# zhuker/lamejs

Measured on AMD Instinct MI355X. Metric: 1152-sample frames/s encoded (44.1kHz 128kbps CBR); bit-exact, higher is better.
Workload: dtype f64; 1 GPU; BASELINE configs[2]: stereo 44.1kHz 128kbps CBR, 1 stream(s) x 100000 synthetic sine frames per GPU; input=Int16 PCM resident in HBM, output=MP3 bytes in HBM, seed_repaired_frames=0, distinct_streams=1, distinct_devices=1

## Files before the change

### lamejs_amd/csrc/k_quant.h

```cpp
#pragma once
#include "lhip_defs.h"
#include "lhip_wave.h"
#include "lhip_math.h"
#include "lhip_layout.h"

namespace lhip {

struct GI {
    double xrpow_max;
    int part2_3_length, big_values, count1, global_gain, scalefac_compress, block_type;
    int table_select[3], subblock_gain[4];
    int region0_count, region1_count, preflag, scalefac_scale, count1table_select;
    int part2_length, sfb_lmax, sfb_smin, psy_lmax, sfbmax, psymax, sfbdivide;
    int count1bits, max_nonzero_coeff;
    int firstcut;
};

struct NoiseRes { double max_noise; int over_count, over_SSD, bits; };

LHIP_DEV void uni_gi(GI& g) {
    g.xrpow_max = unid(g.xrpow_max);
    g.part2_3_length = uni(g.part2_3_length); g.big_values = uni(g.big_values); g.count1 = uni(g.count1); g.global_gain = uni(g.global_gain);
    g.scalefac_compress = uni(g.scalefac_compress); g.block_type = uni(g.block_type);
    for (int i = 0; i < 3; i++) g.table_select[i] = uni(g.table_select[i]);
    for (int i = 0; i < 4; i++) g.subblock_gain[i] = uni(g.subblock_gain[i]);
    g.region0_count = uni(g.region0_count); g.region1_count = uni(g.region1_count); g.preflag = uni(g.preflag); g.scalefac_scale = uni(g.scalefac_scale);
    g.count1table_select = uni(g.count1table_select); g.part2_length = uni(g.part2_length); g.sfb_lmax = uni(g.sfb_lmax); g.sfb_smin = uni(g.sfb_smin);
    g.psy_lmax = uni(g.psy_lmax); g.sfbmax = uni(g.sfbmax); g.psymax = uni(g.psymax); g.sfbdivide = uni(g.sfbdivide);
    g.count1bits = uni(g.count1bits); g.max_nonzero_coeff = uni(g.max_nonzero_coeff); g.firstcut = uni(g.firstcut);
}

#if defined(LHIP_PHASE_PROF) && !defined(LHIP_HOSTSIM)
#define PH_BEGIN() const unsigned long long ph_t0_ = __builtin_amdgcn_s_memtime()
#define PH_END(L, id) do { if (lane == 0) { (L).prof[id] += (unsigned int)(__builtin_amdgcn_s_memtime() - ph_t0_); (L).prof[32 + id] += 1; } } while (0)
#define PH_MARK(L, id, t) do { const unsigned long long n_ = __builtin_amdgcn_s_memtime(); if (lane == 0) { (L).prof[id] += (unsigned int)(n_ - (t)); (L).prof[32 + id] += 1; } (t) = n_; } while (0)
#define PH_NOW() __builtin_amdgcn_s_memtime()
#else
#define PH_BEGIN() do {} while (0)
#define PH_END(L, id) do {} while (0)
#define PH_MARK(L, id, t) do {} while (0)
#define PH_NOW() 0ull
#endif
#ifdef LHIP_PROF_BALANCE
#define PH_MARKB(L, id, t) PH_MARK(L, id, t)
#else
#define PH_MARKB(L, id, t) do {} while (0)
#endif
enum { PH_INIT, PH_XRPOW, PH_XMIN, PH_QUANTIZE, PH_COUNT, PH_NOISE, PH_BALANCE, PH_SFSTORE, PH_HUFFDIV, PH_PUBLISH, PH_COPY, PH_TOTAL,
       PH_C_LOAD, PH_C_QUADS, PH_C_MAX, PH_C_SUMS, PH_C_FIN, PH_N_WALK, PH_N_TERMS, PH_N_SUMS, PH_Q_MASK, PH_Q_LINES, PH_N, PH_DRAIN = 29 ,
       PH_N_LINES = 30, PH_N_FOLD = 31 ,
       PH_B_TRIG = 22, PH_B_AMP = 23, PH_B_BREAK = 24, PH_B_BITCOUNT = 25  };

enum { QT_N = 256 };
enum { HL_T1 = 0, HL_T2 = 4, HL_T3 = 13, HL_T5 = 22, HL_T6 = 38, HL_T7 = 54, HL_T8 = 90, HL_T9 = 126, HL_T10 = 162, HL_T11 = 226,
       HL_T12 = 290, HL_T13 = 354, HL_T14 = 610, HL_T15 = 866, HL_EHI = 1122, HL_ELO = 1378, HL_END = 1634 };
LHIP_DEV int hl_off(int t) {
    switch (t) {
        case 1: return HL_T1; case 2: return HL_T2; case 3: return HL_T3; case 5: return HL_T5; case 6: return HL_T6;
        case 7: return HL_T7; case 8: return HL_T8; case 9: return HL_T9; case 10: return HL_T10; case 11: return HL_T11;
        case 12: return HL_T12; case 13: return HL_T13; case 14: return HL_T14; case 15: return HL_T15; default: return 0;
    }
}
// ... 196 lines not shown
    for (int k = 0; k < NV; k++) { va[k] = X.a[src[k]]; vb[k] = 0.f; }
    if (X.b) {
#pragma unroll
        for (int k = 0; k < NV; k++) vb[k] = X.b[src[k]];
    }
#pragma unroll
    for (int k = 0; k < NV; k++) { LHIP_PIN_LOADED(va[k]); LHIP_PIN_LOADED(vb[k]); }
#pragma unroll
    for (int k = 0; k < NV; k++) {
        float v = va[k];
        if (X.b) { const double l = va[k], r = vb[k]; v = X.side ? (float)((l - r) * (LHIP_SQRT2 * 0.5)) : (float)((l + r) * (LHIP_SQRT2 * 0.5)); }
        L.xr[lane + LHIP_NL * k] = v;
    }
#endif
}

LHIP_DEV void q_init_outer_loop(const Tables& T, const PowBase& pb10, double ath_adjust, GI& g, int block_type,
                                const XrSrc& xr_g, float* xr_wb, int skip_silence, int lane, QuantLds& L, const QuantTabs& Q) {
    lane = fresh_lane(lane);
    unsigned long long tmi_ = PH_NOW(); (void)tmi_;
    (void)pb10; (void)ath_adjust;
#if defined(LHIP_PHASE_PROF) && !defined(LHIP_HOSTSIM)
    __builtin_amdgcn_s_waitcnt(0);
    PH_MARK(L, PH_DRAIN, tmi_);
#endif
    g.part2_3_length = 0; g.big_values = 0; g.count1 = 0; g.global_gain = 210; g.scalefac_compress = 0;
    g.block_type = block_type;
    g.table_select[0] = g.table_select[1] = g.table_select[2] = 0;
    g.subblock_gain[0] = g.subblock_gain[1] = g.subblock_gain[2] = g.subblock_gain[3] = 0;
    g.region0_count = 0; g.region1_count = 0; g.preflag = 0; g.scalefac_scale = 0; g.count1table_select = 0;
    g.part2_length = 0; g.sfb_lmax = SBPSY_l; g.sfb_smin = SBPSY_s;
    g.psy_lmax = T.sfb21_extra ? SBMAX_l : SBPSY_l;
    g.psymax = g.psy_lmax; g.sfbmax = g.sfb_lmax; g.sfbdivide = 11;
    g.count1bits = 0; g.max_nonzero_coeff = 575; g.xrpow_max = 0; g.firstcut = 64;
    int nsfb;
    if (block_type == SHORT_TYPE) {
        g.sfb_smin = 0; g.sfb_lmax = 0;
        g.psymax = 3 * ((T.sfb21_extra ? SBMAX_s : SBPSY_s));
        g.sfbmax = 3 * SBPSY_s;
        g.sfbdivide = g.sfbmax - 18;
        g.psy_lmax = 0;
        nsfb = 3 * SBMAX_s;
        LHIP_LANE_ONCE(i, 0, nsfb) {
            const int sfb = i / 3, win = i - 3 * sfb;
            const int w = Q.sfb_s[sfb + 1] - Q.sfb_s[sfb];
            L.width[i] = (int16_t)w; L.window[i] = (int16_t)win; L.start[i] = (int16_t)(3 * Q.sfb_s[sfb] + win * w);
        }
        if (lane == 0) L.start[nsfb] = 576;
        q_load_lines(xr_g, 1, lane, L, Q);
    } else {
        nsfb = SBMAX_l;
        LHIP_LANE_ONCE(i, 0, SBMAX_l) {
            L.width[i] = (int16_t)(Q.sfb_l[i + 1] - Q.sfb_l[i]); L.window[i] = 3; L.start[i] = (int16_t)Q.sfb_l[i];
        }
        if (lane == 0) L.start[SBMAX_l] = 576;
        q_load_lines(xr_g, 0, lane, L, Q);
    }
    LHIP_LANE_ONCE(i, 0, (SFBMAX) + 1) { L.sfw[i] = 0; L.sfb[i] = 0; }
    wave_sync();
    PH_MARK(L, PH_COPY, tmi_);

    if (skip_silence) return;
    if (block_type != SHORT_TYPE) {
        const int lo = Q.psfb21[0];
        int top = lo - 1;
        for (int j = lo + lane; j < 576; j += LHIP_NL) {
            int gsfb = 0;
// ... 62 lines not shown
#else
    unsigned endm = 0;
    double keep[NLN_FOLD]; int bnd[NLN_FOLD];
    int prevb = (lane == 0) ? -1 : (int)l2s[NLN_FOLD * lane - 1];
#pragma unroll
    for (int k = 0; k < NLN_FOLD; k++) {
        const int j = NLN_FOLD * lane + k;
        bnd[k] = l2s[j];
        keep[k] = (bnd[k] != prevb) ? 0.0 : 1.0;
        prevb = bnd[k];
    }
    const int nextb = (lane == LHIP_NL - 1) ? -1 : (int)l2s[NLN_FOLD * (lane + 1)];
#pragma unroll
    for (int k = 0; k < NLN_FOLD; k++) if (bnd[k] != (k + 1 < NLN_FOLD ? bnd[k + 1 < NLN_FOLD ? k + 1 : k] : nextb)) endm |= 1u << k;
    const int nsteps = (maxlen + NLN_FOLD - 1) / NLN_FOLD + 1;
    double carry = 0.0;
    for (int st = 0; st + 1 < nsteps; st++) {
        double sacc = carry;
#pragma unroll
        for (int k = 0; k < NLN_FOLD; k++) sacc = __builtin_fma(sacc, keep[k], tq[k]);
        carry = wave_shr1d(sacc, 0.0);
    }
    {
        double sacc = carry;
#pragma unroll
        for (int k = 0; k < NLN_FOLD; k++) { sacc = __builtin_fma(sacc, keep[k], tq[k]); tq[k] = sacc; }
    }
#pragma unroll
    for (int k = 0; k < NLN_FOLD; k++) if ((endm >> k) & 1u) L.nsum[bnd[k]] = tq[k];
#endif
    wave_sync();
}

LHIP_DEV void q_calc_xmin(const Tables& T, double ath_adjust, double masking_lower, const float* ratio ,
                          GI& g, int lane, QuantLds& L, const QuantTabs& Q) {
    lane = fresh_lane(lane);
    {
        double tq[NLN_FOLD];
#pragma unroll
        for (int k = 0; k < NLN_FOLD; k++) { const double x = L.xr[NLN_FOLD * lane + k]; tq[k] = x * x; }
        int maxw = 0;
        const int nb = (g.block_type != SHORT_TYPE) ? g.psy_lmax : 3 * SBPSY_s;
        LHIP_LANE_ONCE(b, 0, nb) if (maxw < L.width[b]) maxw = L.width[b];
        maxw = wave_max(maxw);
        fold_band_sums(tq, line2sfb(Q, g.block_type), maxw, lane, L);
    }
    if (g.block_type != SHORT_TYPE) {
        LHIP_LANE_ONCE(gsfb, 0, g.psy_lmax) {
            double xmin = ath_adjust * (double)T.ATH_l[gsfb];
            const double en0 = L.nsum[gsfb];
            const double en = ratio[E_EN_L + gsfb];
            if (en > 0.0) {
                const double x = en0 * (double)ratio[E_THM_L + gsfb] * masking_lower / en;
                if (xmin < x) xmin = x;
            }
            const float xm = (float)(xmin * (double)T.longfact[gsfb]);
            L.xmin[gsfb] = xm; L.rxmin[gsfb] = recip_for_div((double)xm);
        }
        int t = -1;
        for (int k = lane; k < 576; k += LHIP_NL) if (!((double)L.xr[k] == 0)) t = k;
        t = wave_max(t);
        g.max_nonzero_coeff = (t >= 575) ? 575 : t + 1;
    } else {
        LHIP_LANE_ONCE(sfb, 0, SBPSY_s) {
            const double tmpATH = ath_adjust * (double)T.ATH_s[sfb];
            float px[3];
            for (int b = 0; b < 3; b++) {
                const int gs = 3 * sfb + b;
                double xmin = tmpATH;
                const double en0 = L.nsum[gs];
                const double en = ratio[E_EN_S + sfb * 3 + b];
                if (en > 0.0) {
                    const double x = en0 * (double)ratio[E_THM_S + sfb * 3 + b] * masking_lower / en;
                    if (xmin < x) xmin = x;
                }
                px[b] = (float)(xmin * (double)T.shortfact[sfb]);
            }
            if (T.useTemporal) {
                if ((double)px[0] > (double)px[1]) px[1] = (float)((double)px[1] + ((double)px[0] - (double)px[1]) * T.decay);
                if ((double)px[1] > (double)px[2]) px[2] = (float)((double)px[2] + ((double)px[1] - (double)px[2]) * T.decay);
            }
            L.xmin[3 * sfb] = px[0]; L.xmin[3 * sfb + 1] = px[1]; L.xmin[3 * sfb + 2] = px[2];
            L.rxmin[3 * sfb] = recip_for_div((double)px[0]); L.rxmin[3 * sfb + 1] = recip_for_div((double)px[1]); L.rxmin[3 * sfb + 2] = recip_for_div((double)px[2]);
        }
        g.max_nonzero_coeff = 575;
    }
    q_set_firstcut(g, lane, L);
    wave_sync();
}

enum { NPL = (288 + LHIP_NL - 1) / LHIP_NL };
LHIP_DEV void q_quantize(const Tables& T, const GI& g, const int32_t* scalefac, int16_t* ix, int use_prev,
                         int pn_gain, int pn_sfb_count1, int (&vx)[NPL], int (&vy)[NPL], int lane, QuantLds& L, const QuantTabs& Q) {
    lane = fresh_lane(lane);
    const double istep = ipow20(Q, g.global_gain);
    const int may_big = !(g.xrpow_max * istep < (double)QT_N);
    const int sfbmax = (g.block_type == SHORT_TYPE) ? 38 : 21;
    const int prev_data_use = use_prev && (g.global_gain == pn_gain);
    unsigned long long tm_ = PH_NOW(); (void)tm_;
    float xa[NPL], xb[NPL];
#pragma unroll
    for (int j = 0; j < NPL; j++) {
        const int p = 2 * (lane + LHIP_NL * j);
        xa[j] = 0.f; xb[j] = 0.f;
        if (p < 576) { struct F2 { float x, y; }; const F2 xx = *(const F2*)(L.xrpow + p); xa[j] = xx.x; xb[j] = xx.y; }
    }
    uint64_t m_cached = 0, m_zo = 0;
    if (use_prev) {
        LHIP_LANE_ONCE(sfb, 0, (sfbmax) + 1) {
            int step = -1;
            const int pstep = L.pn_step[sfb];
            if (prev_data_use || g.block_type == NORM_TYPE) step = sf_step(Q, g, scalefac, L.window, sfb);
            if (prev_data_use && pstep == step) m_cached |= 1ull << sfb;
            else if (pn_sfb_count1 > 0 && sfb >= pn_sfb_count1 && pstep > 0 && step >= pstep) m_zo |= 1ull << sfb;
        }
    }
    m_cached = wave_lane_bits(m_cached); m_zo = wave_lane_bits(m_zo);
    const uint64_t m_cut = (use_prev && g.firstcut <= sfbmax) ? ((~0ull << g.firstcut) & ((2ull << sfbmax) - 1) & ~m_cached) : 0;
    const int sstar = m_cut ? (int)__builtin_ctzll(m_cut) : 99;
    if (sstar <= sfbmax) m_zo &= ~(1ull << sstar);
    PH_MARK(L, PH_Q_MASK, tm_);
    const uint8_t* l2s = line2sfb(Q, g.block_type);
    const int need_old = (m_cached != 0);
    const float istep_f = Q.ipow20[g.global_gain];
    int ra[NPL], rb[NPL];
    q_floor_prod(xa, xb, istep_f, ra, rb);
    float aa[NPL], ab[NPL];
    if (!may_big) {
#pragma unroll
        for (int j = 0; j < NPL; j++) { aa[j] = Q.adj43[ra[j]]; ab[j] = Q.adj43[rb[j]]; }
    } else {
#pragma unroll
        for (int j = 0; j < NPL; j++) { aa[j] = Q.adj43[ra[j] < QT_N ? ra[j] : QT_N - 1]; ab[j] = Q.adj43[rb[j] < QT_N ? rb[j] : QT_N - 1]; }
#pragma unroll
        for (int j = 0; j < NPL; j++) {
            if (ra[j] >= QT_N) aa[j] = T.adj43[ra[j]];
            if (rb[j] >= QT_N) ab[j] = T.adj43[rb[j]];
        }
    }
    q_floor_fma(xa, xb, istep_f, aa, ab, vx, vy);
    if (!need_old && m_zo == 0) {
#pragma unroll
        for (int j = 0; j < NPL; j++) {
            const int p = 2 * (lane + LHIP_NL * j);
            if (p < 576) *(uint32_t*)(ix + p) = (uint32_t)vx[j] | ((uint32_t)vy[j] << 16);
        }
    } else if (m_zo == 0) {
#pragma unroll
        for (int j = 0; j < NPL; j++) {
            const int p = 2 * (lane + LHIP_NL * j);
            int sf = 0; uint32_t oldw = 0;
            if (p < 576) { sf = l2s[p]; oldw = *(const uint32_t*)(ix + p); }
            const int cached = (int)((m_cached >> sf) & 1);
            const int va = cached ? (int)(oldw & 0xffffu) : vx[j], vb = cached ? (int)(oldw >> 16) : vy[j];
            vx[j] = va; vy[j] = vb;
            if (p < 576) *(uint32_t*)(ix + p) = (uint32_t)va | ((uint32_t)vb << 16);
        }
    } else {
        const double compareval0 = (1.0 - 0.4054) / istep;
        float zo_thr = (float)compareval0;
        if ((double)zo_thr < compareval0) zo_thr = f32_next_up(zo_thr);
#pragma unroll
        for (int j = 0; j < NPL; j++) {
            const int p = 2 * (lane + LHIP_NL * j);
            int sf = 0; uint32_t oldw = 0;
            if (p < 576) { sf = l2s[p]; if (need_old) oldw = *(const uint32_t*)(ix + p); }
            const int cached = (int)((m_cached >> sf) & 1), zo = (int)((m_zo >> sf) & 1);
            int va = vx[j], vb = vy[j];
            if (zo) { va = (xa[j] < zo_thr) ? 0 : 1; vb = (xb[j] < zo_thr) ? 0 : 1; }
            const int oa = (int)(oldw & 0xffffu), ob = (int)(oldw >> 16);
            va = cached ? oa : va;
            vb = cached ? ob : vb;
            vx[j] = va; vy[j] = vb;
            if (p < 576) *(uint32_t*)(ix + p) = (uint32_t)va | ((uint32_t)vb << 16);
        }
    }
    wave_sync();
    PH_MARK(L, PH_Q_LINES, tm_);
}

struct RegionPlan { int kind, t1, xlen, lb1, lb2, choice, choice2, o0, o1, o2; };

LHIP_DEV void esc_choice(int mx15, int* choice, int* choice2, int* lb1, int* lb2) {
    const int bl = 32 - __builtin_clz((unsigned)mx15);
    const int c24 = bl <= 4 ? 0 : bl <= 9 ? bl - 4 : bl <= 11 ? 6 : 7;
    int f16 = bl <= 4 ? bl - 1 : 4 + ((bl - 5) >> 1);
    if (f16 > 7) f16 = 7;
    int c16 = c24 - 8 + 8;
    if (c16 < f16) c16 = f16;
    *choice2 = 24 + c24; *choice = 16 + c16;
    *lb1 = (int)((0xDA864321u >> (4 * c16)) & 15u);
    *lb2 = (int)((0xDB987654u >> (4 * c24)) & 15u);
}

LHIP_DEV int plan_index(int m) { return m <= 15 ? m : (m <= IXMAX_VAL ? 15 + (32 - __builtin_clz((unsigned)(m - 15) | 1u)) : 29); }
LHIP_DEV void q_fill_plans(QuantTabs& Q, int tid, int nthr) {
// ... 59 lines not shown
        case 2: { int t1 = r.t1, sum2 = s0 & 0xffff, sum = s0 >> 16; if (sum > sum2) { sum = sum2; t1++; } *bits += sum; return t1; }
        case 4: { int t = r.t1; if (s0 > s1) { s0 = s1; t++; } if (s0 > s2) { s0 = s2; t = r.t1 + 2; } *bits += s0; return t; }
        case 5: { int c = r.choice; if (s0 > s1) { s0 = s1; c = r.choice2; } *bits += s0; return c; }
        default: *bits = LARGE_BITS; return -1;
    }
}

LHIP_DEV int q_choose_table(const Tables& T, const int16_t* ix, int a, int b, int* bits, int lane, const QuantLds& L, const QuantTabs& Q) {
    int mx = 0;
    for (int p = a + 2 * lane; p < b; p += 2 * LHIP_NL) { const int x1 = ix[p], x2 = ix[p + 1]; if (mx < x1) mx = x1; if (mx < x2) mx = x2; }
    mx = wave_max(mx);
    const RegionPlan r = plan_region_(Q, mx);
    int s0 = 0, s1 = 0, s2 = 0;
    if (r.kind >= 1 && r.kind <= 5)
        for (int p = a + 2 * lane; p < b; p += 2 * LHIP_NL) pair_bits(Q, r, ix[p], ix[p + 1], s0, s1, s2);
    s0 = wave_sum(s0);
    if (r.kind >= 4) s1 = wave_sum(s1);
    if (r.kind == 4) s2 = wave_sum(s2);
    return finish_region(r, s0, s1, s2, bits);
}

LHIP_DEV int pack_cond_fields(const GI& g, int mask) {
    return mask | ((g.table_select[0] + 1) << 4) | ((g.table_select[1] + 1) << 10) | ((g.table_select[2] + 1) << 16) |
           (g.region0_count << 22) | (g.region1_count << 26);
}
LHIP_DEV int apply_cond_fields(int state, int asg) {
    if (asg & 1) state = (state & ~(63 << 4)) | (asg & (63 << 4));
    if (asg & 2) state = (state & ~(63 << 10)) | (asg & (63 << 10));
    if (asg & 4) state = (state & ~(63 << 16)) | (asg & (63 << 16));
    if (asg & 8) state = (state & ~(0x3ff << 22)) | (asg & (0x3ff << 22));
    return state & ~15;
}

LHIP_DEV int q_noquant_count_bits(const Tables& T, GI& g, const int16_t* ix, int (&vx)[NPL], int (&vy)[NPL], int use_prev, int* pn_sfb_count1, int* asg_mask, int lane, QuantLds& L, const QuantTabs& Q) {
    *asg_mask = 0;
    lane = fresh_lane(lane);
    unsigned long long tm_ = PH_NOW(); (void)tm_;
    int i = ((g.max_nonzero_coeff + 2) >> 1) << 1;
    if (i > 576) i = 576;
    if (use_prev) *pn_sfb_count1 = 0;
    int firstbig;
#if LHIP_NL == 1
    {
        int top = 0;
        for (int j = 0; j < NPL; j++) if ((vx[j] | vy[j]) != 0) top = 2 * (lane + LHIP_NL * j) + 2;
        i = top;
        const int nq = i >> 2;
        firstbig = nq;
        for (int k = 0; k < nq; k++) {
            const int e = i - 4 * k;
            if (((ix[e - 1] | ix[e - 2] | ix[e - 3] | ix[e - 4]) & 0x7fff) > 1) { firstbig = k; break; }
        }
    }
#else
    {
        int tp = -1, bp = -1;
#pragma unroll
        for (int j = 0; j < NPL; j++) {
            const uint64_t nz = wave_ballot((vx[j] | vy[j]) != 0), bg = wave_ballot((vx[j] | vy[j]) > 1);
            if (nz) tp = 64 * j + 63 - (int)__builtin_clzll(nz);
            if (bg) bp = 64 * j + 63 - (int)__builtin_clzll(bg);
        }
        i = 2 * tp + 2;
        const int P = tp + 1, nq = i >> 2;
        firstbig = (P - 1 - bp) >> 1;
        if (firstbig > nq) firstbig = nq;
    }
#endif
    g.count1 = i;
    PH_MARK(L, PH_C_LOAD, tm_);
    int a12 = 0;
    for (int k = lane; k < firstbig; k += LHIP_NL) {
        const int e = i - 4 * k;
        const uint32_t w0 = *(const uint32_t*)(ix + e - 4), w1 = *(const uint32_t*)(ix + e - 2);
        const int p = (int)(((w0 & 1u) << 3) | ((w0 >> 16) << 2) | ((w1 & 1u) << 1) | (w1 >> 16));
        a12 += Q.t32l[p] + (Q.t33l[p] << 16);
    }
    i -= 4 * firstbig;
    g.big_values = i;
    int a1, a2, bits;
#define COUNT1_FINISH(A12) do { const int c1_ = (A12) & 0xffff, c2_ = (int)((unsigned)(A12) >> 16); bits = c1_; g.count1table_select = 0; \
                                if (c1_ > c2_) { bits = c2_; g.count1table_select = 1; } g.count1bits = bits; } while (0)
    PH_MARK(L, PH_C_QUADS, tm_);
    if (i == 0) { const int t = wave_sum(a12); COUNT1_FINISH(t); return bits; }
    int use2 = 0, cnt1_norm = 0;
    if (g.block_type == SHORT_TYPE) {
        a1 = 3 * Q.sfb_s[3];
        if (a1 > g.big_values) a1 = g.big_values;
        a2 = g.big_values;
    } else if (g.block_type == NORM_TYPE) {
        const uint32_t bt = Q.bvtab[i >> 1];
        g.region0_count = (int)((bt >> 20) & 15u); g.region1_count = (int)((bt >> 24) & 7u);
        a1 = (int)(bt & 1023u); a2 = (int)((bt >> 10) & 1023u);
        cnt1_norm = (int)(bt >> 27);
        if (a2 < i) use2 = 1;
    } else {
        g.region0_count = 7;
        g.region1_count = SBMAX_l - 1 - 7 - 1;
        a1 = Q.sfb_l[7 + 1];
        a2 = i;
        if (a1 > a2) a1 = a2;
    }
    if (a1 > i) a1 = i;
    if (a2 > i) a2 = i;
    *asg_mask = (g.block_type != SHORT_TYPE ? 8 : 0) | (use2 ? 4 : 0) | (0 < a1 ? 1 : 0) | (a1 < a2 ? 2 : 0);
    int m0 = 0, m1 = 0, m2 = 0;
    int rj[NPL];
#pragma unroll
    for (int j = 0; j < NPL; j++) {
        rj[j] = 3;
        if (2 * LHIP_NL * j >= i) continue;
        const int p = 2 * (lane + LHIP_NL * j);
        const int r = (p >= a1) + (p >= a2) + (p >= i);
        const int m = vx[j] > vy[j] ? vx[j] : vy[j];
        const int mr0 = (r == 0) ? m : 0, mr1 = (r == 1) ? m : 0, mr2 = (r == 2) ? m : 0;
        m0 = m0 > mr0 ? m0 : mr0; m1 = m1 > mr1 ? m1 : mr1; m2 = m2 > mr2 ? m2 : mr2;
        rj[j] = r;
    }
    { int mm[3] = {m0, m1, m2}; wave_max_n(mm); m0 = mm[0]; m1 = mm[1]; m2 = mm[2]; }
    struct LanePlan { int kind, t0, t1, t2, lbA, lbB; };
#if LHIP_NL == 1
    LanePlan lp[3]; int pv[3];
#define LP_(r) lp[r]
#define PV_(r) pv[r]
#else
    LanePlan lp1; int pv1 = 0;
    lp1.kind = 0; lp1.t0 = lp1.t1 = lp1.t2 = lp1.lbA = lp1.lbB = 0;
#define LP_(r) lp1
#define PV_(r) pv1
#endif
    LHIP_LANE_ONCE(r, 0, 3) {
        const int m = (r == 0) ? m0 : (r == 1) ? m1 : (r == 2) ? m2 : 0;
        const QuantTabs::PlanEnt pe = Q.plan[plan_index(m)];
        L.rdesc[r][0] = pe.d0;
        L.rdesc[r][1] = pe.d1;
        LanePlan& q = LP_(r);
        q.kind = (int)(pe.pw & 7u); q.t0 = (int)((pe.pw >> 3) & 63u); q.t1 = (int)((pe.pw >> 9) & 63u); q.t2 = (int)((pe.pw >> 15) & 63u);
        q.lbA = (int)((pe.pw >> 21) & 15u); q.lbB = (int)((pe.pw >> 25) & 15u);
    }
    wave_sync();
    PH_MARK(L, PH_C_MAX, tm_);
#if LHIP_NL == 1
    typedef uint64_t acc_t; enum { FB = 21 };
#else
    typedef uint32_t acc_t; enum { FB = 10 };
#endif
    const acc_t FM = ((acc_t)1 << FB) - 1;
    acc_t accA = 0, accB = 0, accC = 0, accN = 0;
    const int any_esc = (m0 > 15) | (m1 > 15) | (m2 > 15);
#if LHIP_NL == 1
#pragma unroll
    for (int j = 0; j < NPL; j++) {
        const int p = 2 * (lane + LHIP_NL * j);
        if (p < i) {
            const int r = (p >= a1) + (p >= a2);
            const uint64_t d = *(const uint64_t*)L.rdesc[r];
            const uint32_t d0 = (uint32_t)d, d1 = (uint32_t)(d >> 32);
            const int x = vx[j], y = vy[j];
            const int idx = (x < 15 ? x : 15) * (int)(d1 >> 16) + (y < 15 ? y : 15);
            const int sh = FB * r;
            accA += (acc_t)Q.hlen[(d0 & 0xffffu) + idx] << sh;
            accB += (acc_t)Q.hlen[(d0 >> 16) + idx] << sh;
            accC += (acc_t)Q.hlen[(d1 & 0xffffu) + idx] << sh;
            if (any_esc) accN += (acc_t)((x > 14) + (y > 14)) << sh;
        }
    }
    (void)rj;
#else
    if (any_esc) {
#pragma unroll
        for (int j = 0; j < NPL; j++) {
            if (rj[j] < 3) {
                const int r = rj[j];
                const uint64_t d = *(const uint64_t*)L.rdesc[r];
                const uint32_t d0 = (uint32_t)d, d1 = (uint32_t)(d >> 32);
                const int x = vx[j], y = vy[j];
                const int idx = (x < 15 ? x : 15) * (int)(d1 >> 16) + (y < 15 ? y : 15);
                const unsigned mult = 1u << (FB * r);
                accA = mul24((unsigned)Q.hlen[(d0 & 0xffffu) + idx], mult) + accA;
                accB = mul24((unsigned)Q.hlen[(d0 >> 16) + idx], mult) + accB;
                accC = mul24((unsigned)Q.hlen[(d1 & 0xffffu) + idx], mult) + accC;
                accN = mul24((unsigned)((x > 14) + (y > 14)), mult) + accN;
            }
        }
    } else {
#pragma unroll
        for (int j = 0; j < NPL; j++) {
            if (rj[j] < 3) {
                const int r = rj[j];
                const uint64_t d = *(const uint64_t*)L.rdesc[r];
                const uint32_t d0 = (uint32_t)d, d1 = (uint32_t)(d >> 32);
                const int idx = vx[j] * (int)(d1 >> 16) + vy[j];
                const unsigned mult = 1u << (FB * r);
                accA = mul24((unsigned)Q.hlen[(d0 & 0xffffu) + idx], mult) + accA;
                accB = mul24((unsigned)Q.hlen[(d0 >> 16) + idx], mult) + accB;
                accC = mul24((unsigned)Q.hlen[(d1 & 0xffffu) + idx], mult) + accC;
            }
        }
    }
#endif
#define FLD(A, R) ((uint32_t)(((A) >> (FB * (R))) & FM))
    int qq[7] = {(int)(FLD(accA, 0) | (FLD(accB, 0) << 16)), (int)(FLD(accC, 0) | (FLD(accN, 0) << 16)), (int)(FLD(accA, 1) | (FLD(accB, 1) << 16)),
                 (int)(FLD(accC, 1) | (FLD(accN, 1) << 16)), (int)(FLD(accA, 2) | (FLD(accB, 2) << 16)), (int)(FLD(accC, 2) | (FLD(accN, 2) << 16)), a12};
    wave_sum_n(qq);
    const int q0 = qq[0], q1 = qq[1], q2 = qq[2], q3 = qq[3], q4 = qq[4], q5 = qq[5];
    COUNT1_FINISH(qq[6]);
#undef COUNT1_FINISH
#undef FLD
    PH_MARK(L, PH_C_SUMS, tm_);
    LHIP_LANE_ONCE(r, 0, 3) {
        const LanePlan& q = LP_(r);
        const int qa = (r == 0) ? q0 : (r == 1) ? q2 : q4, qc = (r == 0) ? q1 : (r == 1) ? q3 : q5;
        const int n = (int)((unsigned)qc >> 16);
        const int c0 = (qa & 0xffff) + n * q.lbA, c1 = (int)((unsigned)qa >> 16) + n * q.lbB, c2 = qc & 0xffff;
        int b = c0, t = q.t0;
        if ((q.kind == 2 || q.kind == 4 || q.kind == 5) && b > c1) { b = c1; t = q.t1; }
        if (q.kind == 4 && b > c2) { b = c2; t = q.t2; }
        if (q.kind == 0) { b = 0; t = 0; }
        if (q.kind == 6) { b = 0; t = 63; }
        PV_(r) = t | ((q.kind == 6) << 6) | (b << 8);
    }
#if LHIP_NL == 1
    const int pv0 = pv[0], pv1_ = pv[1], pv2 = pv[2];
#else
    const int pv0 = wave_bcast(pv1, 0), pv1_ = wave_bcast(pv1, 1), pv2 = wave_bcast(pv1, 2);
#endif
#define APPLY(PV, SLOT) do { const int t_ = (PV) & 63; if ((PV) & 64) bits = LARGE_BITS; else bits += (PV) >> 8; g.table_select[SLOT] = (t_ == 63) ? -1 : t_; } while (0)
    if (use2) APPLY(pv2, 2);
    if (0 < a1) APPLY(pv0, 0);
    if (a1 < a2) APPLY(pv1_, 1);
#undef APPLY
#undef LP_
#undef PV_
    if (use_prev && g.block_type == NORM_TYPE) *pn_sfb_count1 = cnt1_norm;
    PH_MARK(L, PH_C_FIN, tm_);
    return bits;
}

struct PrevNoise { int gain, sfb_count1; };

LHIP_DEV int q_count_bits(const Tables& T, GI& g, const int32_t* scalefac, int16_t* ix, int use_pn, PrevNoise& pn, int* asg, int lane, QuantLds& L, const QuantTabs& Q) {
    *asg = 0;
    {
        const double ip = ipow20(Q, g.global_gain);
        if (g.xrpow_max * ip > (double)IXMAX_VAL * (1.0 - 0x1p-50)) {
            const double w = (double)IXMAX_VAL / ip;
            if (g.xrpow_max > w) return LARGE_BITS;
        }
    }
    int vx[NPL], vy[NPL];
    { PH_BEGIN(); q_quantize(T, g, scalefac, ix, use_pn, use_pn ? pn.gain : 0, use_pn ? pn.sfb_count1 : 0, vx, vy, lane, L, Q); PH_END(L, PH_QUANTIZE); }
    int cnt1 = pn.sfb_count1;
    PH_BEGIN();
    int amask = 0;
    const int r = q_noquant_count_bits(T, g, ix, vx, vy, use_pn, &cnt1, &amask, lane, L, Q);
    *asg = pack_cond_fields(g, amask);
    if (use_pn) pn.sfb_count1 = cnt1;
    PH_END(L, PH_COUNT);
    return r;
}

struct NoiseCommit { int fresh, step, cls; float dist; double x; };
LHIP_DEV void q_noise_commit(const GI& g, const NoiseCommit& nc, PrevNoise& pn, int lane, QuantLds& L) {
    lane = fresh_lane(lane);
    LHIP_LANE_ONCE(sfb, 0, g.psymax) {
        if (nc.fresh) { L.pn_step[sfb] = nc.step; L.pn_dist[sfb] = nc.dist; L.pn_x[sfb] = nc.x; L.pn_cls[sfb] = (int16_t)nc.cls; }
    }
    pn.gain = g.global_gain;
    wave_sync();
}
LHIP_DEV void q_calc_noise_(const Tables& T, const GI& g, const int32_t* scalefac, const int16_t* ix, NoiseRes* res,
                           int use_pn, PrevNoise& pn, int need_max, int lane, QuantLds& L, const QuantTabs& Q, NoiseCommit* defer = nullptr) {
    lane = fresh_lane(lane);
    unsigned long long tm_ = PH_NOW(); (void)tm_;
    const int is_short = g.block_type == SHORT_TYPE;
    const int may_big = !(g.xrpow_max * ipow20(Q, g.global_gain) < (double)(QT_N - 1));
#if LHIP_NL == 1
    const uint8_t* l2s = line2sfb(Q, g.block_type);
    int over = 0, ssd = 0;
    uint64_t m_fresh = 0;
    (void)may_big; (void)is_short;
    for (int sfb = 0; sfb < g.psymax; sfb++) {
        const int s = sf_step(Q, g, scalefac, L.window, sfb);
        if (!(use_pn && L.pn_step[sfb] == s)) m_fresh |= 1ull << sfb;
        L.qmode[sfb] = s;
        L.bstep[sfb] = Q.pow20[s + Q_MAX2];
    }
    PH_MARK(L, PH_N_WALK, tm_);
    {
        double sacc = 0.0;
        for (int j = 0; j < 576; j++) {
            const int bnd = l2s[j];
// ... 188 lines not shown
#define LHIP_PIPE_COUNT(f) do { if (lane == 0) pipe_stats().f++; } while (0)
#else
#define LHIP_PIPE_COUNT(f) do { } while (0)
#endif
#if LHIP_NL != 1
LHIP_DEV void q_count_helper(const Tables& T, CountShare& cs, const QuantLds& Lo, QuantLds& L, const QuantTabs& Q, int lane) {
    for (;;) {
        const int s = wg_wait_not(&cs.state, CS_IDLE, CS_DONE, lane);
        if (s == CS_QUIT) break;
        if (s == CS_BARRIER) { wg_store(&cs.state, CS_IDLE, lane); wg_barrier(); continue; }
#ifdef LHIP_PHASE_PROF
        const unsigned long long hp_seen_ = __builtin_amdgcn_s_memtime();
#endif
#if HO_ON
        const unsigned long long ho_h0_ = HO_NOW();
#endif
        wg_acquire();
        lane = lane_anew(lane);
        GI g;
        g.block_type = uni(s >> 8); g.max_nonzero_coeff = 0;
        g.region0_count = 0; g.region1_count = 0; g.table_select[0] = g.table_select[1] = g.table_select[2] = 0;
        g.count1table_select = 0; g.count1bits = 0; g.count1 = 0; g.big_values = 0;
        int cnt1 = 0, amask = 0;
        int vx[NPL], vy[NPL];
#pragma unroll
        for (int j = 0; j < NPL; j++) {
            const int i = lane + LHIP_NL * j;
            const uint32_t w = i < 288 ? ((const uint32_t*)Lo.ixw)[i] : 0u;
            vx[j] = (int)(w & 0xffffu); vy[j] = (int)(w >> 16);
        }
#ifdef LHIP_PHASE_PROF
        const unsigned long long hp_start_ = __builtin_amdgcn_s_memtime();
#endif
        const int bits = uni(q_noquant_count_bits(T, g, Lo.ixw, vx, vy, 1, &cnt1, &amask, lane, L, Q));
#ifdef LHIP_PHASE_PROF
        const unsigned long long hp_end_ = __builtin_amdgcn_s_memtime();
#endif
        uni_gi(g);
        const uint32_t w0 = (uint32_t)bits | ((uint32_t)g.count1 << 17);
        const uint32_t w1 = (uint32_t)g.big_values | ((uint32_t)g.count1bits << 10) | ((uint32_t)g.count1table_select << 23) | ((uint32_t)g.region0_count << 24) | ((uint32_t)g.region1_count << 28);
        const uint32_t w2 = (uint32_t)(g.table_select[0] + 1) | ((uint32_t)(g.table_select[1] + 1) << 6) | ((uint32_t)(g.table_select[2] + 1) << 12) | ((uint32_t)uni(cnt1) << 18) | ((uint32_t)uni(amask) << 24);
        if (lane == 0) { cs.w[0] = w0; cs.w[1] = w1; cs.w[2] = w2; }
#ifdef LHIP_PHASE_PROF
        if (lane == 0) { const unsigned long long now_ = __builtin_amdgcn_s_memtime(); cs.acc[0] += (unsigned int)(hp_seen_ - cs.t_post); cs.acc[1] += (unsigned int)(hp_start_ - hp_seen_);
                         cs.acc[2] += (unsigned int)(hp_end_ - hp_start_); cs.acc[3] += (unsigned int)(now_ - hp_end_); cs.acc[7] += 1; cs.t_reply = now_; }
#endif
#if HO_ON
        const unsigned long long ho_h1_ = HO_NOW();
        if (lane == 0) cs.t_reply = ho_h1_;
#endif
        wg_store(&cs.state, CS_DONE, lane);
#if HO_ON
        HO_ADD(cs, 3, ho_h1_ - ho_h0_); HO_ADD(cs, 4, 1); HO_ADD(cs, 5, ho_h0_ - cs.t_post);
#endif
    }
}
LHIP_DEV int q_count_bits_piped(const Tables& T, GI& g, const int32_t* scalefac, int16_t* ix, PrevNoise& pn, int* asg, CountShare& cs,
                                NoiseRes* ni, NoiseCommit* nc, int need_max, int* spec, int lane, QuantLds& L, const QuantTabs& Q) {
    *asg = 0; *spec = 0;
    {
        const double ip = ipow20(Q, g.global_gain);
        if (g.xrpow_max * ip > (double)IXMAX_VAL * (1.0 - 0x1p-50)) {
            const double w = (double)IXMAX_VAL / ip;
            if (g.xrpow_max > w) return LARGE_BITS;
        }
    }
    {
        int vx[NPL], vy[NPL];
        PH_BEGIN(); q_quantize(T, g, scalefac, ix, 1, pn.gain, pn.sfb_count1, vx, vy, lane, L, Q); PH_END(L, PH_QUANTIZE);
        (void)vx; (void)vy;
    }
#ifdef LHIP_PHASE_PROF
    if (lane == 0) cs.t_post = __builtin_amdgcn_s_memtime();
#endif
#if HO_ON
    const unsigned long long ho_t0_ = HO_NOW();
    if (lane == 0) cs.t_post = ho_t0_;
#endif
    wg_store(&cs.state, CS_REQ | (g.block_type << 8), lane);
    LHIP_PIPE_COUNT(piped);
    { PH_BEGIN(); q_calc_noise_(T, g, scalefac, ix, ni, 1, pn, need_max, lane, L, Q, nc); PH_END(L, PH_NOISE); }
    *spec = 1;
#if HO_ON
    const unsigned long long ho_t1_ = HO_NOW();
#endif
    PH_BEGIN();
#ifdef LHIP_PHASE_PROF
    const unsigned long long op_wait0_ = __builtin_amdgcn_s_memtime();
#endif
    (void)wg_wait_not(&cs.state, CS_REQ | (g.block_type << 8), CS_REQ | (g.block_type << 8), lane);
#ifdef LHIP_PHASE_PROF
    if (lane == 0) { const unsigned long long now_ = __builtin_amdgcn_s_memtime(); cs.acc[4] += (unsigned int)(now_ - cs.t_reply); cs.acc[5] += (unsigned int)(op_wait0_ - cs.t_post); cs.acc[6] += (unsigned int)(now_ - op_wait0_); }
#endif
#if HO_ON
    const unsigned long long ho_t2_ = HO_NOW();
#endif
    wg_acquire();
    const uint32_t w0 = (uint32_t)uni((int)cs.w[0]), w1 = (uint32_t)uni((int)cs.w[1]), w2 = (uint32_t)uni((int)cs.w[2]);
#if HO_ON
    HO_ADD(cs, 0, ho_t1_ - ho_t0_); HO_ADD(cs, 1, ho_t2_ - ho_t1_); HO_ADD(cs, 2, 1); HO_ADD(cs, 6, ho_t2_ - cs.t_reply);
#endif
    const int bits = (int)(w0 & 0x1ffffu), amask = (int)((w2 >> 24) & 15u);
// ... 51 lines not shown
    uint32_t m = 0;
    LHIP_LANE_ONCE(i, 0, end) {
        int v = scalefac[i];
        if (v < 0) v = 0;
        const int part = (i >= b1) + (i >= b2) + (i >= b3);
        m |= (uint32_t)v << (8 * part);
    }
    m = (uint32_t)wave_or((int)m);
    int over = 0, slen[4];
    for (int p = 0; p < 4; p++) {
        const uint32_t mp = (m >> (8 * p)) & 0xffu;
        if (mp > ((range >> (8 * p)) & 0xffu)) over = 1;
        slen[p] = mp ? 32 - __builtin_clz(mp) : 0;
    }
    if (!over) {
        g.scalefac_compress = pre ? 500 + slen[0] * 3 + slen[1] : ((slen[0] * 5 + slen[1]) << 4) + (slen[2] << 2) + slen[3];
        g.part2_length = slen[0] * n0 + slen[1] * n1 + slen[2] * n2 + slen[3] * n3;
    }
    return over;
}

LHIP_DEV int q_scale_bitcount_any(const Tables& T, const QuantTabs& Q, GI& g, int32_t* scalefac, int lane) {
    return T.mode_gr == 2 ? q_scale_bitcount(Q, g, scalefac, lane) : q_scale_bitcount_lsf(g, scalefac, lane);
}

LHIP_DEV int q_loop_break(const GI& g, const int32_t* scalefac, int lane, QuantLds& L, const QuantTabs& Q) {
    lane = fresh_lane(lane);
    int z = 0;
    LHIP_LANE_ONCE(sfb, 0, g.sfbmax)
        if (scalefac[sfb] + band_sbgain(g, L.window, sfb) == 0) z = 1;
    return !wave_any(z);
}

LHIP_DEV void q_amplify_flagged(GI& g, double amp, uint64_t m_amp, int lane, QuantLds& L, const QuantTabs& Q) {
    lane = fresh_lane(lane);
    float m = 0.f;
    const uint8_t* l2s = line2sfb(Q, g.block_type);
    struct F2 { float x, y; };
    F2 xx[NPL]; int bnd[NPL];
#pragma unroll
    for (int j = 0; j < NPL; j++) {
        const int p = 2 * (lane + LHIP_NL * j);
        xx[j].x = 0.f; xx[j].y = 0.f; bnd[j] = 0;
        if (p < 576) { xx[j] = *(const F2*)(L.xrpow + p); bnd[j] = l2s[p]; }
    }
#pragma unroll
    for (int j = 0; j < NPL; j++) {
        const int p = 2 * (lane + LHIP_NL * j);
        const double a = ((m_amp >> bnd[j]) & 1) ? amp : 1.0;
        xx[j].x = (float)((double)xx[j].x * a); xx[j].y = (float)((double)xx[j].y * a);
        if (p < 576) *(F2*)(L.xrpow + p) = xx[j];
        m = fmax_nonneg(m, fmax_nonneg(xx[j].x, xx[j].y));
    }
    m = wave_maxf_pos(m);
    if ((double)m > g.xrpow_max) g.xrpow_max = m;
    wave_sync();
}

LHIP_DEV void q_amp_scalefac_bands(const Tables& T, GI& g, int32_t* scalefac, int* all_nonzero, int* pre_bad, int* m12_out,
                                   int lane, QuantLds& L, const QuantTabs& Q) {
    lane = fresh_lane(lane);
    const double ifqstep34 = (g.scalefac_scale == 0) ? 1.29683955465100964055 : 1.68179283050742922612;
    float tr = 0.f;
    LHIP_LANE_ONCE(sfb, 0, g.sfbmax) if (tr < L.distort[sfb]) tr = L.distort[sfb];
    double trigger = wave_maxf_pos(tr);
    const int by_square = T.noise_shaping_amp == 1 && trigger > 1.0;
    const double max_dist = trigger;
    switch (T.noise_shaping_amp) {
        case 2: break;
        case 1:
            if (!(trigger > 1.0)) trigger *= .95;
            break;
        default:
            if (trigger > 1.0) trigger = 1.0;
            else trigger *= .95;
            break;
    }
    uint64_t m_amp = 0;
    LHIP_LANE_ONCE(sfb, 0, g.sfbmax) {
        const double d = (double)L.distort[sfb];
        const int below = by_square ? (d * d < max_dist) : (d < trigger);
        if (!below) m_amp |= 1ull << sfb;
    }
    m_amp = wave_lane_bits(m_amp);
    if (T.noise_shaping_amp == 2 && m_amp) m_amp = 1ull << __builtin_ctzll(m_amp);
    int z = 0, bad = 0, m12 = 0;
    LHIP_LANE_ONCE(sfb, 0, g.sfbmax) {
        const int v = scalefac[sfb] + (int)((m_amp >> sfb) & 1);
        scalefac[sfb] = v;
        if (v + band_sbgain(g, L.window, sfb) == 0) z = 1;
        if (sfb >= 11 && sfb < SBPSY_l && v < Q.pretab[sfb]) bad = 1;
        m12 |= (sfb < g.sfbdivide) ? v : (v << 8);
    }
    {
        const int r = wave_or(m12 | (z << 16) | (bad << 17));
        *m12_out = r & 0xffff; *all_nonzero = !((r >> 16) & 1); *pre_bad = (r >> 17) & 1;
    }
    { unsigned long long tt_ = PH_NOW(); (void)tt_; q_amplify_flagged(g, ifqstep34, m_amp, lane, L, Q); PH_MARKB(L, PH_B_TRIG, tt_); }
}

LHIP_DEV int q_scale_bitcount_from(const QuantTabs& Q, GI& g, int32_t* scalefac, int pre_bad, int m12, int lane) {
    lane = fresh_lane(lane);
    const int sh = (g.block_type == SHORT_TYPE) ? 24 : 16;
    if (g.block_type != SHORT_TYPE && 0 == g.preflag && !pre_bad) {
        g.preflag = 1;
        wave_sync();
        LHIP_LANE_ONCE(sfb, 11, SBPSY_l) scalefac[sfb] -= Q.pretab[sfb];
        wave_sync();
        m12 = 0;
        LHIP_LANE_ONCE(sfb, 0, g.sfbmax) { const int v = scalefac[sfb]; m12 |= (sfb < g.sfbdivide) ? v : (v << 8); }
        m12 = wave_or(m12);
    }
    const int m1 = m12 & 0xff, m2 = m12 >> 8;
    int best = 0x7fffffff;
    LHIP_LANE_ONCE(k, 0, 16) {
        const uint32_t e = Q.sbc[k];
        if (m1 < (int)(e & 0xffu) && m2 < (int)((e >> 8) & 0xffu)) { const int v = (int)((e >> sh) & 0xffu) * 16 + k; if (v < best) best = v; }
    }
    best = wave_min(best);
    g.part2_length = LARGE_BITS;
    if (best != 0x7fffffff) { g.part2_length = best >> 4; g.scalefac_compress = best & 15; }
    return g.part2_length == LARGE_BITS;
}

LHIP_DEV void q_inc_scalefac_scale(const Tables& T, GI& g, int32_t* scalefac, int lane, QuantLds& L, const QuantTabs& Q) {
    lane = fresh_lane(lane);
    uint64_t m_amp = 0;
    LHIP_LANE_ONCE(sfb, 0, g.sfbmax) {
        int s = scalefac[sfb];
        if (g.preflag != 0) s += Q.pretab[sfb];
        if ((s & 1) != 0) { s++; m_amp |= 1ull << sfb; }
        scalefac[sfb] = s >> 1;
    }
    m_amp = wave_lane_bits(m_amp);
    wave_sync();
    g.preflag = 0;
    g.scalefac_scale = 1;
    q_amplify_flagged(g, 1.29683955465100964055, m_amp, lane, L, Q);
}

LHIP_DEV int q_inc_subblock_gain(const Tables& T, GI& g, int32_t* scalefac, int lane, QuantLds& L, const QuantTabs& Q) {
    lane = fresh_lane(lane);
    for (int window = 0; window < 3; window++) {
        int s1 = 0, s2 = 0;
        LHIP_LANE_ONCE3(sfb, window, g.sfbmax) {
            const int v = scalefac[sfb];
            if (sfb < g.sfbdivide) { if (s1 < v) s1 = v; } else { if (s2 < v) s2 = v; }
        }
        s1 = wave_max(s1); s2 = wave_max(s2);
        if (s1 < 16 && s2 < 8) continue;
        if (sbgain(g, window) >= 7) return 1;
        if (window == 0) g.subblock_gain[0]++; else if (window == 1) g.subblock_gain[1]++; else g.subblock_gain[2]++;
        wave_sync();
        for (int sfb = window; sfb < g.sfbmax + 3; sfb += 3) {
            double amp;
            int doamp = 0;
            int s = (sfb < g.sfbmax) ? scalefac[sfb] : 0;
            wave_sync();
            if (sfb < g.sfbmax) {
                s = s - (4 >> g.scalefac_scale);
                if (s >= 0) { if (lane == 0) scalefac[sfb] = s; }
                else {
                    if (lane == 0) scalefac[sfb] = 0;
                    amp = ipow20(Q, 210 + s * (1 << (g.scalefac_scale + 1)));
                    doamp = 1;
                }
            } else { amp = ipow20(Q, 202); doamp = 1; }
            wave_sync();
            if (uni(doamp)) {
                float m = 0.f;
                const int st = L.start[sfb], w = L.width[sfb];
                for (int i = st + lane; i < st + w; i += LHIP_NL) {
                    const float v = (float)((double)L.xrpow[i] * amp);
                    L.xrpow[i] = v;
                    m = fmax_nonneg(m, v);
                }
                m = wave_maxf_pos(m);
                if ((double)m > g.xrpow_max) g.xrpow_max = m;
            }
        }
        wave_sync();
    }
    return 0;
}

LHIP_DEV int q_balance_noise(const Tables& T, GI& g, int32_t* scalefac, int lane, QuantLds& L, const QuantTabs& Q) {
    lane = fresh_lane(lane);
    unsigned long long tb_ = PH_NOW(); (void)tb_;
    int all_nonzero, pre_bad, m12;
    q_amp_scalefac_bands(T, g, scalefac, &all_nonzero, &pre_bad, &m12, lane, L, Q);
    PH_MARKB(L, PH_B_AMP, tb_);
    int status = all_nonzero;
    if (status) return 0;
    status = T.mode_gr == 2 ? q_scale_bitcount_from(Q, g, scalefac, pre_bad, m12, lane) : q_scale_bitcount_lsf(g, scalefac, lane);
    PH_MARKB(L, PH_B_BITCOUNT, tb_);
    if (!status) return 1;
    if (T.noise_shaping > 1) {
        if (0 == g.scalefac_scale) {
            q_inc_scalefac_scale(T, g, scalefac, lane, L, Q);
            status = 0;
        } else if (g.block_type == SHORT_TYPE && T.subblock_gain > 0) {
            status = (q_inc_subblock_gain(T, g, scalefac, lane, L, Q) || q_loop_break(g, scalefac, lane, L, Q));
        }
    }
    if (!status) status = q_scale_bitcount_any(T, Q, g, scalefac, lane);
    return !status;
}

LHIP_DEV int q_quant_compare(const NoiseRes& best, const NoiseRes& calc) {
    int better;
    if (best.over_count > 0) {
        better = calc.over_SSD <= best.over_SSD;
        if (calc.over_SSD == best.over_SSD) better = calc.bits < best.bits;
    } else {
        better = ((calc.max_noise < 0) && ((calc.max_noise * 10 + calc.bits) <= (best.max_noise * 10 + best.bits)));
    }
    if (best.over_count == 0) better = better && calc.bits < best.bits;
    return better;
}

LHIP_DEV void gi_keep_store(QuantLds& L, const GI& w, int lane) {
    lane = fresh_lane(lane);
    if (lane == 0) {
        int32_t* k = L.gkeep;
        k[0] = w.part2_3_length; k[1] = w.big_values; k[2] = w.count1; k[3] = w.global_gain; k[4] = w.scalefac_compress;
        k[5] = w.table_select[0]; k[6] = w.table_select[1]; k[7] = w.table_select[2];
        k[8] = w.subblock_gain[0]; k[9] = w.subblock_gain[1]; k[10] = w.subblock_gain[2]; k[11] = w.subblock_gain[3];
        k[12] = w.region0_count; k[13] = w.region1_count; k[14] = w.preflag; k[15] = w.scalefac_scale; k[16] = w.count1table_select;
        k[17] = w.part2_length; k[18] = w.count1bits;
        union { double d; int32_t i[2]; } u; u.d = w.xrpow_max; k[19] = u.i[0]; k[20] = u.i[1];
    }
}
LHIP_DEV void gi_keep_load(const QuantLds& L, GI& g) {
    const int32_t* k = L.gkeep;
    g.part2_3_length = uni(k[0]); g.big_values = uni(k[1]); g.count1 = uni(k[2]); g.global_gain = uni(k[3]); g.scalefac_compress = uni(k[4]);
    g.table_select[0] = uni(k[5]); g.table_select[1] = uni(k[6]); g.table_select[2] = uni(k[7]);
    g.subblock_gain[0] = uni(k[8]); g.subblock_gain[1] = uni(k[9]); g.subblock_gain[2] = uni(k[10]); g.subblock_gain[3] = uni(k[11]);
    g.region0_count = uni(k[12]); g.region1_count = uni(k[13]); g.preflag = uni(k[14]); g.scalefac_scale = uni(k[15]); g.count1table_select = uni(k[16]);
    g.part2_length = uni(k[17]); g.count1bits = uni(k[18]);
    union { double d; int32_t i[2]; } u; u.i[0] = uni(k[19]); u.i[1] = uni(k[20]); g.xrpow_max = u.d;
}

#if defined(LHIP_HOSTSIM)
struct SearchStats {
    long bs[40] = {0}, bsup[40] = {0}, run[40] = {0}, run_cnt1_moved[40] = {0}, rounds = 0, evals = 0, searches = 0, run_steps = 0, run_steps_cnt1_moved = 0, run_steps_zo = 0;
    long bsdir[8][3][2] = {{{0}}};
    long mfail[24] = {0}, mfit[24] = {0};
    bool on = getenv("LAMEJS_SEARCH_STATS") != nullptr;
    ~SearchStats() {
        if (!on) return;
        fprintf(stderr, "search stats: %ld granule-channel searches, %ld evaluations, %ld outer-loop rounds; %ld evaluations inside gain++ runs (%ld of them with sfb_count1 moved by the evaluation before, %ld with a live 0/1 shortcut)\n", searches, evals, rounds, run_steps, run_steps_cnt1_moved, run_steps_zo);
        auto pr = [](const char* nm, const long* h) { fprintf(stderr, "  %s:", nm); for (int i = 0; i < 40; i++) if (h[i]) fprintf(stderr, " %d:%ld", i, h[i]); fprintf(stderr, "\n"); };
        pr("bin-search evaluations per search", bs); pr("step-up evaluations after it", bsup); pr("gain++ run length per outer-loop round (0 = the first evaluation fits)", run);
        pr("runs in which sfb_count1 moved, by run length", run_cnt1_moved);
        fprintf(stderr, "  bin-search evaluations, index / last move (- up down): under/over:"); for (int i = 0; i < 8; i++) for (int d = 0; d < 3; d++) if (bsdir[i][d][0] + bsdir[i][d][1]) fprintf(stderr, " %d%c:%ld/%ld", i, "-ud"[d], bsdir[i][d][0], bsdir[i][d][1]); fprintf(stderr, "\n");
        fprintf(stderr, "  first evaluation of a round, by margin huff_bits - previous bits (bucket of 8 bits: fails / fits):"); for (int i = 0; i < 24; i++) if (mfail[i] + mfit[i]) fprintf(stderr, " %d:%ld/%ld", 8 * (i - 4), mfail[i], mfit[i]); fprintf(stderr, "\n");
    }
};
inline SearchStats& search_stats() { static SearchStats t; return t; }
#define LHIP_SS(...) do { if (lane == 0 && search_stats().on) { SearchStats& ss_ = search_stats(); __VA_ARGS__; } } while (0)
#else
#define LHIP_SS(...) do { } while (0)
#endif
LHIP_DEV void q_outer_loop(const Tables& T, GI& g, int targ_bits, int bs_start, int bs_step, int* bs_gain_out,
                           int16_t* kept, GrSide* rec, uint32_t* dig, int64_t dn, int lane, QuantLds& L, const QuantTabs& Q, CountShare* cs = nullptr) {
    lane = fresh_lane(lane);
    enum { ST_BS, ST_BSUP, ST_A, ST_B };
    NoiseRes best, ni;
    PrevNoise pn; pn.gain = 0; pn.sfb_count1 = 0;
    best.max_noise = 0; best.over_count = 0; best.over_SSD = 0; best.bits = 0;
    LHIP_LANE_ONCE(i, 0, (SFBMAX) + 1) { L.pn_step[i] = 0; L.pn_dist[i] = 0.f; L.pn_x[i] = 1.0; L.pn_cls[i] = 0; L.distort[i] = 0.f; }
    wave_sync();
    targ_bits = uni(targ_bits); bs_start = uni(bs_start); bs_step = uni(bs_step);
    uni_gi(g);
    GI w = g;
    int CurrentStep = bs_step, flagGoneOver = 0, Direction = 0;
    const int desired_rate = targ_bits - w.part2_length;
    w.global_gain = bs_start;
    int best_part2_3_length = 9999999, age = 0, maxggain = 255, huff_bits = 0, first = 1;
    int kept_p23 = g.part2_3_length;
    const int search_limit = 3;
    int st = ST_BS, nbs = 0;
    int ss_nbs = 0, ss_nup = 0, ss_run = 0, ss_moved = 0, ss_first_ = 0, ss_prev_bits_ = 0; (void)ss_nbs; (void)ss_nup; (void)ss_run; (void)ss_moved; (void)ss_first_; (void)ss_prev_bits_;
    LHIP_SS(ss_.searches++);
    for (;;) {
#ifndef LHIP_NO_FORCE_UNI
        uni_gi(w); kept_p23 = uni(kept_p23); st = uni(st); CurrentStep = uni(CurrentStep); flagGoneOver = uni(flagGoneOver); Direction = uni(Direction);
        best_part2_3_length = uni(best_part2_3_length); age = uni(age); maxggain = uni(maxggain); huff_bits = uni(huff_bits); first = uni(first);
        pn.gain = uni(pn.gain); pn.sfb_count1 = uni(pn.sfb_count1);
        best.max_noise = unid(best.max_noise); best.over_count = uni(best.over_count); best.over_SSD = uni(best.over_SSD); best.bits = uni(best.bits);
#endif
        int asg = 0;
        const int cnt1_seen = pn.sfb_count1;
        int nBits, spec = 0;
        NoiseCommit nc; nc.fresh = 0; nc.step = 0; nc.cls = 0; nc.dist = 0.f; nc.x = 0.0;
#if LHIP_NL != 1
        if (cs != nullptr && st >= ST_A) nBits = q_count_bits_piped(T, w, L.sfw, L.ixw, pn, &asg, *cs, &ni, &nc, best.over_count == 0, &spec, lane, L, Q);
        else
#endif
        nBits = q_count_bits(T, w, L.sfw, L.ixw, st >= ST_A, pn, &asg, lane, L, Q);
        LHIP_SS(ss_.evals++; if (st == ST_BS) ss_nbs++; else if (st == ST_BSUP) ss_nup++;
                if (st >= ST_A && ss_run > 0) { ss_.run_steps++; if (ss_moved) ss_.run_steps_cnt1_moved++; if (cnt1_seen > 0) ss_.run_steps_zo++; });
        if (st <= ST_BSUP && nbs < BS_TAB_MAX) { if (lane == 0) { L.memo.bs_tab[nbs] = (w.global_gain << 24) | nBits; L.memo.bs_asg[nbs] = asg; } nbs++; }
        LHIP_SS(if (st <= ST_BSUP) { const int i_ = (ss_nbs + ss_nup - 1) < 7 ? (ss_nbs + ss_nup - 1) : 7; ss_.bsdir[i_ < 0 ? 0 : i_][st == ST_BSUP ? 1 : Direction][nBits > desired_rate]++; });
        if (st == ST_BS) {
            if (CurrentStep == 1 || nBits == desired_rate) st = ST_BSUP;
            else {
                int step;
                if (nBits > desired_rate) {
                    if (Direction == 2) flagGoneOver = 1;
                    if (flagGoneOver) CurrentStep /= 2;
                    Direction = 1;
                    step = CurrentStep;
                } else {
                    if (Direction == 1) flagGoneOver = 1;
                    if (flagGoneOver) CurrentStep /= 2;
                    Direction = 2;
                    step = -CurrentStep;
                }
                w.global_gain += step;
                if (w.global_gain < 0) { w.global_gain = 0; flagGoneOver = 1; }
                if (w.global_gain > 255) { w.global_gain = 255; flagGoneOver = 1; }
                continue;
            }
        }
        if (st == ST_BSUP) {
            if (nBits > desired_rate && w.global_gain < 255) { w.global_gain++; continue; }
            w.part2_3_length = nBits;
            LHIP_SS(ss_.bs[ss_nbs < 39 ? ss_nbs : 39]++; ss_.bsup[ss_nup < 39 ? ss_nup : 39]++);
            *bs_gain_out = w.global_gain;
            wave_sync();
            LHIP_LANE_ONCE(i, 0, nbs) {
                const int32_t e = L.memo.bs_tab[i], a = L.memo.bs_asg[i];
// ... 21 lines not shown
            if (best.over_count == 0) {
                st = ST_B;
                if (pn.sfb_count1 != cnt1_seen) continue;
                if (nBits > best_part2_3_length && w.global_gain <= maxggain) { LHIP_SS(ss_run++; ss_moved = (pn.sfb_count1 != cnt1_seen)); w.global_gain++; continue; }
                if (w.global_gain > maxggain) break;
            }
        } else {
            w.part2_3_length = nBits;
            if (nBits > best_part2_3_length && w.global_gain <= maxggain) { LHIP_SS(ss_run++; ss_moved = (pn.sfb_count1 != cnt1_seen)); w.global_gain++; continue; }
            if (w.global_gain > maxggain) break;
        }
        LHIP_SS(if (st >= ST_A) { ss_.rounds++; ss_.run[ss_run < 39 ? ss_run : 39]++; }  ss_run = 0; ss_moved = 0);
        if (spec) { q_noise_commit(w, nc, pn, lane, L); LHIP_PIPE_COUNT(committed); }
        else q_calc_noise(T, w, L.sfw, L.ixw, &ni, 1, pn, best.over_count == 0, lane, L, Q);
        ni.bits = w.part2_3_length;
        int keep;
        if (first) keep = 1;
        else keep = q_quant_compare(best, ni);
        if (keep) {
            if (!first) best_part2_3_length = kept_p23;
            best = ni;
            gi_keep_store(L, w, lane);
            kept_p23 = w.part2_3_length;
            for (int i = lane; i < 288; i += LHIP_NL) ((uint32_t*)kept)[i] = ((const uint32_t*)L.ixw)[i];
            LHIP_LANE_ONCE(i, 0, (SFBMAX) + 1) L.sfb[i] = L.sfw[i];
            wave_sync();
            age = 0;
        } else if (T.full_outer_loop == 0) {
            if (++age > search_limit && best.over_count == 0) break;
        }
        if (!first && !((w.global_gain + w.scalefac_scale) < 255)) break;
        first = 0;
        int bal_;
        { PH_BEGIN(); bal_ = q_balance_noise(T, w, L.sfw, lane, L, Q); PH_END(L, PH_BALANCE); }
        if (!bal_) break;
        maxggain = (w.scalefac_scale != 0) ? 254 : 255;
        huff_bits = targ_bits - w.part2_length;
        if (huff_bits <= 0) break;
        LHIP_SS(ss_first_ = 1; ss_prev_bits_ = w.part2_3_length);
        st = ST_A;
    }
    wave_sync();
    { const GI inv = w; g = inv; gi_keep_load(L, g); }
}

LHIP_DEV void q_best_scalefac_store(const Tables& T, GI& g, int gr, int ch, int gr0_block_type, int* scfsi ,
                                    int lane, QuantLds& L, const QuantTabs& Q) {
    lane = fresh_lane(lane);
    int32_t* sf = L.sfb;
    int recalc = 0;
    {
        LHIP_LANE_ONCE(sfb, 0, (SFBMAX) + 1) L.qmode[sfb] = 0;
        wave_sync();
        const uint8_t* l2s = line2sfb(Q, g.block_type);
        for (int p = 2 * lane; p < 576; p += 2 * LHIP_NL)
            if (*(const uint32_t*)(L.ixw + p) != 0) L.qmode[l2s[p]] = 1;
        wave_sync();
        int any = 0;
        LHIP_LANE_ONCE(sfb, 0, g.sfbmax) if (!L.qmode[sfb]) { sf[sfb] = -2; any = 1; }
        if (wave_any(any)) recalc = -2;
        wave_sync();
    }
    if (0 == g.scalefac_scale && 0 == g.preflag) {
        int s = 0;
        LHIP_LANE_ONCE(sfb, 0, g.sfbmax) if (sf[sfb] > 0) s |= sf[sfb];
        s = wave_or(s);
        if (0 == (s & 1) && s != 0) {
// ... 398 lines not shown
            targ[1] -= move_bits;
        } else {
            targ[0] += targ[1] - 125;
            targ[1] = 125;
        }
    }
    move_bits = targ[0] + targ[1];
    if (move_bits > max_bits) {
        targ[0] = js_toint32((max_bits * targ[0]) / move_bits);
        targ[1] = js_toint32((max_bits * targ[1]) / move_bits);
    }
}

LHIP_DEV int targ_bits_for(const Tables& T, int mean_bits, int gr, int ResvSize, int* targ) {
    const int C = uni_here(T.channels_out);
    int rs = ResvSize, tbits, bits = 0;
    if (gr != 0) rs += mean_bits;
    tbits = mean_bits;
    if (rs * 10 > 0) tbits += rs;
    for (int ch = 0; ch < C; ++ch) {
        const double t = (double)tbits / C;
        targ[ch] = js_toint32(t < MAX_BITS_PER_CHANNEL ? t : (double)MAX_BITS_PER_CHANNEL);
        bits += targ[ch];
    }
    if (bits > MAX_BITS_PER_GRANULE)
        for (int ch = 0; ch < C; ++ch) {
            targ[ch] = js_toint32((double)targ[ch] * MAX_BITS_PER_GRANULE);
            targ[ch] = js_toint32((double)targ[ch] / bits);
        }
    return tbits < MAX_BITS_PER_GRANULE ? tbits : MAX_BITS_PER_GRANULE;
}

struct UnitOut { int bits; Seed next; int block_type; int active; };
LHIP_DEV UnitOut q_unit(const Tables& T, const PowBase& pb10, const Workspace& W, int C, int Cp, int fidx, int gslot, int gr, int ch, int mode_ext,
                        double ath_adjust, int targ_ch, Seed used, int gr0_bt, int lane, QuantLds& L, const QuantTabs& Q, CountShare* cs = nullptr) {
    lane = lane_anew(lane);
    UnitOut u; u.next = used;
    GI g;
    const int bt = W.blocktype[(int64_t)gslot * C + ch];
    const double masking_lower = (bt != SHORT_TYPE) ? T.masking_lower_long : T.masking_lower_short;
    const float* ratio = W.E + ((int64_t)(gslot - 1) * Cp + ch + mode_ext) * E_STRIDE;
    { PH_BEGIN(); q_init_outer_loop(T, pb10, ath_adjust, g, bt, xr_source(W, C, gslot, ch, mode_ext == 2), mode_ext == 2 ? nullptr : W.xr + ((int64_t)gslot * C + ch) * 576, 0, lane, L, Q); PH_END(L, PH_INIT); }
    int active = 0, bs_gain = 0;
    if (q_init_xrpow(g, lane, L, Q)) {
        active = 1;
        { PH_BEGIN(); q_calc_xmin(T, ath_adjust, masking_lower, ratio, g, lane, L, Q); PH_END(L, PH_XMIN); }
        int16_t* kept = cs ? cs->kept : W.l3 + (((int64_t)fidx * 2 + gr) * C + ch) * 576;
        { PH_BEGIN(); q_outer_loop(T, g, targ_ch, used.start, used.step, &bs_gain, kept, W.side + ((int64_t)fidx * 2 + gr) * C + ch, W.vdig + ((int64_t)fidx * 2 + gr) * C + ch, W.vdig_n, lane, L, Q, cs); PH_END(L, PH_XRPOW); }
        uni_gi(g); bs_gain = uni(bs_gain);
        lane = lane_anew(lane);
        wave_sync();
#if LHIP_NL == 1
        for (int i = lane; i < 288; i += LHIP_NL) ((uint32_t*)L.ixw)[i] = ((const uint32_t*)kept)[i];
#else
        {
            uint32_t kw[NPL];
#pragma unroll
            for (int j = 0; j < NPL; j++) { const int i = lane + LHIP_NL * j; kw[j] = ((const uint32_t*)kept)[i < 288 ? i : 287]; }
#pragma unroll
            for (int j = 0; j < NPL; j++) LHIP_PIN_LOADED(kw[j]);
#pragma unroll
            for (int j = 0; j < NPL; j++) { const int i = lane + LHIP_NL * j; if (i < 288) ((uint32_t*)L.ixw)[i] = kw[j]; }
        }
#endif
        wave_sync();
        Seed nx; nx.step = (used.start - bs_gain >= 4) ? 4 : 2; nx.start = bs_gain;
        u.next = nx;
    } else {
        for (int i = lane; i < 576; i += LHIP_NL) L.ixw[i] = 0;
        wave_sync();
    }
    int scfsi[4];
    { PH_BEGIN(); q_best_scalefac_store(T, g, gr, ch, gr0_bt, scfsi, lane, L, Q); PH_END(L, PH_SFSTORE); }
    uni_gi(g);
    if (T.use_best_huffman == 1) { PH_BEGIN(); q_best_huffman_divide(T, g, lane, L, Q); PH_END(L, PH_HUFFDIV); }
    uni_gi(g);
    u.bits = g.part2_3_length + g.part2_length;
    u.block_type = g.block_type;
    if (gr == 0) { LHIP_LANE_ONCE(i, 0, (SFBMAX) + 1) L.sf_gr0[ch][i] = (int8_t)L.sfb[i]; }
    lane = lane_anew(lane);
    GrSide* out = W.side + ((int64_t)fidx * 2 + gr) * C + ch;
    if (lane == 0) {
        out->part2_3_length = g.part2_3_length; out->part2_length = g.part2_length; out->big_values = g.big_values;
        out->count1 = g.count1; out->global_gain = g.global_gain; out->scalefac_compress = g.scalefac_compress;
        out->block_type = g.block_type;
        for (int i = 0; i < 3; i++) { out->table_select[i] = g.table_select[i]; out->subblock_gain[i] = g.subblock_gain[i]; }
        out->region0_count = g.region0_count; out->region1_count = g.region1_count; out->preflag = g.preflag;
        out->scalefac_scale = g.scalefac_scale; out->count1table_select = g.count1table_select;
        out->sfbmax = g.sfbmax; out->sfbdivide = g.sfbdivide;
        out->active = active; out->bs_start = used.start; out->bs_step_in = used.step; out->bs_gain = bs_gain;
        W.vdig[((int64_t)fidx * 2 + gr) * C + ch] = vd_head(active, used.start, used.step, bs_gain);
        out->targ_bits = targ_ch;
        out->mode_ext = mode_ext;
        out->scfsi = scfsi[0] | (scfsi[1] << 1) | (scfsi[2] << 2) | (scfsi[3] << 3);
    }
    LHIP_LANE_ONCE(i, 0, SFBMAX) out->scalefac[i] = L.sfb[i];
    if (!active && lane == 0) { out->bs_ntab = 0; out->bs_state = 0; }
    int16_t* l3o = W.l3 + (((int64_t)fidx * 2 + gr) * C + ch) * 576;
    for (int i = lane; i < 576; i += LHIP_NL) {
        const int v = L.ixw[i];
        l3o[i] = (int16_t)(((double)L.xr[i] < 0) ? -v : v);
    }
    wave_sync();
    u.active = active;
    return u;
}

template <int PAIR = 0, int RESV = 0>
LHIP_DEV void kb_quant(const Tables& T, const PowBase& pb10, const Workspace& W, const StreamDesc* SD, int fslot,
                       int chain, int lane, QuantLds& L, const QuantTabs& Q, int my_ch = -1, int* mbox = nullptr, const ResvState* rvp = nullptr,
                       int* hint = nullptr, CountShare* cs = nullptr, const int* later_granules_ready = nullptr) {
    const int C = T.channels_out;
    const int st = W.fslot_stream[fslot];
    const StreamDesc sd = SD[st];
    const int k = fslot - sd.fslot0 - 1;
    if (k < 0) return;
    const int fidx = sd.out_slot0 + k;
    if (chain == 1 && !W.seed_flag[fidx]) return;
#ifdef LHIP_PHASE_PROF
    const unsigned long long ph_total0_ = __builtin_amdgcn_s_memtime();
#endif
    const double ath_adjust = W.ath_adjust[fslot];
    const int padding = frame_padding(T, sd, k);
    const int mean_bits = (frame_bits_of(T, padding) - T.sideinfo_len * 8) / T.mode_gr;
    Seed seed0, seed1;
    seed0.start = seed1.start = W.spec_start; seed0.step = seed1.step = W.spec_step;
    if (chain == 2) {
        const int32_t* ps = W.seed + (int64_t)(fslot - 1) * C * 2;
        seed0.start = uni(ps[0]); seed0.step = uni(ps[1]);
        if (C > 1) { seed1.start = uni(ps[2]); seed1.step = uni(ps[3]); }
    } else if (chain || k == 0) {
        seed0 = seed_before(W, sd, C, k, 0, 0);
        if (C > 1) seed1 = seed_before(W, sd, C, k, 0, 1);
    }
#ifndef LHIP_NO_SEED_HINT
    else if (hint && hint[0] == st) {
        if (hint[1] >= 0) { seed0.start = hint[1]; seed0.step = 2; }
        if (C > 1 && hint[2] >= 0) { seed1.start = hint[2]; seed1.step = 2; }
    }
#endif
    int gr0_bt0 = 0, gr0_bt1 = 0;
// ... 11 lines not shown
        if (ResvMax > resvLimit) ResvMax = resvLimit;
        if (ResvMax < 0) ResvMax = 0;
        if (T.mode != 1) q_frame_pe(T, W, sd, k, lane, L);
        double f = 0.0;
        for (int gr = 0; gr < T.mode_gr; gr++)
            for (int ch = 0; ch < C; ch++) { pe_use[gr][ch] = L.nsum[4 * gr + ch + mode_ext]; f += pe_use[gr][ch]; }
        pefir_new = (float)f;
        {
            const double fircoef[9] = {-0.0207887 * 5, -0.0378413 * 5, -0.0432472 * 5, -0.031183 * 5, 7.79609e-18 * 5, 0.0467745 * 5,
                                       0.10091 * 5, 0.151365 * 5, 0.187098 * 5};
            f = rv->pefirbuf[10];
            for (int i = 0; i < 9; i++) f += ((double)rv->pefirbuf[i + 1] + (double)(i == 0 ? pefir_new : rv->pefirbuf[19 - i])) * fircoef[i];
        }
        f = (670 * 5 * T.mode_gr * C) / f;
        for (int gr = 0; gr < T.mode_gr; gr++)
            for (int ch = 0; ch < C; ch++) pe_use[gr][ch] *= f;
        wave_sync();
    }
    q_ath_pseudo(T, pb10, ath_adjust, lane, L, Q);
    for (int gr = 0; gr < T.mode_gr; gr++) {
        const int gslot = sd.gslot0 + 1 + T.mode_gr * k + gr;
        if (gr > 0 && later_granules_ready) { (void)wg_wait_not(later_granules_ready, 0, 0, lane); wg_acquire(); }
        int targ[2] = {0, 0};
        const double max_bits = resv ? q_on_pe_resv(T, pe_use[gr], targ, mean_bits, gr, ResvSize, ResvMax) : (double)targ_bits_for(T, mean_bits, gr, ResvSize, targ);
        if (mode_ext == 2) {
            const float* te = W.tot_ener + (int64_t)(gslot - 1) * 4;
            double r = (double)te[2] + (double)te[3];
            if (r > 0) r = (double)te[3] / r;
            q_reduce_side(targ, r, mean_bits, max_bits);
        }
        const int targ0 = uni(targ[0]), targ1 = uni(targ[1]);
        for (int ch = 0; ch < C; ch++) {
            if (PAIR && ch != my_ch) continue;
            const UnitOut u = q_unit(T, pb10, W, C, Cp, fidx, gslot, gr, ch, mode_ext, ath_adjust, ch == 0 ? targ0 : targ1, ch == 0 ? seed0 : seed1,
                                     ch == 0 ? gr0_bt0 : gr0_bt1, lane, L, Q, cs);
            if (u.active) { if (ch == 0) seed0 = u.next; else seed1 = u.next; }
            if (!PAIR) ResvSize = uni(ResvSize - u.bits);
            else if (lane == 0) mbox[2 * gr + ch] = u.bits;
            if (gr == 0) { if (ch == 0) gr0_bt0 = u.block_type; else gr0_bt1 = u.block_type; }
        }
        if (PAIR) {
            if (cs) wg_store(&cs->state, CS_BARRIER, lane);
            wg_barrier();
            ResvSize = uni(ResvSize - (mbox[2 * gr] + mbox[2 * gr + 1]));
        }
    }
    if constexpr (resv) if (lane == 0 && (!PAIR || my_ch == 0)) {
        const double mdb0 = rv->main_data_begin;
        int rs = ResvSize + mean_bits * T.mode_gr, over_bits, stuffingBits = 0;
        if ((over_bits = rs % 8) != 0) stuffingBits += over_bits;
        over_bits = (rs - stuffingBits) - ResvMax;
        if (over_bits > 0) stuffingBits += over_bits;
        const double mdb_bytes = (mdb0 * 8 < stuffingBits ? mdb0 * 8 : (double)stuffingBits) / 8;
        FrameResv fr;
        fr.drain_pre = js_toint32(8 * mdb_bytes);
        stuffingBits -= fr.drain_pre;
        rs -= fr.drain_pre;
        fr.main_data_begin = mdb0 - mdb_bytes;
        fr.drain_post = stuffingBits;
        rs -= stuffingBits;
        fr.ResvSize = rs; fr.ResvMax = ResvMax; fr.pefir_new = pefir_new; fr.pad_ = 0;
        W.fr[fidx] = fr;
    }
    if (hint) { hint[0] = st; hint[1] = seed0.start; hint[2] = C > 1 ? seed1.start : -1; }
    if (chain == 1 && lane == 0) W.seed_flag[fidx] = 0;
    if (chain == 2 && lane == 0) {
        int32_t* ps = W.seed + (int64_t)fslot * C * 2;
        if (!PAIR || my_ch == 0) { ps[0] = seed0.start; ps[1] = seed0.step; }
        if (C > 1 && (!PAIR || my_ch == 1)) { ps[2] = seed1.start; ps[3] = seed1.step; }
    }
#ifdef LHIP_PHASE_PROF
    if (lane == 0) { L.prof[PH_TOTAL] += (unsigned int)(__builtin_amdgcn_s_memtime() - ph_total0_); L.prof[32 + PH_TOTAL] += 1; }
#endif
}

LHIP_DEV void kb_validate(const Tables& T, const PowBase& pb10, const Workspace& W, const StreamDesc* SD, int fslot,
                          int lane, QuantLds& L, const QuantTabs& Q) {
    const int C = T.channels_out;
    const int st = W.fslot_stream[fslot];
    const StreamDesc sd = SD[st];
    const int k = fslot - sd.fslot0 - 1;
    if (k < 0) return;
    const int fidx = sd.out_slot0 + k;
    if (uni(W.seed_flag[fidx]) != 2) return;
    const double ath_adjust = W.ath_adjust[fslot];
    int bad = 0;
    for (int gr = 0; gr < T.mode_gr && !bad; gr++) {
        const int gslot = sd.gslot0 + 1 + T.mode_gr * k + gr;
        for (int ch = 0; ch < C && !bad; ch++) {
            const GrSide* rec = W.side + ((int64_t)fidx * 2 + gr) * C + ch;
            if (!rec->active) continue;
            const Seed s = seed_before(W, sd, C, k, gr, ch);
            if (s.start == rec->bs_start && s.step == rec->bs_step_in) continue;
            const int ntab = uni(rec->bs_ntab);
            int my_ent = 0, my_asg = 0;
            LHIP_LANE_ONCE(i, 0, ntab) { my_ent = rec->bs_tab[i]; my_asg = rec->bs_asg[i]; }
            GI g;
            PrevNoise pn_none; pn_none.gain = 0; pn_none.sfb_count1 = 0;
            int inited = 0;
            const int desired_rate = uni(rec->targ_bits);
            int gain = uni(s.start), CurrentStep = uni(s.step), flagGoneOver = 0, Direction = 0, up = 0;
            GI g0;
            g0.table_select[0] = g0.table_select[1] = g0.table_select[2] = 0; g0.region0_count = 0; g0.region1_count = 0;
            int cstate = pack_cond_fields(g0, 0);
            for (;;) {
                int nBits = -1, asg = 0;
#if LHIP_NL == 1
                for (int i = 0; i < ntab; i++) if ((int)((uint32_t)rec->bs_tab[i] >> 24) == gain) { nBits = rec->bs_tab[i] & 0xffffff; asg = rec->bs_asg[i]; break; }
                (void)my_ent; (void)my_asg;
#else
                {
                    const uint64_t hit = wave_ballot(lane < ntab && (int)((uint32_t)my_ent >> 24) == gain);
                    if (hit) {
                        const int src = (int)__builtin_ctzll(hit);
                        nBits = wave_bcast(my_ent, src) & 0xffffff;
                        asg = wave_bcast(my_asg, src);
                    }
                }
#endif
                if (nBits < 0) {
                    if (!inited) {
                        const int ms = uni(rec->mode_ext) == 2;
                        if (ms) q_ath_pseudo(T, pb10, ath_adjust, lane, L, Q);
                        q_init_outer_loop(T, pb10, ath_adjust, g, W.blocktype[(int64_t)gslot * C + ch],
                                          xr_source(W, C, gslot, ch, ms), nullptr, ms ? 0 : 1, lane, L, Q);
                        q_init_xrpow(g, lane, L, Q);
                        if (g.block_type != SHORT_TYPE) {
                            int t = -1;
                            for (int i = lane; i < 576; i += LHIP_NL) if (!((double)L.xr[i] == 0)) t = i;
                            t = wave_max(t);
                            g.max_nonzero_coeff = (t >= 575) ? 575 : t + 1;
                        }
                        q_set_firstcut(g, lane, L);
                        inited = 1;
                    }
                    g.global_gain = gain;
                    nBits = q_count_bits(T, g, L.sfb, L.ixw, 0, pn_none, &asg, lane, L, Q);
                }
                nBits = uni(nBits);
                cstate = apply_cond_fields(cstate, uni(asg));
                if (!up) {
                    if (CurrentStep == 1 || nBits == desired_rate) up = 1;
                    else {
                        int step;
                        if (nBits > desired_rate) {
                            if (Direction == 2) flagGoneOver = 1;
                            if (flagGoneOver) CurrentStep /= 2;
                            Direction = 1;
                            step = CurrentStep;
                        } else {
                            if (Direction == 1) flagGoneOver = 1;
                            if (flagGoneOver) CurrentStep /= 2;
                            Direction = 2;
                            step = -CurrentStep;
                        }
                        gain += step;
                        if (gain < 0) { gain = 0; flagGoneOver = 1; }
                        if (gain > 255) { gain = 255; flagGoneOver = 1; }
                        continue;
                    }
                }
                if (nBits > desired_rate && gain < 255) { gain++; continue; }
                break;
            }
            if (gain != rec->bs_gain || cstate != (rec->bs_state & ~15)) bad = 1;
        }
    }
    if (lane == 0) {
        W.seed_flag[fidx] = bad ? 1 : 0;
        if (bad) {
// ... 149 lines not shown
```

### lamejs_amd/csrc/k_quant_tail.h

```cpp
#pragma once
namespace lhip {

struct TailOffer { int state, fslot, gr, mode_ext, targ, seed_start, seed_step, gr0_bt, bits, next_start, next_step, block_type, active, pad_[3]; };
struct TailShare { int drawing, pad_[3]; TailOffer offer[8]; };

#if defined(LHIP_WAVESIM)
struct TailStats { long claimed = 0, withdrawn = 0; ~TailStats() { if (getenv("LAMEJS_TAILHELP_STATS")) fprintf(stderr, "tail-help: %ld granule-channels by helpers, %ld offers withdrawn\n", claimed, withdrawn); } };
inline TailStats& tail_stats() { static TailStats t; return t; }
#define LHIP_TAIL_COUNT(f) do { if (lane == 0) tail_stats().f++; } while (0)
#else
#define LHIP_TAIL_COUNT(f) do { } while (0)
#endif

LHIP_DEV void kb_quant_th(const Tables& T, const PowBase& pb10, const Workspace& W, const StreamDesc* SD, int fslot, int lane, QuantLds& L,
                          const QuantTabs& Q, int* hint, TailShare& TS, int wv) {
    lane = lane_anew(lane);
    const int C = T.channels_out;
    const int st = uni(W.fslot_stream[fslot]);
    const StreamDesc sd = SD[st];
    const int k = uni(fslot - sd.fslot0 - 1);
    if (k < 0) return;
    const int fidx = uni(sd.out_slot0 + k);
#ifdef LHIP_PHASE_PROF
    const unsigned long long ph_total0_ = __builtin_amdgcn_s_memtime();
#endif
    const double ath_adjust = unid(W.ath_adjust[fslot]);
    const int padding = uni(frame_padding(T, sd, k));
    const int mean_bits = uni((frame_bits_of(T, padding) - T.sideinfo_len * 8) / T.mode_gr);
    Seed seed0, seed1;
    seed0.start = seed1.start = W.spec_start; seed0.step = seed1.step = W.spec_step;
    if (k == 0) {
        seed0 = seed_before(W, sd, C, k, 0, 0);
        if (C > 1) seed1 = seed_before(W, sd, C, k, 0, 1);
        seed0.start = uni(seed0.start); seed0.step = uni(seed0.step); seed1.start = uni(seed1.start); seed1.step = uni(seed1.step);
    } else if (hint[0] == st) {
        if (hint[1] >= 0) { seed0.start = hint[1]; seed0.step = 2; }
        if (C > 1 && hint[2] >= 0) { seed1.start = hint[2]; seed1.step = 2; }
    }
    int gr0_bt0 = 0, gr0_bt1 = 0;
    const int Cp = T.psy_channels;
    const int mode_ext = (T.mode == 1) ? q_ms_decision(T, W, sd, k, lane, L) : 0;
    int ResvSize = 0;
    q_ath_pseudo(T, pb10, ath_adjust, lane, L, Q);
    TailOffer& o = TS.offer[wv];
    for (int gr = 0; gr < T.mode_gr; gr++) {
        const int gslot = sd.gslot0 + 1 + T.mode_gr * k + gr;
        int targ[2] = {0, 0};
        const double max_bits = (double)targ_bits_for(T, mean_bits, gr, ResvSize, targ);
        if (mode_ext == 2) {
            const float* te = W.tot_ener + (int64_t)(gslot - 1) * 4;
            double r = (double)te[2] + (double)te[3];
            if (r > 0) r = (double)te[3] / r;
            q_reduce_side(targ, r, mean_bits, max_bits);
        }
        const int targ0 = uni(targ[0]), targ1 = uni(targ[1]);
        if (C == 2) {
            if (lane == 0) { o.fslot = fslot; o.gr = gr; o.mode_ext = mode_ext; o.targ = targ1; o.seed_start = seed1.start; o.seed_step = seed1.step; o.gr0_bt = gr0_bt1; }
            wg_store(&o.state, 1, lane);
        }
        for (int ch = 0; ch < C; ch++) {
            if (ch == 1 && wg_cas(&o.state, 1, 0, lane) != 1) {
                { long spins = 0; while (wg_load(&o.state, lane) != 3) { wg_idle(); LHIP_SPIN_GUARD(spins); } }
                wg_acquire();
                const int bits = uni(o.bits), act = uni(o.active), ns = uni(o.next_start), nstep = uni(o.next_step), bt = uni(o.block_type);
                if (act) { seed1.start = ns; seed1.step = nstep; }
                ResvSize = uni(ResvSize - bits);
                if (gr == 0) gr0_bt1 = bt;
                wg_store(&o.state, 0, lane);
                continue;
            }
            if (ch == 1) LHIP_TAIL_COUNT(withdrawn);
            const UnitOut u = q_unit(T, pb10, W, C, Cp, fidx, gslot, gr, ch, mode_ext, ath_adjust, ch == 0 ? targ0 : targ1, ch == 0 ? seed0 : seed1,
                                     ch == 0 ? gr0_bt0 : gr0_bt1, lane, L, Q);
            if (u.active) { if (ch == 0) seed0 = u.next; else seed1 = u.next; }
            ResvSize = uni(ResvSize - u.bits);
            if (gr == 0) { if (ch == 0) gr0_bt0 = u.block_type; else gr0_bt1 = u.block_type; }
        }
    }
    hint[0] = st; hint[1] = seed0.start; hint[2] = C > 1 ? seed1.start : -1;
#ifdef LHIP_PHASE_PROF
    if (lane == 0) { L.prof[PH_TOTAL] += (unsigned int)(__builtin_amdgcn_s_memtime() - ph_total0_); L.prof[32 + PH_TOTAL] += 1; }
#endif
}

LHIP_DEV void tail_help(const Tables& T, const PowBase& pb10, const Workspace& W, const StreamDesc* SD, int lane, QuantLds* Lall, int wv, int nwaves,
                        const QuantTabs& Q, TailShare& TS) {
    lane = lane_anew(lane);
    QuantLds& L = Lall[wv];
    const int C = T.channels_out, Cp = T.psy_channels;
    wg_add(&TS.drawing, -1, lane);
    long idle_rounds = 0;
    for (;;) {
        int took = 0;
        for (int w = 0; w < nwaves; w++) {
            if (w == wv) continue;
            TailOffer& o = TS.offer[w];
            if (wg_load(&o.state, lane) != 1) continue;
            if (wg_cas(&o.state, 1, 2, lane) != 1) continue;
            wg_acquire();
            took = 1;
            lane = lane_anew(lane);
            LHIP_TAIL_COUNT(claimed);
            const int fslot = uni(o.fslot), gr = uni(o.gr), mode_ext = uni(o.mode_ext), targ = uni(o.targ), gr0_bt = uni(o.gr0_bt);
            Seed seed; seed.start = uni(o.seed_start); seed.step = uni(o.seed_step);
            const int st = uni(W.fslot_stream[fslot]);
            const StreamDesc sd = SD[st];
            const int k = uni(fslot - sd.fslot0 - 1), fidx = uni(sd.out_slot0 + k), gslot = uni(sd.gslot0 + 1 + T.mode_gr * k + gr);
            const double ath_adjust = unid(W.ath_adjust[fslot]);
            q_ath_pseudo(T, pb10, ath_adjust, lane, L, Q);
            if (gr == 1) { LHIP_LANE_ONCE(i, 0, (SFBMAX) + 1) L.sf_gr0[1][i] = Lall[w].sf_gr0[1][i]; }
            wave_sync();
            const UnitOut u = q_unit(T, pb10, W, C, Cp, fidx, gslot, gr, 1, mode_ext, ath_adjust, targ, seed, gr0_bt, lane, L, Q);
            if (gr == 0) { LHIP_LANE_ONCE(i, 0, (SFBMAX) + 1) Lall[w].sf_gr0[1][i] = L.sf_gr0[1][i]; }
            if (lane == 0) { o.bits = u.bits; o.active = u.active; o.next_start = u.next.start; o.next_step = u.next.step; o.block_type = u.block_type; }
            wg_store(&o.state, 3, lane);
        }
        if (!took) {
            if (wg_load(&TS.drawing, lane) <= 0) break;
            wg_idle();
            LHIP_SPIN_GUARD(idle_rounds);
        }
    }
}

}
```

### lamejs_amd/csrc/lhip_api.cpp

```cpp
#include "../../include/lamejs_hip.h"
#include "lhip_defs.h"
#include "lhip_wave.h"
#include "lhip_math.h"
#include "lhip_layout.h"
#include "k_psy.h"
#include "k_fb.h"
#include "k_quant.h"
#if !defined(LHIP_HOSTSIM) || defined(LHIP_WAVESIM)
#include "k_quant_tail.h"
#endif
#include "k_bits.h"
#include "k_crc.h"
#include "k_ingest.h"
#include "k_gain.h"

#include <string>
#include <vector>
#include <map>
#include <mutex>
#include <thread>
#include <atomic>
#include <memory>
#include <cstring>
#include <cstdlib>
// ... 574 lines not shown
    Context* ctx = get_context(device);
    std::lock_guard<std::mutex> lk(ctx->mu);
    ctx->stream = hip_stream;
    return 0;
}

void lhip_last_batch_stats(int64_t* frames, int64_t* repaired_frames, int64_t* repair_iterations) {
#ifndef LHIP_HOSTSIM
    if (g_stat_pending) {
        Context* ctx = g_stat_pending;
        g_stat_pending = nullptr;
        std::lock_guard<std::mutex> lk(ctx->mu);
        int32_t fx[3] = {0, 0, 0};
        WorkSet& ws = ctx->ws;
        void* st = ctx->stream;
        if (rt::set_device(ctx->device) && rt::d2h(fx, (const int32_t*)ws.nflagged.p + FX_STATS, sizeof fx, st) && rt::sync(st)) {
            g_stat_repaired = fx[0]; g_stat_iters = fx[1];
            if (fx[2]) set_err("seed-chain repair did not converge");
        }
    }
#endif
    if (frames) *frames = g_stat_frames;
    if (repaired_frames) *repaired_frames = g_stat_repaired;
    if (repair_iterations) *repair_iterations = g_stat_iters;
}

int lhip_debug_last_paths(uint32_t* mask) {
    if (!mask) { set_err("lhip_debug_last_paths: null argument"); return LHIP_ERR_INTERNAL; }
    *mask = g_last_paths;
    return 0;
}

int64_t lhip_debug_read(int what, void* dst, size_t cap) {
#ifdef LHIP_PHASE_PROF
    if (what == 9) { const size_t n = cap < sizeof g_call_prof ? cap : sizeof g_call_prof; memcpy(dst, g_call_prof, n); return (int64_t)n; }
#endif
    Context* ctx = nullptr;
    { std::lock_guard<std::mutex> lk(g_ctx_mu); for (auto& kv : g_ctx) if (kv.second->ws.have_last) ctx = kv.second.get(); }
    if (!ctx) { set_err("no batch has run"); return LHIP_ERR_INTERNAL; }
    std::lock_guard<std::mutex> lk(ctx->mu);
    rt::set_device(ctx->device);
    const WorkSet& ws = ctx->ws;
    const Workspace& W = ws.lastW;
    const size_t GC = (size_t)W.ngslots * ws.lastC;
    const void* src = nullptr; size_t n = 0;
    switch (what) {
        case 0: src = W.xr; n = GC * 576 * 4; break;
        case 1: src = W.blocktype; n = GC * 4; break;
        case 2: src = W.E; n = (size_t)W.ngslots * ws.lastCp * E_STRIDE * 4; break;
        case 3: src = W.ath_adjust; n = (size_t)W.nfslots * 8; break;
        case 4: src = W.side; n = (size_t)W.nframes_total * 2 * ws.lastC * sizeof(GrSide); break;
        case 5: src = W.sb; n = GC * SB_STRIDE * 4; break;
        case 6: src = W.peaks; n = GC * PK_STRIDE * 4; break;
        case 7: src = W.prof; n = PROF_BYTES; break;
        case 8: src = W.nflagged; n = 256; break;
        default: set_err("unknown tap"); return LHIP_ERR_INTERNAL;
    }
    if (n > cap) n = cap;
    if (!rt::d2h(dst, src, n, ctx->stream) || !rt::sync(ctx->stream)) return LHIP_ERR_INTERNAL;
    return (int64_t)n;
}

int lhip_stream_info(const lhip_stream* s, lhip_stream_info_t* info) {
    if (!s || s->magic != 0x4c484950) { set_err("bad stream handle"); return LHIP_ERR_BAD_HANDLE; }
    if (!info) { set_err("lhip_stream_info: null argument"); return LHIP_ERR_INTERNAL; }
    if (!s->tag) { set_err("lhip_stream_info: the stream was not created with the infoTag option (its totals are not kept)"); return LHIP_ERR_INTERNAL; }
// ... 253 lines not shown
```

### lamejs_amd/csrc/lhip_kernels.h

```cpp
#pragma once
#define XCD_GRID(n) (8 * (((n) + 7) / 8))
static __device__ __forceinline__ int xcd_item(int b, int n) { const int it = (b & 7) * ((n + 7) >> 3) + (b >> 3); return it < n && (b >> 3) < ((n + 7) >> 3) ? it : -1; }
__global__ __launch_bounds__(64) void g_load(Tables T, Workspace W, const StreamDesc* SD, const StreamIO* IO) { kb_load(T, W, SD, IO, blockIdx.x, threadIdx.x); }
__global__ __launch_bounds__(64) void g_save(Tables T, Workspace W, const StreamDesc* SD, const StreamIO* IO) { kb_save(T, W, SD, IO, blockIdx.x, threadIdx.x); }
#ifndef LHIP_WPB
#define LHIP_WPB 4
#endif
enum { WPB = LHIP_WPB };
#define XCD_GRID_W(n) XCD_GRID(((n) + WPB - 1) / WPB)
static __device__ __forceinline__ int xcd_wave_item(int n, int* lane) {
    const int wv = __builtin_amdgcn_readfirstlane((int)(threadIdx.x >> 6));
    *lane = (int)(threadIdx.x & 63);
    const int g = xcd_item(blockIdx.x, (n + WPB - 1) / WPB);
    const int it = g * WPB + wv;
    return (g >= 0 && it < n) ? it : -1;
}
#define WAVE_LDS(TYPE, NAME) __shared__ TYPE NAME##_[WPB]; TYPE& NAME = NAME##_[__builtin_amdgcn_readfirstlane((int)(threadIdx.x >> 6))]
__global__ __launch_bounds__(64 * WPB) void g_psyA(Tables T, Workspace W, const StreamDesc* SD, const StreamIO* IO, int chn0, int nch) {
    WAVE_LDS(PsyALds, L);
    int lane;
    const int it = xcd_wave_item(W.ngslots * nch, &lane);
    if (it >= 0) kb_psyA(T, W, SD, IO, it / nch, chn0 + it % nch, lane, L);
}
__global__ __launch_bounds__(256) void g_prep(Tables T, Workspace W, const StreamDesc* SD, const StreamIO* IO, int nstreams) {
// ... 12 lines not shown
    int lane;
    const int it = xcd_wave_item(W.ngslots, &lane);
    if (it >= 0) kb_psyB<NCH>(T, pb, W, SD, it, lane, L, par);
}
__global__ __launch_bounds__(64, 4) void g_poly(Tables T, Workspace W, const StreamDesc* SD, const StreamIO* IO, int nitems) {
    __shared__ PolyLds L;
    const int it = xcd_item(blockIdx.x, (nitems + POLY_PER_WAVE - 1) / POLY_PER_WAVE);
    if (it >= 0) kb_polyphase(T, W, SD, IO, it, nitems, threadIdx.x, L);
}
__global__ __launch_bounds__(64) void g_mdct(Tables T, Workspace W, const StreamDesc* SD) {
    __shared__ MdctLds L;
    const int it = xcd_item(blockIdx.x, W.ngslots);
    if (it >= 0) kb_mdct(T, W, SD, it, threadIdx.x, L);
}
#ifdef LHIP_PHASE_PROF
enum { QWAVES = 7 };
#else
enum { QWAVES = 8 };
#endif
#ifndef LHIP_QOCC
#define LHIP_QOCC 4
#endif
LHIP_DEV int next_frame_slot(int32_t* ctr) {
    int v = 0;
    if ((threadIdx.x & 63) == 0) v = atomicAdd(ctr, 1);
    return __builtin_amdgcn_readfirstlane(v);
}
struct QArgs { Tables T; PowBase pb; Workspace W; const StreamDesc* SD; int chain, nfs, ctr; };
#ifdef LHIP_QVGPR
#define LHIP_QUANT_BOUNDS __attribute__((amdgpu_flat_work_group_size(1, 64 * QWAVES), amdgpu_waves_per_eu(LHIP_QOCC, 8), amdgpu_num_vgpr((LHIP_QVGPR) / 2)))
#else
#define LHIP_QUANT_BOUNDS __launch_bounds__(64 * QWAVES, LHIP_QOCC)
#endif
template <int RESV> __global__ LHIP_QUANT_BOUNDS void g_quant(QArgs a_unused) {
    __shared__ QuantTabs Q;
    __shared__ QuantLds L[QWAVES];
    __shared__ TailShare TS;
#ifndef LHIP_PHASE_PROF
    static_assert(QWAVES * sizeof(QuantLds) + sizeof(QuantTabs) + sizeof(TailShare) <= 80 * 1024, "g_quant: LDS budget for 2 workgroups per CU exceeded");
#endif
    const QArgs* A = (const QArgs*)__builtin_amdgcn_kernarg_segment_ptr();
    q_copy_tabs(A->T, Q, threadIdx.x, 64 * QWAVES);
    if (threadIdx.x == 0) TS.drawing = QWAVES;
    if (threadIdx.x < QWAVES) TS.offer[threadIdx.x].state = 0;
    const bool tail_help_on = !RESV && A->T.channels_out == 2;
    __syncthreads();
    const int wv = __builtin_amdgcn_readfirstlane(threadIdx.x >> 6);
#ifdef LHIP_PHASE_PROF
    L[wv].prof[threadIdx.x & 63] = 0;
#endif
#if defined(LHIP_PHASE_PROF) || defined(LHIP_WAVE_TIMES)
    const unsigned long long wave_t0_ = wall_clock64();
#endif
    int hint[3] = {-1, -1, -1};
    for (;;) {
        const int fslot = next_frame_slot(A->W.work_ctr + A->ctr);
        if (fslot >= A->nfs) break;
        if constexpr (!RESV) kb_quant_th(A->T, A->pb, A->W, A->SD, fslot, threadIdx.x & 63, L[wv], Q, hint, TS, wv);
        else kb_quant<0, RESV>(A->T, A->pb, A->W, A->SD, fslot, A->chain, threadIdx.x & 63, L[wv], Q, -1, nullptr, nullptr, nullptr);
        hint[0] = __builtin_amdgcn_readfirstlane(hint[0]); hint[1] = __builtin_amdgcn_readfirstlane(hint[1]); hint[2] = __builtin_amdgcn_readfirstlane(hint[2]);
    }
    if (tail_help_on) tail_help(A->T, A->pb, A->W, A->SD, threadIdx.x & 63, L, wv, QWAVES, Q, TS);
#ifdef LHIP_PHASE_PROF
    atomicAdd((unsigned long long*)A->W.prof + (threadIdx.x & 63), (unsigned long long)L[wv].prof[threadIdx.x & 63]);
#endif
#if defined(LHIP_PHASE_PROF) || defined(LHIP_WAVE_TIMES)
    {
        const int wid = blockIdx.x * QWAVES + wv;
        if ((threadIdx.x & 63) == 0 && wid < 8192) { A->W.prof[64 + 2 * wid] = wave_t0_; A->W.prof[64 + 2 * wid + 1] = wall_clock64(); }
    }
#endif
}
template <int RESV> __global__ __launch_bounds__(128, LHIP_QOCC) void g_quant_pair(QArgs a_unused) {
    __shared__ QuantTabs Q;
    __shared__ QuantLds L[2];
    __shared__ int mbox[4];
    const QArgs* A = (const QArgs*)__builtin_amdgcn_kernarg_segment_ptr();
    q_copy_tabs(A->T, Q, threadIdx.x, 128);
    __syncthreads();
    const int wv = __builtin_amdgcn_readfirstlane(threadIdx.x >> 6);
    kb_quant<1, RESV>(A->T, A->pb, A->W, A->SD, blockIdx.x, A->chain, threadIdx.x & 63, L[wv], Q, wv, mbox);
}
__global__ __launch_bounds__(256) void g_validate_fast(Tables T, Workspace W, const StreamDesc* SD, int nfs) {
    __shared__ ValidateShare S;
    const int t = blockIdx.x * 256 + threadIdx.x, fslot = t >> 2;
    kb_validate_fast_quad(T, W, SD, fslot < nfs ? fslot : 0, t & 3, fslot < nfs, S);
}
enum { FX_NFLAG = 0, FX_NSLOW = 1, FX_WORK_REPAIR = 2, FX_WORK_SLOW = 3, FX_PARITY_STRIDE = 8, FX_BAR = 24, FX_STATS = 32 };
LHIP_DEV void grid_barrier(int32_t* bar, int nblocks) {
    __syncthreads();
    if (nblocks > 1 && threadIdx.x == 0) {
        __builtin_amdgcn_fence(__ATOMIC_RELEASE, "agent");
        asm volatile("s_waitcnt vmcnt(0)" ::: "memory");
        const int gen = __hip_atomic_load(bar + 1, __ATOMIC_RELAXED, __HIP_MEMORY_SCOPE_AGENT);
        if (__hip_atomic_fetch_add(bar, 1, __ATOMIC_RELAXED, __HIP_MEMORY_SCOPE_AGENT) == nblocks - 1) {
            __hip_atomic_store(bar, 0, __ATOMIC_RELAXED, __HIP_MEMORY_SCOPE_AGENT);
            __builtin_amdgcn_fence(__ATOMIC_RELEASE, "agent");
            asm volatile("s_waitcnt vmcnt(0)" ::: "memory");
            __hip_atomic_fetch_add(bar + 1, 1, __ATOMIC_RELAXED, __HIP_MEMORY_SCOPE_AGENT);
        } else {
            for (int n = 0; __hip_atomic_load(bar + 1, __ATOMIC_RELAXED, __HIP_MEMORY_SCOPE_AGENT) == gen; n++) { if (n > (1 << 26)) __builtin_trap(); __builtin_amdgcn_s_sleep(4); }
        }
        __builtin_amdgcn_fence(__ATOMIC_ACQUIRE, "agent");
    }
    __syncthreads();
}
#ifndef LHIP_FIXUP_OCC
#define LHIP_FIXUP_OCC 4
#endif
__global__ __launch_bounds__(64 * QWAVES, LHIP_FIXUP_OCC) void g_fixup(QArgs a_unused) {
    __shared__ QuantTabs Q;
    __shared__ QuantLds L[QWAVES];
    const QArgs* A = (const QArgs*)__builtin_amdgcn_kernarg_segment_ptr();
    const int nfs = A->nfs, nblocks = gridDim.x, nthr = 64 * QWAVES;
    const int wv = __builtin_amdgcn_readfirstlane(threadIdx.x >> 6), lane = threadIdx.x & 63;
    int32_t* base = A->W.nflagged;
    bool tabs = false;
    int repaired = 0, iters = 0, failed = 0;
    for (int it = 0;; it++) {
        int32_t* ctr = base + FX_PARITY_STRIDE * (it & 1);
        Workspace W = A->W;
        W.nflagged = ctr;
        if (blockIdx.x == 0 && threadIdx.x < FX_PARITY_STRIDE) base[FX_PARITY_STRIDE * ((it + 1) & 1) + threadIdx.x] = 0;
        if (it > 0) {
            for (int f = blockIdx.x * nthr + threadIdx.x; f < nfs; f += nblocks * nthr) kb_validate_fast(A->T, W, A->SD, f, it);
            grid_barrier(base + FX_BAR, nblocks);
        }
        const int nslow = __builtin_amdgcn_readfirstlane(__hip_atomic_load(ctr + FX_NSLOW, __ATOMIC_RELAXED, __HIP_MEMORY_SCOPE_AGENT));
        const int gw = blockIdx.x * QWAVES + wv, nw = nblocks * QWAVES;
        if (nslow > 0) {
            if (!tabs) { q_copy_tabs(A->T, Q, threadIdx.x, nthr); __syncthreads(); tabs = true; }
            for (int i = gw; i < nslow; i += nw)
                kb_validate(A->T, A->pb, W, A->SD, __builtin_amdgcn_readfirstlane(W.slow_list[i]), lane, L[wv], Q);
            grid_barrier(base + FX_BAR, nblocks);
        }
        const int nflag = __builtin_amdgcn_readfirstlane(__hip_atomic_load(ctr + FX_NFLAG, __ATOMIC_RELAXED, __HIP_MEMORY_SCOPE_AGENT));
        if (nflag == 0) break;
        repaired += nflag; iters++;
        if (iters > nfs + 2) { failed = 1; break; }
        if (!tabs) { q_copy_tabs(A->T, Q, threadIdx.x, nthr); __syncthreads(); tabs = true; }
        for (int b0 = gw; b0 < nfs; b0 += 64 * nw) {
            int flagged = 0;
            const int f = b0 + nw * lane;
            if (f < nfs) {
                const StreamDesc* sd = A->SD + W.fslot_stream[f];
                const int k = f - sd->fslot0 - 1;
                if (k >= 0) flagged = W.seed_flag[sd->out_slot0 + k] == 1;
            }
            uint64_t m = __ballot(flagged);
            while (m) {
                const int l = (int)__builtin_ctzll(m);
                m &= m - 1;
                const int fr = b0 + nw * l;
                kb_quant(A->T, A->pb, W, A->SD, fr, 1, lane, L[wv], Q);
                if (lane == 0) {
                    const StreamDesc* sd = A->SD + W.fslot_stream[fr];
                    const int k = fr - sd->fslot0 - 1;
                    if (k + 1 < sd->nframes) W.reval[sd->out_slot0 + k + 1] = it + 1;
                }
            }
        }
        grid_barrier(base + FX_BAR, nblocks);
    }
    if (blockIdx.x == 0 && threadIdx.x == 0) { base[FX_STATS + 0] = repaired; base[FX_STATS + 1] = iters; base[FX_STATS + 2] = failed; }
}
__global__ __launch_bounds__(64) void g_bits(Tables T, Workspace W, const StreamDesc* SD) {
    __shared__ BitsLds L;
    kb_bits(T, W, SD, blockIdx.x, threadIdx.x, L);
}
__global__ __launch_bounds__(64) void g_resv_flush(Tables T, Workspace W, const StreamDesc* SD) {
    __shared__ BitsLds L;
    if (SD[blockIdx.x].flush) kb_resv_flush(T, W, blockIdx.x, threadIdx.x, L, W.io[blockIdx.x].state->rv, W.out_bytes + blockIdx.x);
}
__global__ __launch_bounds__(64) void g_out_crc(const CrcDesc* D, int nstreams, uint32_t* partial) {
    const int s = crc_find_stream(D, nstreams, (int)blockIdx.x);
    kb_out_crc(D, s, (int)blockIdx.x - D[s].part0, threadIdx.x, partial);
}
__global__ __launch_bounds__(64) void g_ingest(const IngestDesc* D, int nstreams, float limit, unsigned long long* ctr) {
    __shared__ __attribute__((aligned(16))) uint8_t L[ING_WINDOW];
    const int s = ingest_find_stream(D, nstreams, (int)blockIdx.x);
    const unsigned bad = kb_ingest(D, s, (int64_t)blockIdx.x - D[s].blk0, threadIdx.x, L, limit);
    if (ctr && bad && threadIdx.x == 0) atomicAdd(ctr, (unsigned long long)bad);
}
__global__ __launch_bounds__(GAIN_STAGE_NT) void g_gain_stage(Tables T, Workspace W, const StreamDesc* SD, const StreamIO* IO, const GainDesc* D, int nstreams) {
    const int s = gain_find_stream<true>(D, nstreams, (int)blockIdx.x);
    kb_gain_stage(T, W, SD, IO, D, s, (int64_t)((int)blockIdx.x - D[s].blk0) * GAIN_STAGE_NT + threadIdx.x);
}
// ... 112 lines not shown
```

### lamejs_amd/csrc/lhip_math.h

```cpp
#pragma once
#include "lhip_defs.h"

namespace lhip {

#ifdef LHIP_HOSTSIM
LHIP_DEV uint32_t d_hi(double x) { uint64_t u; memcpy(&u, &x, 8); return (uint32_t)(u >> 32); }
LHIP_DEV uint32_t d_lo(double x) { uint64_t u; memcpy(&u, &x, 8); return (uint32_t)u; }
LHIP_DEV double d_make(uint32_t hi, uint32_t lo) { uint64_t u = ((uint64_t)hi << 32) | lo; double x; memcpy(&x, &u, 8); return x; }
LHIP_DEV double d_sqrt(double x) { return sqrt(x); }
LHIP_DEV double d_abs(double x) { return fabs(x); }
#else
LHIP_DEV uint32_t d_hi(double x) { return (uint32_t)__double2hiint(x); }
LHIP_DEV uint32_t d_lo(double x) { return (uint32_t)__double2loint(x); }
LHIP_DEV double d_make(uint32_t hi, uint32_t lo) { return __hiloint2double((int)hi, (int)lo); }
LHIP_DEV double d_sqrt(double x) { return __builtin_sqrt(x); }
LHIP_DEV double d_abs(double x) { return __builtin_fabs(x); }
#endif
LHIP_DEV double d_with_hi(double x, uint32_t hi) { return d_make(hi, d_lo(x)); }
LHIP_DEV double d_trunc_lo(double x) { return d_make(d_hi(x), 0u); }

LHIP_DEV int32_t js_toint32(double d) {
    if (d >= -2147483648.0 && d <= 2147483647.0) return (int32_t)d;
    const uint32_t hi = d_hi(d), lo = d_lo(d);
    const int32_t e = (int32_t)((hi >> 20) & 0x7ffu);
// ... 57 lines not shown
        return dk * ln2_hi - ((hfsq - (s * (hfsq + R) + dk * ln2_lo)) - f);
    }
    if (k == 0) return f - s * (f - R);
    return dk * ln2_hi - ((s * (f - R) - dk * ln2_lo) - f);
}

LHIP_DEV double v8_log10(double x) {
    const double two54 = 1.80143985094819840000e+16, ivln10 = 4.34294481903251816668e-01,
                 log10_2hi = 3.01029995663611771306e-01, log10_2lo = 3.69423907715893078616e-13;
    int32_t hx = (int32_t)d_hi(x);
    uint32_t lx = d_lo(x);
    int32_t k = 0;
    if (hx < 0x00100000) {
        if (((hx & 0x7fffffff) | lx) == 0) return -two54 / 0.0;
        if (hx < 0) return (x - x) / 0.0;
        k -= 54;
        x *= two54;
        hx = (int32_t)d_hi(x);
    }
    if (hx >= 0x7ff00000) return x + x;
    k += (hx >> 20) - 1023;
    int32_t i = (int32_t)(((uint32_t)k & 0x80000000u) >> 31);
    hx = (hx & 0x000fffff) | ((0x3ff - i) << 20);
    double y = (double)(k + i);
    x = d_with_hi(x, (uint32_t)hx);
    double z = y * log10_2lo + ivln10 * v8_log(x);
    return z + y * log10_2hi;
}

template <int N> LHIP_DEV void q_floor_prod(const float (&xa)[N], const float (&xb)[N], float istep, int (&ra)[N], int (&rb)[N]) {
#ifdef LHIP_HOSTSIM
    for (int j = 0; j < N; j++) { ra[j] = (int)((double)xa[j] * (double)istep); rb[j] = (int)((double)xb[j] * (double)istep); }
#else
    static_assert(N == 5, "device form is written for 5 pairs per lane");
    float a0, a1, a2, a3, a4, b0, b1, b2, b3, b4;
    asm volatile("s_setreg_imm32_b32 hwreg(HW_REG_MODE, 0, 2), 3\n\ts_nop 1\n\t"
                 "v_mul_f32 %0, %10, %20\n\tv_mul_f32 %1, %11, %20\n\tv_mul_f32 %2, %12, %20\n\tv_mul_f32 %3, %13, %20\n\tv_mul_f32 %4, %14, %20\n\t"
                 "v_mul_f32 %5, %15, %20\n\tv_mul_f32 %6, %16, %20\n\tv_mul_f32 %7, %17, %20\n\tv_mul_f32 %8, %18, %20\n\tv_mul_f32 %9, %19, %20\n\t"
                 "s_setreg_imm32_b32 hwreg(HW_REG_MODE, 0, 2), 0\n\ts_nop 1"
                 : "=&v"(a0), "=&v"(a1), "=&v"(a2), "=&v"(a3), "=&v"(a4), "=&v"(b0), "=&v"(b1), "=&v"(b2), "=&v"(b3), "=&v"(b4)
                 : "v"(xa[0]), "v"(xa[1]), "v"(xa[2]), "v"(xa[3]), "v"(xa[4]), "v"(xb[0]), "v"(xb[1]), "v"(xb[2]), "v"(xb[3]), "v"(xb[4]), "v"(istep));
    ra[0] = (int)a0; ra[1] = (int)a1; ra[2] = (int)a2; ra[3] = (int)a3; ra[4] = (int)a4;
    rb[0] = (int)b0; rb[1] = (int)b1; rb[2] = (int)b2; rb[3] = (int)b3; rb[4] = (int)b4;
#endif
}
template <int N> LHIP_DEV void q_floor_fma(const float (&xa)[N], const float (&xb)[N], float istep, const float (&ja)[N], const float (&jb)[N],
                                           int (&va)[N], int (&vb)[N]) {
#ifdef LHIP_HOSTSIM
    for (int j = 0; j < N; j++) {
        va[j] = (int)((double)xa[j] * (double)istep + (double)ja[j]);
        vb[j] = (int)((double)xb[j] * (double)istep + (double)jb[j]);
    }
#else
    static_assert(N == 5, "device form is written for 5 pairs per lane");
    float a0, a1, a2, a3, a4, b0, b1, b2, b3, b4;
    asm volatile("s_setreg_imm32_b32 hwreg(HW_REG_MODE, 0, 2), 3\n\ts_nop 1\n\t"
                 "v_fma_f32 %0, %10, %20, %21\n\tv_fma_f32 %1, %11, %20, %22\n\tv_fma_f32 %2, %12, %20, %23\n\tv_fma_f32 %3, %13, %20, %24\n\tv_fma_f32 %4, %14, %20, %25\n\t"
                 "v_fma_f32 %5, %15, %20, %26\n\tv_fma_f32 %6, %16, %20, %27\n\tv_fma_f32 %7, %17, %20, %28\n\tv_fma_f32 %8, %18, %20, %29\n\tv_fma_f32 %9, %19, %20, %30\n\t"
                 "s_setreg_imm32_b32 hwreg(HW_REG_MODE, 0, 2), 0\n\ts_nop 1"
                 : "=&v"(a0), "=&v"(a1), "=&v"(a2), "=&v"(a3), "=&v"(a4), "=&v"(b0), "=&v"(b1), "=&v"(b2), "=&v"(b3), "=&v"(b4)
                 : "v"(xa[0]), "v"(xa[1]), "v"(xa[2]), "v"(xa[3]), "v"(xa[4]), "v"(xb[0]), "v"(xb[1]), "v"(xb[2]), "v"(xb[3]), "v"(xb[4]), "v"(istep),
                   "v"(ja[0]), "v"(ja[1]), "v"(ja[2]), "v"(ja[3]), "v"(ja[4]), "v"(jb[0]), "v"(jb[1]), "v"(jb[2]), "v"(jb[3]), "v"(jb[4]));
    va[0] = (int)a0; va[1] = (int)a1; va[2] = (int)a2; va[3] = (int)a3; va[4] = (int)a4;
    vb[0] = (int)b0; vb[1] = (int)b1; vb[2] = (int)b2; vb[3] = (int)b3; vb[4] = (int)b4;
#endif
}

LHIP_DEV double v8_log10_pos(double x) {
    const double ivln10 = 4.34294481903251816668e-01, log10_2hi = 3.01029995663611771306e-01, log10_2lo = 3.69423907715893078616e-13;
    const double ln2_hi = 6.93147180369123816490e-01, ln2_lo = 1.90821492927058770002e-10;
    const double Lg1 = 6.666666666666735130e-01, Lg2 = 3.999999999940941908e-01, Lg3 = 2.857142874366239149e-01,
                 Lg4 = 2.222219843214978396e-01, Lg5 = 1.818357216161805012e-01, Lg6 = 1.531383769920937332e-01,
                 Lg7 = 1.479819860511658591e-01;
    int32_t hx = (int32_t)d_hi(x);
    const bool infnan = hx >= 0x7ff00000;
    const int32_t k10 = (hx >> 20) - 1023;
    const int32_t i10 = (int32_t)(((uint32_t)k10 & 0x80000000u) >> 31);
    const double y = (double)(k10 + i10);
    hx = (hx & 0x000fffff) | ((0x3ff - i10) << 20);
    int32_t k = (hx >> 20) - 1023;
    hx &= 0x000fffff;
    const int32_t i = (hx + 0x95f64) & 0x100000;
    const double xm = d_make((uint32_t)(hx | (i ^ 0x3ff00000)), d_lo(x));
    k += (i >> 20);
    const double f = xm - 1.0;
    const bool small = (0x000fffff & (2 + hx)) < 3;
    const double s = f / (2.0 + f);
    const double dk = (double)k;
    const double z = s * s;
    const int32_t i2 = (hx - 0x6147a) | (0x6b851 - hx);
    const double w = z * z;
    const double t1 = w * (Lg2 + w * (Lg4 + w * Lg6));
    const double t2 = z * (Lg1 + w * (Lg3 + w * (Lg5 + w * Lg7)));
    const double R = t2 + t1;
    const double ff = f * f;
    const double hfsq = 0.5 * ff;
    const double Rs = ff * (0.5 - 0.33333333333333333 * f);
// ... 189 lines not shown
```

### lamejs_amd/csrc/lhip_pipeline_hip.h

```cpp
#pragma once
static inline bool g_kt_on_() { return g_kt_on; }
static_assert(FX_STATS_OFF == FX_STATS * 4, "counter block layout");
static bool collect_kernel_times(void* st) { if (g_kt_on) { if (!rt::sync(st)) return false; kt_collect(); } return true; }
static bool collect_repair_stats(Context* ctx, BatchPlan& P, bool fetch_fx, const int32_t* fx) {
    g_stat_pending = nullptr;
    if (fetch_fx) {
        P.repaired = fx[0]; P.iters = fx[1];
        if (fx[2]) { set_err("seed-chain repair did not converge"); return false; }
    } else if (P.nfr > 0) g_stat_pending = ctx;
    return true;
}
static bool run_pipeline(Context* ctx, BatchPlan& P) {
    const TableSet& ts = *P.ts; const Tables& T = ts.T; Workspace& W = P.W; const std::vector<StreamDesc>& sd = P.sd;
    const StreamDesc* dSD = P.dSD; const StreamIO* dIO = P.dIO;
    const int S = P.S, C = T.channels_out, ngs = P.ngs, nfs = P.nfs, nfr = P.nfr; const bool resv = P.resv, use_frame = P.use_frame;
    WorkSet& ws = ctx->ws; void* st = ctx->stream; const int64_t in_total = P.in_total;
    if (P.count_rej) {
        if (!ws.rejected.ensure(64) || !rt::dzero(ws.rejected.p, 8, st)) return false;
        int64_t nb = (in_total + 255) / 256;
        if (nb > 2048) nb = 2048;
        if (nb < 1) nb = 1;
        if (P.count_f32) LAUNCHB(KT_COUNT, g_count_rejected, (int)nb, 256, st, dIO, S, T.channels_in, T.pcm_limit, (unsigned long long*)ws.rejected.p);
        g_rej_pending = ctx;
    }
// ... 30 lines not shown
            hipStream_t a; hipEvent_t e1, e2;
            if (hipStreamCreateWithFlags(&a, hipStreamNonBlocking) == hipSuccess && hipEventCreateWithFlags(&e1, hipEventDisableTiming) == hipSuccess &&
                hipEventCreateWithFlags(&e2, hipEventDisableTiming) == hipSuccess) { ws.aux_stream = a; ws.ev_fork = e1; ws.ev_join = e2; }
        }
        if (ws.aux_stream && hipEventRecord((hipEvent_t)ws.ev_fork, (hipStream_t)st) == hipSuccess &&
            hipStreamWaitEvent((hipStream_t)ws.aux_stream, (hipEvent_t)ws.ev_fork, 0) == hipSuccess) {
            LAUNCHB(KT_SCAN, g_scan_ath, S, ATH_NT, ws.aux_stream, T, W, dSD);
            aux_guard.aux = ws.aux_stream;
            HIPCK(hipEventRecord((hipEvent_t)ws.ev_join, (hipStream_t)ws.aux_stream));
            forked = true;
        }
    }
    if (!forked) LAUNCHB(KT_SCAN, g_scan_ath, S, ATH_NT, st, T, W, dSD);
    LAUNCH(KT_POLY, g_poly, XCD_GRID((ngs * C + POLY_PER_WAVE - 1) / POLY_PER_WAVE), st, T, W, dSD, dIO, ngs * C);
    LAUNCH(KT_MDCT, g_mdct, XCD_GRID(ngs), st, T, W, dSD);
    if (forked) { HIPCK(hipStreamWaitEvent((hipStream_t)st, (hipEvent_t)ws.ev_join, 0)); aux_guard.aux = nullptr; }
    if (resv) {
        QArgs qa; qa.T = T; qa.pb = ts.pb10; qa.W = W; qa.SD = dSD; qa.chain = 2; qa.nfs = nfs; qa.ctr = S <= ctx->num_cus ? 1 : 0;
        P.paths |= qa.ctr ? LHIP_PATH_RESV_STREAM_HELPERS : LHIP_PATH_RESV_STREAM_NOHELPERS;
        LAUNCHB(KT_QUANT, g_resv_stream, S, 64 * RS_WAVES, st, qa);
    } else {
    if (T.psy_channels == 4) LAUNCHB(KT_PSYB, g_psyB<4>, XCD_GRID_W(ngs), 64 * WPB, st, T, ts.pb10, W, dSD, -1);
    else LAUNCHB(KT_PSYB, g_psyB<2>, XCD_GRID_W(ngs), 64 * WPB, st, T, ts.pb10, W, dSD, -1);
    int qgrid = (nfs + QWAVES - 1) / QWAVES;
    if (qgrid > ctx->num_cus * 2) qgrid = ctx->num_cus * 2;
#ifdef LHIP_PHASE_PROF
    const bool pair = false;
#else
    static const int pair_max = []() { const char* e = getenv("LAMEJS_HIP_PAIR_MAX_FRAMES"); return e ? atoi(e) : -1; }();
    const bool pair = (C == 2 && nfs <= (pair_max >= 0 ? pair_max : 6 * ctx->num_cus));
#endif
    P.paths |= pair ? LHIP_PATH_QUANT_PAIR : LHIP_PATH_QUANT_PERSISTENT;
    { QArgs qa; qa.T = T; qa.pb = ts.pb10; qa.W = W; qa.SD = dSD; qa.chain = 0; qa.nfs = nfs; qa.ctr = 0;
      if (pair) LAUNCHB(KT_QUANT, g_quant_pair<0>, nfs, 128, st, qa); else LAUNCHB(KT_QUANT, g_quant<0>, qgrid, 64 * QWAVES, st, qa); }
    if (nfr > 0) {
        QArgs qa; qa.T = T; qa.pb = ts.pb10; qa.W = W; qa.SD = dSD; qa.chain = 1; qa.nfs = nfs; qa.ctr = 0;
        LAUNCHB(KT_VALIDATE, g_validate_fast, (nfs + 63) / 64, 256, st, T, W, dSD, nfs);
        int fgrid = (nfs + 63) / 64;
        if (ctx->fixup_wg_per_cu == 0) {
            int nb = 0;
            if (hipOccupancyMaxActiveBlocksPerMultiprocessor(&nb, (const void*)g_fixup, 64 * QWAVES, 0) != hipSuccess || nb < 1) nb = 1;
            ctx->fixup_wg_per_cu = nb < LHIP_FIXUP_OCC / 2 ? nb : LHIP_FIXUP_OCC / 2;
        }
        if (fgrid > ctx->num_cus * ctx->fixup_wg_per_cu) fgrid = ctx->num_cus * ctx->fixup_wg_per_cu;
        if (fgrid < 1) fgrid = 1;
        P.paths |= fgrid == 1 ? LHIP_PATH_FIXUP_SINGLE : LHIP_PATH_FIXUP_COOP;
        if (fgrid == 1) LAUNCHB(KT_VALIDATE, g_fixup, 1, 64 * QWAVES, st, qa);
        else {
            kt_begin(KT_VALIDATE, st);
            void* kargs[] = {(void*)&qa};
            hipStream_t cst = (hipStream_t)st;
            if (ctx->own_stream) {
                if (!ctx->ev_coop[0]) { if (!rt::event_create(&ctx->ev_coop[0]) || !rt::event_create(&ctx->ev_coop[1])) return false; }
                if (!rt::event_record(ctx->ev_coop[0], st) || !rt::stream_wait_event(nullptr, ctx->ev_coop[0])) return false;
                cst = nullptr;
            }
            hipError_t e_ = hipLaunchCooperativeKernel((const void*)g_fixup, dim3(fgrid), dim3(64 * QWAVES), kargs, 0, cst);
            if (ctx->own_stream && e_ == hipSuccess) { if (!rt::event_record(ctx->ev_coop[1], nullptr) || !rt::stream_wait_event(st, ctx->ev_coop[1])) return false; }
            kt_end(st);
            TRACE_SYNC(g_fixup_cooperative, st);
            if (e_ != hipSuccess) { set_err(std::string("g_fixup (cooperative launch): ") + hipGetErrorString(e_)); return false; }
        }
    }
    LAUNCH(KT_BITS, g_bits, nfs, st, T, W, dSD);
    }
    LAUNCH(KT_SAVE, g_save, S, st, T, W, dSD, dIO);
    }
    if (P.crc_mode == 2) {
        P.paths |= LHIP_PATH_OUT_CRC;
        LAUNCH(KT_OUT_CRC, g_out_crc, P.crc_parts, st, (const CrcDesc*)ws.crc_desc.p, S, (uint32_t*)ws.crc_part.p);
        LAUNCH(KT_OUT_CRC, g_out_crc_fold, S, st, (const CrcDesc*)ws.crc_desc.p, (const uint32_t*)ws.crc_part.p, P.crc_dst);
    }
    if (P.gain.stage_blocks > 0) {
        P.paths |= LHIP_PATH_GAIN;
        LAUNCHB(KT_GAIN_STAGE, g_gain_stage, P.gain.stage_blocks, GAIN_STAGE_NT, st, T, W, dSD, dIO, P.dGD, S);
        if (C == 2) LAUNCH(KT_GAIN, g_gain<2>, P.gain.waves, st, P.dGD, S); else LAUNCH(KT_GAIN, g_gain<1>, P.gain.waves, st, P.dGD, S);
    }
    return true;
}
```

### lamejs_amd/csrc/lhip_pipeline_sim.h

```cpp
#pragma once
#ifdef LHIP_WAVESIM
#define WAVE_RUN(...) wsim::run([&](int lane_) { __VA_ARGS__; })
#else
#define WAVE_RUN(...) do { const int lane_ = 0; __VA_ARGS__; } while (0)
#endif
#ifdef LHIP_WAVESIM
#define QUANT_RUN(chain_) do { if (pair) wsim::run_block(2, [&](int wave_, int lane_) { kb_quant<1, 0>(T, ts.pb10, W, dSD, b, chain_, lane_, LQ2[wave_], QT, wave_, mbox); }); \
                       else WAVE_RUN(kb_quant<0, 0>(T, ts.pb10, W, dSD, b, chain_, lane_, LQ, QT)); } while (0)
#else
#define QUANT_RUN(chain_) WAVE_RUN(kb_quant<0, 0>(T, ts.pb10, W, dSD, b, chain_, lane_, LQ, QT))
#endif
static void gain_sim_run(const Tables& T, const Workspace& W, const StreamDesc* SD, const StreamIO* IO, const GainDesc* D, int S, int stage_blocks, int waves) {
    static thread_local float LG[LHIP_NL * 2 * GAIN_STRIDE];
    for (int b = 0; b < stage_blocks; b++) { const int s = gain_find_stream<true>(D, S, b); for (int t = 0; t < GAIN_STAGE_NT; t++) kb_gain_stage(T, W, SD, IO, D, s, (int64_t)(b - D[s].blk0) * GAIN_STAGE_NT + t); }
    for (int b = 0; b < waves; b++) {
        const int s = gain_find_stream<false>(D, S, b);
        if (D[s].channels == 2) WAVE_RUN(kb_gain<2>(D, s, b - D[s].wave0, lane_, LG)); else WAVE_RUN(kb_gain<1>(D, s, b - D[s].wave0, lane_, LG));
    }
}
static inline bool g_kt_on_() { return false; }
static bool collect_kernel_times(void*) { return true; }
static bool collect_repair_stats(Context*, BatchPlan&, bool, const int32_t*) { return true; }
static bool run_pipeline(Context* ctx, BatchPlan& P) {
    const TableSet& ts = *P.ts; const Tables& T = ts.T; Workspace& W = P.W; const std::vector<StreamDesc>& sd = P.sd;
    const StreamDesc* dSD = P.dSD; const StreamIO* dIO = P.dIO;
    const int S = P.S, C = T.channels_out, ngs = P.ngs, nfs = P.nfs, nfr = P.nfr; const bool resv = P.resv, use_frame = P.use_frame;
    int64_t& repaired = P.repaired; int64_t& iters = P.iters;
    if (P.count_f32) g_rejected = (int64_t)kb_count_rejected(dIO, S, T.channels_in, T.pcm_limit, 0, 1);
    if (P.ingest_tiles > 0) {
        P.paths |= LHIP_PATH_INGEST;
        alignas(16) static thread_local uint8_t LI[ING_WINDOW];
        unsigned long long bad = 0;
        for (int b = 0; b < P.ingest_tiles; b++) { const int s = ingest_find_stream(P.dING, S, b); WAVE_RUN(const unsigned r = kb_ingest(P.dING, s, (int64_t)b - P.dING[s].blk0, lane_, LI, T.pcm_limit); if (lane_ == 0) bad += r); }
        if (P.count_rej) g_rejected += (int64_t)bad;
    }
    static thread_local PsyALds LA; static thread_local PsyBLds4 LB; static thread_local MdctLds LM; static thread_local PolyLds LP; static thread_local QuantLds LQ; static thread_local BitsLds LBi; static thread_local QuantTabs QT;
    q_load_tabs(T, QT, 0, 1);
    if (use_frame) {
        P.paths |= resv ? LHIP_PATH_FRAME_RESV : LHIP_PATH_FRAME;
        const int NW = FR_WAVES;
        alignas(16) static thread_local unsigned char UL[FR_WAVES][FR_LDS_PER_WAVE]; static thread_local int fmbox[12]; static thread_local CountShare fcs[2];
        for (int s = 0; s < S; s++) {
            fcs[0].state = CS_IDLE; fcs[1].state = CS_IDLE;
// ... 50 lines not shown
                    for (int stage = 0; stage < RS_STAGES; stage++) { kb_resv_stage<1>(stage, T, ts.pb10, W, dSD, s, k, F, wave_, lane_, RU[wave_], QT, rmbox, RV, &nout, rcs); wg_barrier(); }
                if (wave_ == 3 && sd[s].flush) kb_resv_flush(T, W, s, lane_, *(BitsLds*)RU[3], RV, &nout);
            });
#else
            for (int k = 0; k <= F; k++)
                for (int stage = 0; stage < RS_STAGES; stage++)
                    for (int wv = 0; wv < RS_WAVES; wv++) kb_resv_stage<0>(stage, T, ts.pb10, W, dSD, s, k, F, wv, 0, RU[wv], QT, rmbox, RV, &nout);
            if (sd[s].flush) kb_resv_flush(T, W, s, 0, *(BitsLds*)RU[3], RV, &nout);
#endif
            dIO[s].state->rv = RV;
            W.out_bytes[s] = nout;
        }
    } else {
#ifdef LHIP_WAVESIM
    static thread_local QuantLds LQ2[2]; static thread_local int mbox[4];
    static const int pair_max = []() { const char* e = getenv("LAMEJS_HIP_PAIR_MAX_FRAMES"); return e ? atoi(e) : 12; }();
    const bool pair = (C == 2 && nfs <= pair_max);
    P.paths |= pair ? LHIP_PATH_QUANT_PAIR : LHIP_PATH_QUANT_PERSISTENT;
#else
    P.paths |= LHIP_PATH_QUANT_PERSISTENT;
#endif
#if defined(LHIP_WAVESIM)
    if (!pair) {
        static thread_local QuantLds LQ8[8]; static thread_local TailShare TS;
        int ctr = 0;
        TS.drawing = 8; for (int w = 0; w < 8; w++) TS.offer[w].state = 0;
        wsim::run_block(8, [&](int wave_, int lane_) {
            int hint[3] = {-1, -1, -1};
            for (;;) {
                int f = 0;
                if (lane_ == 0) f = ctr++;
                f = wave_bcast(f, 0);
                if (f >= nfs) break;
                kb_quant_th(T, ts.pb10, W, dSD, f, lane_, LQ8[wave_], QT, hint, TS, wave_);
            }
            if (C == 2) tail_help(T, ts.pb10, W, dSD, lane_, LQ8, wave_, 8, QT, TS);
        });
    } else
#endif
    {
        int hints[3][3] = {{-1, -1, -1}, {-1, -1, -1}, {-1, -1, -1}};
        for (int b = 0; b < nfs; b++) {
#ifdef LHIP_WAVESIM
            if (pair) { QUANT_RUN(0); continue; }
            int hl[64][3];
            for (int l = 0; l < 64; l++) for (int q = 0; q < 3; q++) hl[l][q] = hints[b % 3][q];
            WAVE_RUN(kb_quant<0, 0>(T, ts.pb10, W, dSD, b, 0, lane_, LQ, QT, -1, nullptr, nullptr, hl[lane_]));
            for (int l = 1; l < 64; l++) for (int q = 0; q < 3; q++) if (hl[l][q] != hl[0][q]) { set_err("wavesim: seed hint not wave-uniform"); return false; }
            for (int q = 0; q < 3; q++) hints[b % 3][q] = hl[0][q];
#else
            WAVE_RUN(kb_quant<0, 0>(T, ts.pb10, W, dSD, b, 0, lane_, LQ, QT, -1, nullptr, nullptr, hints[b % 3]));
#endif
        }
    }
    for (;;) {
        W.nflagged[0] = 0; W.nflagged[1] = 0;
        for (int b = 0; b < nfs; b++) kb_validate_fast(T, W, dSD, b);
        for (int i = 0; i < W.nflagged[1]; i++) WAVE_RUN(kb_validate(T, ts.pb10, W, dSD, W.slow_list[i], lane_, LQ, QT));
        const int nf = W.nflagged[0];
        if (nf == 0) break;
        repaired += nf; iters++;
        for (int b = 0; b < nfs; b++) QUANT_RUN(1);
        if (iters > nfr + 2) { set_err("seed-chain repair did not converge"); return false; }
    }
    for (int b = 0; b < nfs; b++) WAVE_RUN(kb_bits(T, W, dSD, b, lane_, LBi));
    }
    for (int s = 0; s < S; s++) WAVE_RUN(kb_save(T, W, dSD, dIO, s, lane_));
    }
    if (P.crc_mode == 2) {
        P.paths |= LHIP_PATH_OUT_CRC;
        const CrcDesc* D = (const CrcDesc*)ctx->ws.crc_desc.p; uint32_t* part = (uint32_t*)ctx->ws.crc_part.p;
        for (int b = 0; b < P.crc_parts; b++) { const int s = crc_find_stream(D, S, b); WAVE_RUN(kb_out_crc(D, s, b - D[s].part0, lane_, part)); }
        for (int s = 0; s < S; s++) WAVE_RUN(kb_crc_fold(D, s, lane_, part, P.crc_dst));
    }
    if (P.gain.stage_blocks > 0) {
        P.paths |= LHIP_PATH_GAIN;
        gain_sim_run(T, W, dSD, dIO, P.dGD, S, P.gain.stage_blocks, P.gain.waves);
    }
    return true;
}
#undef QUANT_RUN
#undef WAVE_RUN
```

### lamejs_amd/csrc/lhip_tables.h

```cpp
#pragma once
struct lhtb_entry { char name[32]; uint32_t dtype, count, offset, pad; };

struct TableSet {
    Tables T;
    PowBase pb10;
    std::vector<uint8_t> blob;
    void* d_blob = nullptr;
    void* d_extra = nullptr;
    void* d_qtabs = nullptr;
    int device = 0;
    int base_frame_bytes = 0;
    bool bad_option = false;
    InfoTagCfg tag;
    int gain_on = 0;
    ~TableSet() { rt::dfree(d_blob); rt::dfree(d_extra); rt::dfree(d_qtabs); }
};

static const lhtb_entry* find_entry(const uint8_t* b, const char* name) {
    uint32_t n; memcpy(&n, b + 8, 4);
    const lhtb_entry* e = (const lhtb_entry*)(b + 16);
    for (uint32_t i = 0; i < n; i++) if (strncmp(e[i].name, name, 32) == 0) return &e[i];
    return nullptr;
}

static bool parse_blob(TableSet& ts, const void* blob, size_t nbytes, void* stream) {
    if (nbytes < 16) { set_err("tables blob too small"); return false; }
    uint32_t magic, total;
    memcpy(&magic, blob, 4); memcpy(&total, (const uint8_t*)blob + 12, 4);
    if (magic != 0x4254484cu || total > nbytes) { set_err("tables blob: bad magic/size"); return false; }
    ts.blob.assign((const uint8_t*)blob, (const uint8_t*)blob + total);
    const uint8_t* b = ts.blob.data();
    ts.d_blob = rt::dmalloc(total);
    if (!ts.d_blob) { set_err("hipMalloc(tables) failed"); return false; }
    if (!rt::h2d(ts.d_blob, b, total, stream)) return false;
    Tables& T = ts.T;
    memset(&T, 0, sizeof T);
    bool ok = true;
    auto arr = [&](const char* name, uint32_t dtype, int* count) -> const void* {
        const lhtb_entry* e = find_entry(b, name);
        if (!e || e->dtype != dtype) { set_err(std::string("tables blob: entry missing: ") + name); ok = false; return nullptr; }
        if (count) *count = (int)e->count;
        return (const uint8_t*)ts.d_blob + e->offset;
    };
    auto host_arr = [&](const char* name) -> const void* { const lhtb_entry* e = find_entry(b, name); return e ? b + e->offset : nullptr; };
    bool optional = false;
    auto named = [&](const char* names_key, const char* key) -> int {
// ... 139 lines not shown
    auto host_arr = [&](const char* name) -> const void* { const lhtb_entry* e = find_entry(b, name); return e ? b + e->offset : nullptr; };
    const int32_t* h_s3ind = (const int32_t*)host_arr("s3ind");
    const int32_t* h_s3ind_s = (const int32_t*)host_arr("s3ind_s");
    const int32_t* h_nl = (const int32_t*)host_arr("numlines_l");
    const int32_t* h_ns = (const int32_t*)host_arr("numlines_s");
    const int32_t* h_bo_l = (const int32_t*)host_arr("bo_l");
    const int32_t* h_bo_s = (const int32_t*)host_arr("bo_s");
    std::vector<int32_t> extra(4 * CBANDS, 0);
    int k = 0, j = 0;
    for (int p = 0; p < T.npart_l; p++) { extra[p] = k; k += h_s3ind[2 * p + 1] - h_s3ind[2 * p] + 1; extra[2 * CBANDS + p] = j; j += h_nl[p]; }
    if (j != HBLKSIZE) { set_err("long partitions do not cover 513 lines"); return false; }
    T.n_s3_ll = k;
    if (k > PSYB_S3_LDS) { set_err("configuration outside the supported envelope (spreading table larger than g_psyB's LDS copy)"); return false; }
    k = 0; j = 0;
    for (int p = 0; p < T.npart_s; p++) { extra[CBANDS + p] = k; k += h_s3ind_s[2 * p + 1] - h_s3ind_s[2 * p] + 1; extra[3 * CBANDS + p] = j; j += h_ns[p]; }
    if (j != HBLKSIZE_s) { set_err("short partitions do not cover 129 lines"); return false; }
    auto walk = [&](const int32_t* bo, int nb, int npart, int32_t* stop) {
        int b = 0, sb = 0;
        for (; sb < nb; ++b, ++sb) {
            const int lim = bo[sb] < npart ? bo[sb] : npart;
            if (b < lim) b = lim;
            stop[sb] = b;
            if (b >= npart) { ++sb; break; }
        }
        for (; sb < nb; ++sb) stop[sb] = npart;
    };
    extra.resize(4 * CBANDS + SBMAX_l + SBMAX_s);
    walk(h_bo_l, SBMAX_l, T.npart_l, extra.data() + 4 * CBANDS);
    walk(h_bo_s, SBMAX_s, T.npart_s, extra.data() + 4 * CBANDS + SBMAX_l);
    const size_t amp_at = (extra.size() + 1) & ~(size_t)1;
    extra.resize(amp_at + 64);
    {
        const float* h_af = (const float*)host_arr("amp_filter");
        const int32_t* h_order = (const int32_t*)host_arr("mdct_order");
        double amp[32];
        for (int i = 0; i < 32; i++) amp[i] = 1.0;
        T.amp_mask = 0;
        for (int band = 0; band < 32; band++) {
            const double af = (double)h_af[band];
            const int ob = h_order[band];
            if (ob < 0 || ob > 31) { set_err("mdct_order is not a permutation of 0..31"); return false; }
            if (!(af < 1e-12) && af < 1.0) { amp[ob] = af; T.amp_mask |= 1 << ob; }
        }
        memcpy(extra.data() + amp_at, amp, sizeof amp);
    }
    const size_t fold_at = extra.size();
    extra.resize(fold_at + 128 + 24 + 40 + 289);
    {
        const int32_t* h_sl = (const int32_t*)host_arr("sfb_l");
        const int32_t* h_ss = (const int32_t*)host_arr("sfb_s");
        std::vector<int> band_l(576), band_s(576);
        for (int d = 0, sfb = 0; d < 576; d++) { while (sfb < SBMAX_l - 1 && h_sl[sfb + 1] <= d) sfb++; band_l[d] = sfb; }
        for (int d = 0, sfb = 0; d < 576; d++) {
            while (sfb < SBMAX_s - 1 && 3 * h_ss[sfb + 1] <= d) sfb++;
            const int st = h_ss[sfb], w = h_ss[sfb + 1] - st;
            band_s[d] = 3 * sfb + (w > 0 ? (d - 3 * st) / w : 0);
        }
        for (int sh = 0; sh < 2; sh++) {
            const std::vector<int>& b = sh ? band_s : band_l;
            for (int ln = 0; ln < 64; ln++) {
                uint32_t m = 0;
                for (int kk = 0; kk < 9; kk++) {
                    const int jj = 9 * ln + kk;
                    if (jj == 0 || b[jj - 1] != b[jj]) m |= 1u << kk;
                    if (jj == 575 || b[jj + 1] != b[jj]) m |= 1u << (16 + kk);
                }
// ... 73 lines not shown
```

Measured before the change: 2.293 million frames/s.

## Specialize quantize loops to skip zero spectral tail when lowpass zeroes top bands

Adds a tail0 flag per granule, set when all coefficients at index 512 and above are zero, and a SKIP template parameter that, when the lowpass filter zeroes subbands 28-31, runs quantize, bit counting and amplify over only the first 256 pairs. This cuts per-iteration VALU and LDS work in the inner rate loop. The host picks the kernel variant from the amp_filter table. The FMA asm also gains a narrower 4-wide variant. It adds template instantiations, which raises code size and may change register allocation.

```diff
diff --git a/lamejs_amd/csrc/k_quant.h b/lamejs_amd/csrc/k_quant.h
--- a/lamejs_amd/csrc/k_quant.h
+++ b/lamejs_amd/csrc/k_quant.h
@@ -14,6 +14,7 @@
     int part2_length, sfb_lmax, sfb_smin, psy_lmax, sfbmax, psymax, sfbdivide;
     int count1bits, max_nonzero_coeff;
     int firstcut;
+    int tail0;
 };
 
 struct NoiseRes { double max_noise; int over_count, over_SSD, bits; };
@@ -27,7 +28,7 @@
     g.region0_count = uni(g.region0_count); g.region1_count = uni(g.region1_count); g.preflag = uni(g.preflag); g.scalefac_scale = uni(g.scalefac_scale);
     g.count1table_select = uni(g.count1table_select); g.part2_length = uni(g.part2_length); g.sfb_lmax = uni(g.sfb_lmax); g.sfb_smin = uni(g.sfb_smin);
     g.psy_lmax = uni(g.psy_lmax); g.sfbmax = uni(g.sfbmax); g.psymax = uni(g.psymax); g.sfbdivide = uni(g.sfbdivide);
-    g.count1bits = uni(g.count1bits); g.max_nonzero_coeff = uni(g.max_nonzero_coeff); g.firstcut = uni(g.firstcut);
+    g.count1bits = uni(g.count1bits); g.max_nonzero_coeff = uni(g.max_nonzero_coeff); g.firstcut = uni(g.firstcut); g.tail0 = uni(g.tail0);
 }
 
 #if defined(LHIP_PHASE_PROF) && !defined(LHIP_HOSTSIM)
@@ -290,7 +291,7 @@
     g.part2_length = 0; g.sfb_lmax = SBPSY_l; g.sfb_smin = SBPSY_s;
     g.psy_lmax = T.sfb21_extra ? SBMAX_l : SBPSY_l;
     g.psymax = g.psy_lmax; g.sfbmax = g.sfb_lmax; g.sfbdivide = 11;
-    g.count1bits = 0; g.max_nonzero_coeff = 575; g.xrpow_max = 0; g.firstcut = 64;
+    g.count1bits = 0; g.max_nonzero_coeff = 575; g.xrpow_max = 0; g.firstcut = 64; g.tail0 = 0;
     int nsfb;
     if (block_type == SHORT_TYPE) {
         g.sfb_smin = 0; g.sfb_lmax = 0;
@@ -419,8 +420,14 @@
     wave_sync();
 }
 
+LHIP_DEV int q_tail_is_zero(int lane, const QuantLds& L) {
+    int nz = 0;
+    for (int k = 512 + lane; k < 576; k += LHIP_NL) if (!((double)L.xr[k] == 0)) nz = 1;
+    return !wave_any(nz);
+}
+
 LHIP_DEV void q_calc_xmin(const Tables& T, double ath_adjust, double masking_lower, const float* ratio ,
-                          GI& g, int lane, QuantLds& L, const QuantTabs& Q) {
+                          GI& g, int lane, QuantLds& L, const QuantTabs& Q, const int want_tail0 = 0) {
     lane = fresh_lane(lane);
     {
         double tq[NLN_FOLD];
@@ -448,6 +455,7 @@
         for (int k = lane; k < 576; k += LHIP_NL) if (!((double)L.xr[k] == 0)) t = k;
         t = wave_max(t);
         g.max_nonzero_coeff = (t >= 575) ? 575 : t + 1;
+        if (want_tail0) g.tail0 = t < 512;
     } else {
         LHIP_LANE_ONCE(sfb, 0, SBPSY_s) {
             const double tmpATH = ath_adjust * (double)T.ATH_s[sfb];
@@ -471,23 +479,33 @@
             L.rxmin[3 * sfb] = recip_for_div((double)px[0]); L.rxmin[3 * sfb + 1] = recip_for_div((double)px[1]); L.rxmin[3 * sfb + 2] = recip_for_div((double)px[2]);
         }
         g.max_nonzero_coeff = 575;
+        if (want_tail0) g.tail0 = q_tail_is_zero(lane, L);
     }
     q_set_firstcut(g, lane, L);
     wave_sync();
 }
 
 enum { NPL = (288 + LHIP_NL - 1) / LHIP_NL };
+enum { NPL_HEAD = 256 / LHIP_NL };
+#if defined(LHIP_HOSTSIM)
+struct RoundStats { long head = 0, full = 0; };
+inline RoundStats& round_stats() { static RoundStats t; return t; }
+#define LHIP_ROUND_COUNT(f) do { if (lane == 0) __atomic_fetch_add(&round_stats().f, 1L, __ATOMIC_RELAXED); } while (0)
+#else
+#define LHIP_ROUND_COUNT(f) do { } while (0)
+#endif
+template <int NR>
 LHIP_DEV void q_quantize(const Tables& T, const GI& g, const int32_t* scalefac, int16_t* ix, int use_prev,
-                         int pn_gain, int pn_sfb_count1, int (&vx)[NPL], int (&vy)[NPL], int lane, QuantLds& L, const QuantTabs& Q) {
+                         int pn_gain, int pn_sfb_count1, int (&vx)[NR], int (&vy)[NR], int lane, QuantLds& L, const QuantTabs& Q) {
     lane = fresh_lane(lane);
     const double istep = ipow20(Q, g.global_gain);
     const int may_big = !(g.xrpow_max * istep < (double)QT_N);
     const int sfbmax = (g.block_type == SHORT_TYPE) ? 38 : 21;
     const int prev_data_use = use_prev && (g.global_gain == pn_gain);
     unsigned long long tm_ = PH_NOW(); (void)tm_;
-    float xa[NPL], xb[NPL];
-#pragma unroll
-    for (int j = 0; j < NPL; j++) {
+    float xa[NR], xb[NR];
+#pragma unroll
+    for (int j = 0; j < NR; j++) {
         const int p = 2 * (lane + LHIP_NL * j);
         xa[j] = 0.f; xb[j] = 0.f;
         if (p < 576) { struct F2 { float x, y; }; const F2 xx = *(const F2*)(L.xrpow + p); xa[j] = xx.x; xb[j] = xx.y; }
@@ -510,17 +528,17 @@
     const uint8_t* l2s = line2sfb(Q, g.block_type);
     const int need_old = (m_cached != 0);
     const float istep_f = Q.ipow20[g.global_gain];
-    int ra[NPL], rb[NPL];
+    int ra[NR], rb[NR];
     q_floor_prod(xa, xb, istep_f, ra, rb);
-    float aa[NPL], ab[NPL];
+    float aa[NR], ab[NR];
     if (!may_big) {
 #pragma unroll
-        for (int j = 0; j < NPL; j++) { aa[j] = Q.adj43[ra[j]]; ab[j] = Q.adj43[rb[j]]; }
+        for (int j = 0; j < NR; j++) { aa[j] = Q.adj43[ra[j]]; ab[j] = Q.adj43[rb[j]]; }
     } else {
 #pragma unroll
-        for (int j = 0; j < NPL; j++) { aa[j] = Q.adj43[ra[j] < QT_N ? ra[j] : QT_N - 1]; ab[j] = Q.adj43[rb[j] < QT_N ? rb[j] : QT_N - 1]; }
-#pragma unroll
-        for (int j = 0; j < NPL; j++) {
+        for (int j = 0; j < NR; j++) { aa[j] = Q.adj43[ra[j] < QT_N ? ra[j] : QT_N - 1]; ab[j] = Q.adj43[rb[j] < QT_N ? rb[j] : QT_N - 1]; }
+#pragma unroll
+        for (int j = 0; j < NR; j++) {
             if (ra[j] >= QT_N) aa[j] = T.adj43[ra[j]];
             if (rb[j] >= QT_N) ab[j] = T.adj43[rb[j]];
         }
@@ -528,13 +546,13 @@
     q_floor_fma(xa, xb, istep_f, aa, ab, vx, vy);
     if (!need_old && m_zo == 0) {
 #pragma unroll
-        for (int j = 0; j < NPL; j++) {
+        for (int j = 0; j < NR; j++) {
             const int p = 2 * (lane + LHIP_NL * j);
             if (p < 576) *(uint32_t*)(ix + p) = (uint32_t)vx[j] | ((uint32_t)vy[j] << 16);
         }
     } else if (m_zo == 0) {
 #pragma unroll
-        for (int j = 0; j < NPL; j++) {
+        for (int j = 0; j < NR; j++) {
             const int p = 2 * (lane + LHIP_NL * j);
             int sf = 0; uint32_t oldw = 0;
             if (p < 576) { sf = l2s[p]; oldw = *(const uint32_t*)(ix + p); }
@@ -548,7 +566,7 @@
         float zo_thr = (float)compareval0;
         if ((double)zo_thr < compareval0) zo_thr = f32_next_up(zo_thr);
 #pragma unroll
-        for (int j = 0; j < NPL; j++) {
+        for (int j = 0; j < NR; j++) {
             const int p = 2 * (lane + LHIP_NL * j);
             int sf = 0; uint32_t oldw = 0;
             if (p < 576) { sf = l2s[p]; if (need_old) oldw = *(const uint32_t*)(ix + p); }
@@ -674,7 +692,8 @@
     return state & ~15;
 }
 
-LHIP_DEV int q_noquant_count_bits(const Tables& T, GI& g, const int16_t* ix, int (&vx)[NPL], int (&vy)[NPL], int use_prev, int* pn_sfb_count1, int* asg_mask, int lane, QuantLds& L, const QuantTabs& Q) {
+template <int NR>
+LHIP_DEV int q_noquant_count_bits(const Tables& T, GI& g, const int16_t* ix, int (&vx)[NR], int (&vy)[NR], int use_prev, int* pn_sfb_count1, int* asg_mask, int lane, QuantLds& L, const QuantTabs& Q) {
     *asg_mask = 0;
     lane = fresh_lane(lane);
     unsigned long long tm_ = PH_NOW(); (void)tm_;
@@ -685,7 +704,7 @@
 #if LHIP_NL == 1
     {
         int top = 0;
-        for (int j = 0; j < NPL; j++) if ((vx[j] | vy[j]) != 0) top = 2 * (lane + LHIP_NL * j) + 2;
+        for (int j = 0; j < NR; j++) if ((vx[j] | vy[j]) != 0) top = 2 * (lane + LHIP_NL * j) + 2;
         i = top;
         const int nq = i >> 2;
         firstbig = nq;
@@ -698,7 +717,7 @@
     {
         int tp = -1, bp = -1;
 #pragma unroll
-        for (int j = 0; j < NPL; j++) {
+        for (int j = 0; j < NR; j++) {
             const uint64_t nz = wave_ballot((vx[j] | vy[j]) != 0), bg = wave_ballot((vx[j] | vy[j]) > 1);
             if (nz) tp = 64 * j + 63 - (int)__builtin_clzll(nz);
             if (bg) bp = 64 * j + 63 - (int)__builtin_clzll(bg);
@@ -747,9 +766,9 @@
     if (a2 > i) a2 = i;
     *asg_mask = (g.block_type != SHORT_TYPE ? 8 : 0) | (use2 ? 4 : 0) | (0 < a1 ? 1 : 0) | (a1 < a2 ? 2 : 0);
     int m0 = 0, m1 = 0, m2 = 0;
-    int rj[NPL];
-#pragma unroll
-    for (int j = 0; j < NPL; j++) {
+    int rj[NR];
+#pragma unroll
+    for (int j = 0; j < NR; j++) {
         rj[j] = 3;
         if (2 * LHIP_NL * j >= i) continue;
         const int p = 2 * (lane + LHIP_NL * j);
@@ -792,7 +811,7 @@
     const int any_esc = (m0 > 15) | (m1 > 15) | (m2 > 15);
 #if LHIP_NL == 1
 #pragma unroll
-    for (int j = 0; j < NPL; j++) {
+    for (int j = 0; j < NR; j++) {
         const int p = 2 * (lane + LHIP_NL * j);
         if (p < i) {
             const int r = (p >= a1) + (p >= a2);
@@ -811,7 +830,7 @@
 #else
     if (any_esc) {
 #pragma unroll
-        for (int j = 0; j < NPL; j++) {
+        for (int j = 0; j < NR; j++) {
             if (rj[j] < 3) {
                 const int r = rj[j];
                 const uint64_t d = *(const uint64_t*)L.rdesc[r];
@@ -827,7 +846,7 @@
         }
     } else {
 #pragma unroll
-        for (int j = 0; j < NPL; j++) {
+        for (int j = 0; j < NR; j++) {
             if (rj[j] < 3) {
                 const int r = rj[j];
                 const uint64_t d = *(const uint64_t*)L.rdesc[r];
@@ -881,6 +900,7 @@
 
 struct PrevNoise { int gain, sfb_count1; };
 
+template <int NR>
 LHIP_DEV int q_count_bits(const Tables& T, GI& g, const int32_t* scalefac, int16_t* ix, int use_pn, PrevNoise& pn, int* asg, int lane, QuantLds& L, const QuantTabs& Q) {
     *asg = 0;
     {
@@ -890,16 +910,24 @@
             if (g.xrpow_max > w) return LARGE_BITS;
         }
     }
-    int vx[NPL], vy[NPL];
-    { PH_BEGIN(); q_quantize(T, g, scalefac, ix, use_pn, use_pn ? pn.gain : 0, use_pn ? pn.sfb_count1 : 0, vx, vy, lane, L, Q); PH_END(L, PH_QUANTIZE); }
+    int vx[NR], vy[NR];
+    { PH_BEGIN(); q_quantize<NR>(T, g, scalefac, ix, use_pn, use_pn ? pn.gain : 0, use_pn ? pn.sfb_count1 : 0, vx, vy, lane, L, Q); PH_END(L, PH_QUANTIZE); }
     int cnt1 = pn.sfb_count1;
     PH_BEGIN();
     int amask = 0;
-    const int r = q_noquant_count_bits(T, g, ix, vx, vy, use_pn, &cnt1, &amask, lane, L, Q);
+    const int r = q_noquant_count_bits<NR>(T, g, ix, vx, vy, use_pn, &cnt1, &amask, lane, L, Q);
     *asg = pack_cond_fields(g, amask);
     if (use_pn) pn.sfb_count1 = cnt1;
     PH_END(L, PH_COUNT);
     return r;
+}
+template <int SKIP>
+LHIP_DEV int q_count_bits_rounds(const Tables& T, GI& g, const int32_t* scalefac, int16_t* ix, int use_pn, PrevNoise& pn, int* asg, int lane, QuantLds& L, const QuantTabs& Q) {
+    if constexpr (SKIP != 0) {
+        if (g.tail0) { LHIP_ROUND_COUNT(head); return q_count_bits<NPL_HEAD>(T, g, scalefac, ix, use_pn, pn, asg, lane, L, Q); }
+    }
+    LHIP_ROUND_COUNT(full);
+    return q_count_bits<NPL>(T, g, scalefac, ix, use_pn, pn, asg, lane, L, Q);
 }
 
 struct NoiseCommit { int fresh, step, cls; float dist; double x; };
@@ -1154,7 +1182,7 @@
 #ifdef LHIP_PHASE_PROF
         const unsigned long long hp_start_ = __builtin_amdgcn_s_memtime();
 #endif
-        const int bits = uni(q_noquant_count_bits(T, g, Lo.ixw, vx, vy, 1, &cnt1, &amask, lane, L, Q));
+        const int bits = uni(q_noquant_count_bits<NPL>(T, g, Lo.ixw, vx, vy, 1, &cnt1, &amask, lane, L, Q));
 #ifdef LHIP_PHASE_PROF
         const unsigned long long hp_end_ = __builtin_amdgcn_s_memtime();
 #endif
@@ -1189,7 +1217,7 @@
     }
     {
         int vx[NPL], vy[NPL];
-        PH_BEGIN(); q_quantize(T, g, scalefac, ix, 1, pn.gain, pn.sfb_count1, vx, vy, lane, L, Q); PH_END(L, PH_QUANTIZE);
+        PH_BEGIN(); q_quantize<NPL>(T, g, scalefac, ix, 1, pn.gain, pn.sfb_count1, vx, vy, lane, L, Q); PH_END(L, PH_QUANTIZE);
         (void)vx; (void)vy;
     }
 #ifdef LHIP_PHASE_PROF
@@ -1307,20 +1335,21 @@
     return !wave_any(z);
 }
 
-LHIP_DEV void q_amplify_flagged(GI& g, double amp, uint64_t m_amp, int lane, QuantLds& L, const QuantTabs& Q) {
+template <int NR>
+LHIP_DEV void q_amplify_rounds(GI& g, double amp, uint64_t m_amp, int lane, QuantLds& L, const QuantTabs& Q) {
     lane = fresh_lane(lane);
     float m = 0.f;
     const uint8_t* l2s = line2sfb(Q, g.block_type);
     struct F2 { float x, y; };
-    F2 xx[NPL]; int bnd[NPL];
-#pragma unroll
-    for (int j = 0; j < NPL; j++) {
+    F2 xx[NR]; int bnd[NR];
+#pragma unroll
+    for (int j = 0; j < NR; j++) {
         const int p = 2 * (lane + LHIP_NL * j);
         xx[j].x = 0.f; xx[j].y = 0.f; bnd[j] = 0;
         if (p < 576) { xx[j] = *(const F2*)(L.xrpow + p); bnd[j] = l2s[p]; }
     }
 #pragma unroll
-    for (int j = 0; j < NPL; j++) {
+    for (int j = 0; j < NR; j++) {
         const int p = 2 * (lane + LHIP_NL * j);
         const double a = ((m_amp >> bnd[j]) & 1) ? amp : 1.0;
         xx[j].x = (float)((double)xx[j].x * a); xx[j].y = (float)((double)xx[j].y * a);
@@ -1331,7 +1360,15 @@
     if ((double)m > g.xrpow_max) g.xrpow_max = m;
     wave_sync();
 }
-
+template <int SKIP>
+LHIP_DEV void q_amplify_flagged(GI& g, double amp, uint64_t m_amp, int lane, QuantLds& L, const QuantTabs& Q) {
+    if constexpr (SKIP != 0) {
+        if (g.tail0) { q_amplify_rounds<NPL_HEAD>(g, amp, m_amp, lane, L, Q); return; }
+    }
+    q_amplify_rounds<NPL>(g, amp, m_amp, lane, L, Q);
+}
+
+template <int SKIP>
 LHIP_DEV void q_amp_scalefac_bands(const Tables& T, GI& g, int32_t* scalefac, int* all_nonzero, int* pre_bad, int* m12_out,
                                    int lane, QuantLds& L, const QuantTabs& Q) {
     lane = fresh_lane(lane);
@@ -1371,7 +1408,7 @@
         const int r = wave_or(m12 | (z << 16) | (bad << 17));
         *m12_out = r & 0xffff; *all_nonzero = !((r >> 16) & 1); *pre_bad = (r >> 17) & 1;
     }
-    { unsigned long long tt_ = PH_NOW(); (void)tt_; q_amplify_flagged(g, ifqstep34, m_amp, lane, L, Q); PH_MARKB(L, PH_B_TRIG, tt_); }
+    { unsigned long long tt_ = PH_NOW(); (void)tt_; q_amplify_flagged<SKIP>(g, ifqstep34, m_amp, lane, L, Q); PH_MARKB(L, PH_B_TRIG, tt_); }
 }
 
 LHIP_DEV int q_scale_bitcount_from(const QuantTabs& Q, GI& g, int32_t* scalefac, int pre_bad, int m12, int lane) {
@@ -1398,6 +1435,7 @@
     return g.part2_length == LARGE_BITS;
 }
 
+template <int SKIP>
 LHIP_DEV void q_inc_scalefac_scale(const Tables& T, GI& g, int32_t* scalefac, int lane, QuantLds& L, const QuantTabs& Q) {
     lane = fresh_lane(lane);
     uint64_t m_amp = 0;
@@ -1411,7 +1449,7 @@
     wave_sync();
     g.preflag = 0;
     g.scalefac_scale = 1;
-    q_amplify_flagged(g, 1.29683955465100964055, m_amp, lane, L, Q);
+    q_amplify_flagged<SKIP>(g, 1.29683955465100964055, m_amp, lane, L, Q);
 }
 
 LHIP_DEV int q_inc_subblock_gain(const Tables& T, GI& g, int32_t* scalefac, int lane, QuantLds& L, const QuantTabs& Q) {
@@ -1459,11 +1497,12 @@
     return 0;
 }
 
+template <int SKIP>
 LHIP_DEV int q_balance_noise(const Tables& T, GI& g, int32_t* scalefac, int lane, QuantLds& L, const QuantTabs& Q) {
     lane = fresh_lane(lane);
     unsigned long long tb_ = PH_NOW(); (void)tb_;
     int all_nonzero, pre_bad, m12;
-    q_amp_scalefac_bands(T, g, scalefac, &all_nonzero, &pre_bad, &m12, lane, L, Q);
+    q_amp_scalefac_bands<SKIP>(T, g, scalefac, &all_nonzero, &pre_bad, &m12, lane, L, Q);
     PH_MARKB(L, PH_B_AMP, tb_);
     int status = all_nonzero;
     if (status) return 0;
@@ -1472,7 +1511,7 @@
     if (!status) return 1;
     if (T.noise_shaping > 1) {
         if (0 == g.scalefac_scale) {
-            q_inc_scalefac_scale(T, g, scalefac, lane, L, Q);
+            q_inc_scalefac_scale<SKIP>(T, g, scalefac, lane, L, Q);
             status = 0;
         } else if (g.block_type == SHORT_TYPE && T.subblock_gain > 0) {
             status = (q_inc_subblock_gain(T, g, scalefac, lane, L, Q) || q_loop_break(g, scalefac, lane, L, Q));
@@ -1537,6 +1576,7 @@
 #else
 #define LHIP_SS(...) do { } while (0)
 #endif
+template <int SKIP = 0>
 LHIP_DEV void q_outer_loop(const Tables& T, GI& g, int targ_bits, int bs_start, int bs_step, int* bs_gain_out,
                            int16_t* kept, GrSide* rec, uint32_t* dig, int64_t dn, int lane, QuantLds& L, const QuantTabs& Q, CountShare* cs = nullptr) {
     lane = fresh_lane(lane);
@@ -1573,7 +1613,7 @@
         if (cs != nullptr && st >= ST_A) nBits = q_count_bits_piped(T, w, L.sfw, L.ixw, pn, &asg, *cs, &ni, &nc, best.over_count == 0, &spec, lane, L, Q);
         else
 #endif
-        nBits = q_count_bits(T, w, L.sfw, L.ixw, st >= ST_A, pn, &asg, lane, L, Q);
+        nBits = q_count_bits_rounds<SKIP>(T, w, L.sfw, L.ixw, st >= ST_A, pn, &asg, lane, L, Q);
         LHIP_SS(ss_.evals++; if (st == ST_BS) ss_nbs++; else if (st == ST_BSUP) ss_nup++;
                 if (st >= ST_A && ss_run > 0) { ss_.run_steps++; if (ss_moved) ss_.run_steps_cnt1_moved++; if (cnt1_seen > 0) ss_.run_steps_zo++; });
         if (st <= ST_BSUP && nbs < BS_TAB_MAX) { if (lane == 0) { L.memo.bs_tab[nbs] = (w.global_gain << 24) | nBits; L.memo.bs_asg[nbs] = asg; } nbs++; }
@@ -1661,7 +1701,7 @@
         if (!first && !((w.global_gain + w.scalefac_scale) < 255)) break;
         first = 0;
         int bal_;
-        { PH_BEGIN(); bal_ = q_balance_noise(T, w, L.sfw, lane, L, Q); PH_END(L, PH_BALANCE); }
+        { PH_BEGIN(); bal_ = q_balance_noise<SKIP>(T, w, L.sfw, lane, L, Q); PH_END(L, PH_BALANCE); }
         if (!bal_) break;
         maxggain = (w.scalefac_scale != 0) ? 254 : 255;
         huff_bits = targ_bits - w.part2_length;
@@ -2126,11 +2166,15 @@
 }
 
 struct UnitOut { int bits; Seed next; int block_type; int active; };
+template <int SKIP = 0>
 LHIP_DEV UnitOut q_unit(const Tables& T, const PowBase& pb10, const Workspace& W, int C, int Cp, int fidx, int gslot, int gr, int ch, int mode_ext,
                         double ath_adjust, int targ_ch, Seed used, int gr0_bt, int lane, QuantLds& L, const QuantTabs& Q, CountShare* cs = nullptr) {
     lane = lane_anew(lane);
     UnitOut u; u.next = used;
     GI g;
+#if defined(LHIP_HOSTSIM)
+    if (SKIP) { for (int i = 256 + lane; i < 288; i += LHIP_NL) ((uint32_t*)L.ixw)[i] = 0x1fff1fffu; wave_sync(); }
+#endif
     const int bt = W.blocktype[(int64_t)gslot * C + ch];
     const double masking_lower = (bt != SHORT_TYPE) ? T.masking_lower_long : T.masking_lower_short;
     const float* ratio = W.E + ((int64_t)(gslot - 1) * Cp + ch + mode_ext) * E_STRIDE;
@@ -2138,9 +2182,12 @@
     int active = 0, bs_gain = 0;
     if (q_init_xrpow(g, lane, L, Q)) {
         active = 1;
-        { PH_BEGIN(); q_calc_xmin(T, ath_adjust, masking_lower, ratio, g, lane, L, Q); PH_END(L, PH_XMIN); }
+        { PH_BEGIN(); q_calc_xmin(T, ath_adjust, masking_lower, ratio, g, lane, L, Q, SKIP); PH_END(L, PH_XMIN); }
+        if constexpr (SKIP != 0) {
+            if (g.tail0) { for (int i = 256 + lane; i < 288; i += LHIP_NL) ((uint32_t*)L.ixw)[i] = 0u; wave_sync(); }
+        }
         int16_t* kept = cs ? cs->kept : W.l3 + (((int64_t)fidx * 2 + gr) * C + ch) * 576;
-        { PH_BEGIN(); q_outer_loop(T, g, targ_ch, used.start, used.step, &bs_gain, kept, W.side + ((int64_t)fidx * 2 + gr) * C + ch, W.vdig + ((int64_t)fidx * 2 + gr) * C + ch, W.vdig_n, lane, L, Q, cs); PH_END(L, PH_XRPOW); }
+        { PH_BEGIN(); q_outer_loop<SKIP>(T, g, targ_ch, used.start, used.step, &bs_gain, kept, W.side + ((int64_t)fidx * 2 + gr) * C + ch, W.vdig + ((int64_t)fidx * 2 + gr) * C + ch, W.vdig_n, lane, L, Q, cs); PH_END(L, PH_XRPOW); }
         uni_gi(g); bs_gain = uni(bs_gain);
         lane = lane_anew(lane);
         wave_sync();
@@ -2185,7 +2232,7 @@
         out->active = active; out->bs_start = used.start; out->bs_step_in = used.step; out->bs_gain = bs_gain;
         W.vdig[((int64_t)fidx * 2 + gr) * C + ch] = vd_head(active, used.start, used.step, bs_gain);
         out->targ_bits = targ_ch;
-        out->mode_ext = mode_ext;
+        out->mode_ext = uni_here(mode_ext);
         out->scfsi = scfsi[0] | (scfsi[1] << 1) | (scfsi[2] << 2) | (scfsi[3] << 3);
     }
     LHIP_LANE_ONCE(i, 0, SFBMAX) out->scalefac[i] = L.sfb[i];
@@ -2200,7 +2247,7 @@
     return u;
 }
 
-template <int PAIR = 0, int RESV = 0>
+template <int PAIR = 0, int RESV = 0, int SKIP = 0>
 LHIP_DEV void kb_quant(const Tables& T, const PowBase& pb10, const Workspace& W, const StreamDesc* SD, int fslot,
                        int chain, int lane, QuantLds& L, const QuantTabs& Q, int my_ch = -1, int* mbox = nullptr, const ResvState* rvp = nullptr,
                        int* hint = nullptr, CountShare* cs = nullptr, const int* later_granules_ready = nullptr) {
@@ -2278,8 +2325,8 @@
         const int targ0 = uni(targ[0]), targ1 = uni(targ[1]);
         for (int ch = 0; ch < C; ch++) {
             if (PAIR && ch != my_ch) continue;
-            const UnitOut u = q_unit(T, pb10, W, C, Cp, fidx, gslot, gr, ch, mode_ext, ath_adjust, ch == 0 ? targ0 : targ1, ch == 0 ? seed0 : seed1,
-                                     ch == 0 ? gr0_bt0 : gr0_bt1, lane, L, Q, cs);
+            const UnitOut u = q_unit<SKIP>(T, pb10, W, C, Cp, fidx, gslot, gr, ch, mode_ext, ath_adjust, ch == 0 ? targ0 : targ1, ch == 0 ? seed0 : seed1,
+                                           ch == 0 ? gr0_bt0 : gr0_bt1, lane, L, Q, cs);
             if (u.active) { if (ch == 0) seed0 = u.next; else seed1 = u.next; }
             if (!PAIR) ResvSize = uni(ResvSize - u.bits);
             else if (lane == 0) mbox[2 * gr + ch] = u.bits;
@@ -2320,6 +2367,7 @@
 #endif
 }
 
+template <int SKIP>
 LHIP_DEV void kb_validate(const Tables& T, const PowBase& pb10, const Workspace& W, const StreamDesc* SD, int fslot,
                           int lane, QuantLds& L, const QuantTabs& Q) {
     const int C = T.channels_out;
@@ -2376,12 +2424,13 @@
                             for (int i = lane; i < 576; i += LHIP_NL) if (!((double)L.xr[i] == 0)) t = i;
                             t = wave_max(t);
                             g.max_nonzero_coeff = (t >= 575) ? 575 : t + 1;
-                        }
+                            if (SKIP) g.tail0 = t < 512;
+                        } else if (SKIP) g.tail0 = q_tail_is_zero(lane, L);
                         q_set_firstcut(g, lane, L);
                         inited = 1;
                     }
                     g.global_gain = gain;
-                    nBits = q_count_bits(T, g, L.sfb, L.ixw, 0, pn_none, &asg, lane, L, Q);
+                    nBits = q_count_bits_rounds<SKIP>(T, g, L.sfb, L.ixw, 0, pn_none, &asg, lane, L, Q);
                 }
                 nBits = uni(nBits);
                 cstate = apply_cond_fields(cstate, uni(asg));
diff --git a/lamejs_amd/csrc/k_quant_tail.h b/lamejs_amd/csrc/k_quant_tail.h
--- a/lamejs_amd/csrc/k_quant_tail.h
+++ b/lamejs_amd/csrc/k_quant_tail.h
@@ -12,6 +12,7 @@
 #define LHIP_TAIL_COUNT(f) do { } while (0)
 #endif
 
+template <int SKIP>
 LHIP_DEV void kb_quant_th(const Tables& T, const PowBase& pb10, const Workspace& W, const StreamDesc* SD, int fslot, int lane, QuantLds& L,
                           const QuantTabs& Q, int* hint, TailShare& TS, int wv) {
     lane = lane_anew(lane);
@@ -70,8 +71,8 @@
                 continue;
             }
             if (ch == 1) LHIP_TAIL_COUNT(withdrawn);
-            const UnitOut u = q_unit(T, pb10, W, C, Cp, fidx, gslot, gr, ch, mode_ext, ath_adjust, ch == 0 ? targ0 : targ1, ch == 0 ? seed0 : seed1,
-                                     ch == 0 ? gr0_bt0 : gr0_bt1, lane, L, Q);
+            const UnitOut u = q_unit<SKIP>(T, pb10, W, C, Cp, fidx, gslot, gr, ch, mode_ext, ath_adjust, ch == 0 ? targ0 : targ1, ch == 0 ? seed0 : seed1,
+                                        ch == 0 ? gr0_bt0 : gr0_bt1, lane, L, Q);
             if (u.active) { if (ch == 0) seed0 = u.next; else seed1 = u.next; }
             ResvSize = uni(ResvSize - u.bits);
             if (gr == 0) { if (ch == 0) gr0_bt0 = u.block_type; else gr0_bt1 = u.block_type; }
@@ -83,6 +84,7 @@
 #endif
 }
 
+template <int SKIP>
 LHIP_DEV void tail_help(const Tables& T, const PowBase& pb10, const Workspace& W, const StreamDesc* SD, int lane, QuantLds* Lall, int wv, int nwaves,
                         const QuantTabs& Q, TailShare& TS) {
     lane = lane_anew(lane);
@@ -110,7 +112,7 @@
             q_ath_pseudo(T, pb10, ath_adjust, lane, L, Q);
             if (gr == 1) { LHIP_LANE_ONCE(i, 0, (SFBMAX) + 1) L.sf_gr0[1][i] = Lall[w].sf_gr0[1][i]; }
             wave_sync();
-            const UnitOut u = q_unit(T, pb10, W, C, Cp, fidx, gslot, gr, 1, mode_ext, ath_adjust, targ, seed, gr0_bt, lane, L, Q);
+            const UnitOut u = q_unit<SKIP>(T, pb10, W, C, Cp, fidx, gslot, gr, 1, mode_ext, ath_adjust, targ, seed, gr0_bt, lane, L, Q);
             if (gr == 0) { LHIP_LANE_ONCE(i, 0, (SFBMAX) + 1) Lall[w].sf_gr0[1][i] = L.sf_gr0[1][i]; }
             if (lane == 0) { o.bits = u.bits; o.active = u.active; o.next_start = u.next.start; o.next_step = u.next.step; o.block_type = u.block_type; }
             wg_store(&o.state, 3, lane);
diff --git a/lamejs_amd/csrc/lhip_api.cpp b/lamejs_amd/csrc/lhip_api.cpp
--- a/lamejs_amd/csrc/lhip_api.cpp
+++ b/lamejs_amd/csrc/lhip_api.cpp
@@ -630,6 +630,12 @@
 }
 
 int64_t lhip_debug_read(int what, void* dst, size_t cap) {
+#ifdef LHIP_HOSTSIM
+    if (what == 10) {
+        const int64_t v[2] = {(int64_t)__atomic_load_n(&round_stats().head, __ATOMIC_RELAXED), (int64_t)__atomic_load_n(&round_stats().full, __ATOMIC_RELAXED)};
+        const size_t n = cap < sizeof v ? cap : sizeof v; memcpy(dst, v, n); return (int64_t)n;
+    }
+#endif
 #ifdef LHIP_PHASE_PROF
     if (what == 9) { const size_t n = cap < sizeof g_call_prof ? cap : sizeof g_call_prof; memcpy(dst, g_call_prof, n); return (int64_t)n; }
 #endif
diff --git a/lamejs_amd/csrc/lhip_kernels.h b/lamejs_amd/csrc/lhip_kernels.h
--- a/lamejs_amd/csrc/lhip_kernels.h
+++ b/lamejs_amd/csrc/lhip_kernels.h
@@ -68,7 +68,7 @@
 #else
 #define LHIP_QUANT_BOUNDS __launch_bounds__(64 * QWAVES, LHIP_QOCC)
 #endif
-template <int RESV> __global__ LHIP_QUANT_BOUNDS void g_quant(QArgs a_unused) {
+template <int RESV, int SKIP> __global__ LHIP_QUANT_BOUNDS void g_quant(QArgs a_unused) {
     __shared__ QuantTabs Q;
     __shared__ QuantLds L[QWAVES];
     __shared__ TailShare TS;
@@ -92,11 +92,11 @@
     for (;;) {
         const int fslot = next_frame_slot(A->W.work_ctr + A->ctr);
         if (fslot >= A->nfs) break;
-        if constexpr (!RESV) kb_quant_th(A->T, A->pb, A->W, A->SD, fslot, threadIdx.x & 63, L[wv], Q, hint, TS, wv);
-        else kb_quant<0, RESV>(A->T, A->pb, A->W, A->SD, fslot, A->chain, threadIdx.x & 63, L[wv], Q, -1, nullptr, nullptr, nullptr);
+        if constexpr (!RESV) kb_quant_th<SKIP>(A->T, A->pb, A->W, A->SD, fslot, threadIdx.x & 63, L[wv], Q, hint, TS, wv);
+        else kb_quant<0, RESV, SKIP>(A->T, A->pb, A->W, A->SD, fslot, A->chain, threadIdx.x & 63, L[wv], Q, -1, nullptr, nullptr, nullptr);
         hint[0] = __builtin_amdgcn_readfirstlane(hint[0]); hint[1] = __builtin_amdgcn_readfirstlane(hint[1]); hint[2] = __builtin_amdgcn_readfirstlane(hint[2]);
     }
-    if (tail_help_on) tail_help(A->T, A->pb, A->W, A->SD, threadIdx.x & 63, L, wv, QWAVES, Q, TS);
+    if (tail_help_on) tail_help<SKIP>(A->T, A->pb, A->W, A->SD, threadIdx.x & 63, L, wv, QWAVES, Q, TS);
 #ifdef LHIP_PHASE_PROF
     atomicAdd((unsigned long long*)A->W.prof + (threadIdx.x & 63), (unsigned long long)L[wv].prof[threadIdx.x & 63]);
 #endif
@@ -107,7 +107,7 @@
     }
 #endif
 }
-template <int RESV> __global__ __launch_bounds__(128, LHIP_QOCC) void g_quant_pair(QArgs a_unused) {
+template <int RESV, int SKIP> __global__ __launch_bounds__(128, LHIP_QOCC) void g_quant_pair(QArgs a_unused) {
     __shared__ QuantTabs Q;
     __shared__ QuantLds L[2];
     __shared__ int mbox[4];
@@ -115,7 +115,7 @@
     q_copy_tabs(A->T, Q, threadIdx.x, 128);
     __syncthreads();
     const int wv = __builtin_amdgcn_readfirstlane(threadIdx.x >> 6);
-    kb_quant<1, RESV>(A->T, A->pb, A->W, A->SD, blockIdx.x, A->chain, threadIdx.x & 63, L[wv], Q, wv, mbox);
+    kb_quant<1, RESV, SKIP>(A->T, A->pb, A->W, A->SD, blockIdx.x, A->chain, threadIdx.x & 63, L[wv], Q, wv, mbox);
 }
 __global__ __launch_bounds__(256) void g_validate_fast(Tables T, Workspace W, const StreamDesc* SD, int nfs) {
     __shared__ ValidateShare S;
@@ -144,7 +144,7 @@
 #ifndef LHIP_FIXUP_OCC
 #define LHIP_FIXUP_OCC 4
 #endif
-__global__ __launch_bounds__(64 * QWAVES, LHIP_FIXUP_OCC) void g_fixup(QArgs a_unused) {
+template <int SKIP> __global__ __launch_bounds__(64 * QWAVES, LHIP_FIXUP_OCC) void g_fixup(QArgs a_unused) {
     __shared__ QuantTabs Q;
     __shared__ QuantLds L[QWAVES];
     const QArgs* A = (const QArgs*)__builtin_amdgcn_kernarg_segment_ptr();
@@ -167,7 +167,7 @@
         if (nslow > 0) {
             if (!tabs) { q_copy_tabs(A->T, Q, threadIdx.x, nthr); __syncthreads(); tabs = true; }
             for (int i = gw; i < nslow; i += nw)
-                kb_validate(A->T, A->pb, W, A->SD, __builtin_amdgcn_readfirstlane(W.slow_list[i]), lane, L[wv], Q);
+                kb_validate<SKIP>(A->T, A->pb, W, A->SD, __builtin_amdgcn_readfirstlane(W.slow_list[i]), lane, L[wv], Q);
             grid_barrier(base + FX_BAR, nblocks);
         }
         const int nflag = __builtin_amdgcn_readfirstlane(__hip_atomic_load(ctr + FX_NFLAG, __ATOMIC_RELAXED, __HIP_MEMORY_SCOPE_AGENT));
@@ -188,7 +188,7 @@
                 const int l = (int)__builtin_ctzll(m);
                 m &= m - 1;
                 const int fr = b0 + nw * l;
-                kb_quant(A->T, A->pb, W, A->SD, fr, 1, lane, L[wv], Q);
+                kb_quant<0, 0, SKIP>(A->T, A->pb, W, A->SD, fr, 1, lane, L[wv], Q);
                 if (lane == 0) {
                     const StreamDesc* sd = A->SD + W.fslot_stream[fr];
                     const int k = fr - sd->fslot0 - 1;
diff --git a/lamejs_amd/csrc/lhip_math.h b/lamejs_amd/csrc/lhip_math.h
--- a/lamejs_amd/csrc/lhip_math.h
+++ b/lamejs_amd/csrc/lhip_math.h
@@ -113,16 +113,28 @@
 #ifdef LHIP_HOSTSIM
     for (int j = 0; j < N; j++) { ra[j] = (int)((double)xa[j] * (double)istep); rb[j] = (int)((double)xb[j] * (double)istep); }
 #else
-    static_assert(N == 5, "device form is written for 5 pairs per lane");
-    float a0, a1, a2, a3, a4, b0, b1, b2, b3, b4;
-    asm volatile("s_setreg_imm32_b32 hwreg(HW_REG_MODE, 0, 2), 3\n\ts_nop 1\n\t"
-                 "v_mul_f32 %0, %10, %20\n\tv_mul_f32 %1, %11, %20\n\tv_mul_f32 %2, %12, %20\n\tv_mul_f32 %3, %13, %20\n\tv_mul_f32 %4, %14, %20\n\t"
-                 "v_mul_f32 %5, %15, %20\n\tv_mul_f32 %6, %16, %20\n\tv_mul_f32 %7, %17, %20\n\tv_mul_f32 %8, %18, %20\n\tv_mul_f32 %9, %19, %20\n\t"
-                 "s_setreg_imm32_b32 hwreg(HW_REG_MODE, 0, 2), 0\n\ts_nop 1"
-                 : "=&v"(a0), "=&v"(a1), "=&v"(a2), "=&v"(a3), "=&v"(a4), "=&v"(b0), "=&v"(b1), "=&v"(b2), "=&v"(b3), "=&v"(b4)
-                 : "v"(xa[0]), "v"(xa[1]), "v"(xa[2]), "v"(xa[3]), "v"(xa[4]), "v"(xb[0]), "v"(xb[1]), "v"(xb[2]), "v"(xb[3]), "v"(xb[4]), "v"(istep));
-    ra[0] = (int)a0; ra[1] = (int)a1; ra[2] = (int)a2; ra[3] = (int)a3; ra[4] = (int)a4;
-    rb[0] = (int)b0; rb[1] = (int)b1; rb[2] = (int)b2; rb[3] = (int)b3; rb[4] = (int)b4;
+    static_assert(N == 5 || N == 4, "device forms are written for 5 and for 4 pairs per lane (NPL, NPL_HEAD)");
+    if constexpr (N == 5) {
+        float a0, a1, a2, a3, a4, b0, b1, b2, b3, b4;
+        asm volatile("s_setreg_imm32_b32 hwreg(HW_REG_MODE, 0, 2), 3\n\ts_nop 1\n\t"
+                     "v_mul_f32 %0, %10, %20\n\tv_mul_f32 %1, %11, %20\n\tv_mul_f32 %2, %12, %20\n\tv_mul_f32 %3, %13, %20\n\tv_mul_f32 %4, %14, %20\n\t"
+                     "v_mul_f32 %5, %15, %20\n\tv_mul_f32 %6, %16, %20\n\tv_mul_f32 %7, %17, %20\n\tv_mul_f32 %8, %18, %20\n\tv_mul_f32 %9, %19, %20\n\t"
+                     "s_setreg_imm32_b32 hwreg(HW_REG_MODE, 0, 2), 0\n\ts_nop 1"
+                     : "=&v"(a0), "=&v"(a1), "=&v"(a2), "=&v"(a3), "=&v"(a4), "=&v"(b0), "=&v"(b1), "=&v"(b2), "=&v"(b3), "=&v"(b4)
+                     : "v"(xa[0]), "v"(xa[1]), "v"(xa[2]), "v"(xa[3]), "v"(xa[4]), "v"(xb[0]), "v"(xb[1]), "v"(xb[2]), "v"(xb[3]), "v"(xb[4]), "v"(istep));
+        ra[0] = (int)a0; ra[1] = (int)a1; ra[2] = (int)a2; ra[3] = (int)a3; ra[4] = (int)a4;
+        rb[0] = (int)b0; rb[1] = (int)b1; rb[2] = (int)b2; rb[3] = (int)b3; rb[4] = (int)b4;
+    } else {
+        float a0, a1, a2, a3, b0, b1, b2, b3;
+        asm volatile("s_setreg_imm32_b32 hwreg(HW_REG_MODE, 0, 2), 3\n\ts_nop 1\n\t"
+                     "v_mul_f32 %0, %8, %16\n\tv_mul_f32 %1, %9, %16\n\tv_mul_f32 %2, %10, %16\n\tv_mul_f32 %3, %11, %16\n\t"
+                     "v_mul_f32 %4, %12, %16\n\tv_mul_f32 %5, %13, %16\n\tv_mul_f32 %6, %14, %16\n\tv_mul_f32 %7, %15, %16\n\t"
+                     "s_setreg_imm32_b32 hwreg(HW_REG_MODE, 0, 2), 0\n\ts_nop 1"
+                     : "=&v"(a0), "=&v"(a1), "=&v"(a2), "=&v"(a3), "=&v"(b0), "=&v"(b1), "=&v"(b2), "=&v"(b3)
+                     : "v"(xa[0]), "v"(xa[1]), "v"(xa[2]), "v"(xa[3]), "v"(xb[0]), "v"(xb[1]), "v"(xb[2]), "v"(xb[3]), "v"(istep));
+        ra[0] = (int)a0; ra[1] = (int)a1; ra[2] = (int)a2; ra[3] = (int)a3;
+        rb[0] = (int)b0; rb[1] = (int)b1; rb[2] = (int)b2; rb[3] = (int)b3;
+    }
 #endif
 }
 template <int N> LHIP_DEV void q_floor_fma(const float (&xa)[N], const float (&xb)[N], float istep, const float (&ja)[N], const float (&jb)[N],
@@ -133,17 +145,30 @@
         vb[j] = (int)((double)xb[j] * (double)istep + (double)jb[j]);
     }
 #else
-    static_assert(N == 5, "device form is written for 5 pairs per lane");
-    float a0, a1, a2, a3, a4, b0, b1, b2, b3, b4;
-    asm volatile("s_setreg_imm32_b32 hwreg(HW_REG_MODE, 0, 2), 3\n\ts_nop 1\n\t"
-                 "v_fma_f32 %0, %10, %20, %21\n\tv_fma_f32 %1, %11, %20, %22\n\tv_fma_f32 %2, %12, %20, %23\n\tv_fma_f32 %3, %13, %20, %24\n\tv_fma_f32 %4, %14, %20, %25\n\t"
-                 "v_fma_f32 %5, %15, %20, %26\n\tv_fma_f32 %6, %16, %20, %27\n\tv_fma_f32 %7, %17, %20, %28\n\tv_fma_f32 %8, %18, %20, %29\n\tv_fma_f32 %9, %19, %20, %30\n\t"
-                 "s_setreg_imm32_b32 hwreg(HW_REG_MODE, 0, 2), 0\n\ts_nop 1"
-                 : "=&v"(a0), "=&v"(a1), "=&v"(a2), "=&v"(a3), "=&v"(a4), "=&v"(b0), "=&v"(b1), "=&v"(b2), "=&v"(b3), "=&v"(b4)
-                 : "v"(xa[0]), "v"(xa[1]), "v"(xa[2]), "v"(xa[3]), "v"(xa[4]), "v"(xb[0]), "v"(xb[1]), "v"(xb[2]), "v"(xb[3]), "v"(xb[4]), "v"(istep),
-                   "v"(ja[0]), "v"(ja[1]), "v"(ja[2]), "v"(ja[3]), "v"(ja[4]), "v"(jb[0]), "v"(jb[1]), "v"(jb[2]), "v"(jb[3]), "v"(jb[4]));
-    va[0] = (int)a0; va[1] = (int)a1; va[2] = (int)a2; va[3] = (int)a3; va[4] = (int)a4;
-    vb[0] = (int)b0; vb[1] = (int)b1; vb[2] = (int)b2; vb[3] = (int)b3; vb[4] = (int)b4;
+    static_assert(N == 5 || N == 4, "device forms are written for 5 and for 4 pairs per lane (NPL, NPL_HEAD)");
+    if constexpr (N == 5) {
+        float a0, a1, a2, a3, a4, b0, b1, b2, b3, b4;
+        asm volatile("s_setreg_imm32_b32 hwreg(HW_REG_MODE, 0, 2), 3\n\ts_nop 1\n\t"
+                     "v_fma_f32 %0, %10, %20, %21\n\tv_fma_f32 %1, %11, %20, %22\n\tv_fma_f32 %2, %12, %20, %23\n\tv_fma_f32 %3, %13, %20, %24\n\tv_fma_f32 %4, %14, %20, %25\n\t"
+                     "v_fma_f32 %5, %15, %20, %26\n\tv_fma_f32 %6, %16, %20, %27\n\tv_fma_f32 %7, %17, %20, %28\n\tv_fma_f32 %8, %18, %20, %29\n\tv_fma_f32 %9, %19, %20, %30\n\t"
+                     "s_setreg_imm32_b32 hwreg(HW_REG_MODE, 0, 2), 0\n\ts_nop 1"
+                     : "=&v"(a0), "=&v"(a1), "=&v"(a2), "=&v"(a3), "=&v"(a4), "=&v"(b0), "=&v"(b1), "=&v"(b2), "=&v"(b3), "=&v"(b4)
+                     : "v"(xa[0]), "v"(xa[1]), "v"(xa[2]), "v"(xa[3]), "v"(xa[4]), "v"(xb[0]), "v"(xb[1]), "v"(xb[2]), "v"(xb[3]), "v"(xb[4]), "v"(istep),
+                       "v"(ja[0]), "v"(ja[1]), "v"(ja[2]), "v"(ja[3]), "v"(ja[4]), "v"(jb[0]), "v"(jb[1]), "v"(jb[2]), "v"(jb[3]), "v"(jb[4]));
+        va[0] = (int)a0; va[1] = (int)a1; va[2] = (int)a2; va[3] = (int)a3; va[4] = (int)a4;
+        vb[0] = (int)b0; vb[1] = (int)b1; vb[2] = (int)b2; vb[3] = (int)b3; vb[4] = (int)b4;
+    } else {
+        float a0, a1, a2, a3, b0, b1, b2, b3;
+        asm volatile("s_setreg_imm32_b32 hwreg(HW_REG_MODE, 0, 2), 3\n\ts_nop 1\n\t"
+                     "v_fma_f32 %0, %8, %16, %17\n\tv_fma_f32 %1, %9, %16, %18\n\tv_fma_f32 %2, %10, %16, %19\n\tv_fma_f32 %3, %11, %16, %20\n\t"
+                     "v_fma_f32 %4, %12, %16, %21\n\tv_fma_f32 %5, %13, %16, %22\n\tv_fma_f32 %6, %14, %16, %23\n\tv_fma_f32 %7, %15, %16, %24\n\t"
+                     "s_setreg_imm32_b32 hwreg(HW_REG_MODE, 0, 2), 0\n\ts_nop 1"
+                     : "=&v"(a0), "=&v"(a1), "=&v"(a2), "=&v"(a3), "=&v"(b0), "=&v"(b1), "=&v"(b2), "=&v"(b3)
+                     : "v"(xa[0]), "v"(xa[1]), "v"(xa[2]), "v"(xa[3]), "v"(xb[0]), "v"(xb[1]), "v"(xb[2]), "v"(xb[3]), "v"(istep),
+                       "v"(ja[0]), "v"(ja[1]), "v"(ja[2]), "v"(ja[3]), "v"(jb[0]), "v"(jb[1]), "v"(jb[2]), "v"(jb[3]));
+        va[0] = (int)a0; va[1] = (int)a1; va[2] = (int)a2; va[3] = (int)a3;
+        vb[0] = (int)b0; vb[1] = (int)b1; vb[2] = (int)b2; vb[3] = (int)b3;
+    }
 #endif
 }
 
diff --git a/lamejs_amd/csrc/lhip_pipeline_hip.h b/lamejs_amd/csrc/lhip_pipeline_hip.h
--- a/lamejs_amd/csrc/lhip_pipeline_hip.h
+++ b/lamejs_amd/csrc/lhip_pipeline_hip.h
@@ -86,20 +86,22 @@
 #endif
     P.paths |= pair ? LHIP_PATH_QUANT_PAIR : LHIP_PATH_QUANT_PERSISTENT;
     { QArgs qa; qa.T = T; qa.pb = ts.pb10; qa.W = W; qa.SD = dSD; qa.chain = 0; qa.nfs = nfs; qa.ctr = 0;
-      if (pair) LAUNCHB(KT_QUANT, g_quant_pair<0>, nfs, 128, st, qa); else LAUNCHB(KT_QUANT, g_quant<0>, qgrid, 64 * QWAVES, st, qa); }
+      if (pair) { if (ts.skip_tail) LAUNCHB(KT_QUANT, (g_quant_pair<0, 1>), nfs, 128, st, qa); else LAUNCHB(KT_QUANT, (g_quant_pair<0, 0>), nfs, 128, st, qa); }
+      else { if (ts.skip_tail) LAUNCHB(KT_QUANT, (g_quant<0, 1>), qgrid, 64 * QWAVES, st, qa); else LAUNCHB(KT_QUANT, (g_quant<0, 0>), qgrid, 64 * QWAVES, st, qa); } }
     if (nfr > 0) {
         QArgs qa; qa.T = T; qa.pb = ts.pb10; qa.W = W; qa.SD = dSD; qa.chain = 1; qa.nfs = nfs; qa.ctr = 0;
         LAUNCHB(KT_VALIDATE, g_validate_fast, (nfs + 63) / 64, 256, st, T, W, dSD, nfs);
         int fgrid = (nfs + 63) / 64;
         if (ctx->fixup_wg_per_cu == 0) {
             int nb = 0;
-            if (hipOccupancyMaxActiveBlocksPerMultiprocessor(&nb, (const void*)g_fixup, 64 * QWAVES, 0) != hipSuccess || nb < 1) nb = 1;
+            if (hipOccupancyMaxActiveBlocksPerMultiprocessor(&nb, (const void*)g_fixup<1>, 64 * QWAVES, 0) != hipSuccess || nb < 1) nb = 1;
             ctx->fixup_wg_per_cu = nb < LHIP_FIXUP_OCC / 2 ? nb : LHIP_FIXUP_OCC / 2;
         }
         if (fgrid > ctx->num_cus * ctx->fixup_wg_per_cu) fgrid = ctx->num_cus * ctx->fixup_wg_per_cu;
         if (fgrid < 1) fgrid = 1;
         P.paths |= fgrid == 1 ? LHIP_PATH_FIXUP_SINGLE : LHIP_PATH_FIXUP_COOP;
-        if (fgrid == 1) LAUNCHB(KT_VALIDATE, g_fixup, 1, 64 * QWAVES, st, qa);
+        const void* fixup_fn = ts.skip_tail ? (const void*)g_fixup<1> : (const void*)g_fixup<0>;
+        if (fgrid == 1) { if (ts.skip_tail) LAUNCHB(KT_VALIDATE, g_fixup<1>, 1, 64 * QWAVES, st, qa); else LAUNCHB(KT_VALIDATE, g_fixup<0>, 1, 64 * QWAVES, st, qa); }
         else {
             kt_begin(KT_VALIDATE, st);
             void* kargs[] = {(void*)&qa};
@@ -109,7 +111,7 @@
                 if (!rt::event_record(ctx->ev_coop[0], st) || !rt::stream_wait_event(nullptr, ctx->ev_coop[0])) return false;
                 cst = nullptr;
             }
-            hipError_t e_ = hipLaunchCooperativeKernel((const void*)g_fixup, dim3(fgrid), dim3(64 * QWAVES), kargs, 0, cst);
+            hipError_t e_ = hipLaunchCooperativeKernel(fixup_fn, dim3(fgrid), dim3(64 * QWAVES), kargs, 0, cst);
             if (ctx->own_stream && e_ == hipSuccess) { if (!rt::event_record(ctx->ev_coop[1], nullptr) || !rt::stream_wait_event(st, ctx->ev_coop[1])) return false; }
             kt_end(st);
             TRACE_SYNC(g_fixup_cooperative, st);
diff --git a/lamejs_amd/csrc/lhip_pipeline_sim.h b/lamejs_amd/csrc/lhip_pipeline_sim.h
--- a/lamejs_amd/csrc/lhip_pipeline_sim.h
+++ b/lamejs_amd/csrc/lhip_pipeline_sim.h
@@ -5,10 +5,10 @@
 #define WAVE_RUN(...) do { const int lane_ = 0; __VA_ARGS__; } while (0)
 #endif
 #ifdef LHIP_WAVESIM
-#define QUANT_RUN(chain_) do { if (pair) wsim::run_block(2, [&](int wave_, int lane_) { kb_quant<1, 0>(T, ts.pb10, W, dSD, b, chain_, lane_, LQ2[wave_], QT, wave_, mbox); }); \
-                       else WAVE_RUN(kb_quant<0, 0>(T, ts.pb10, W, dSD, b, chain_, lane_, LQ, QT)); } while (0)
+#define QUANT_RUN(chain_) do { if (pair) wsim::run_block(2, [&](int wave_, int lane_) { kb_quant<1, 0, 1>(T, ts.pb10, W, dSD, b, chain_, lane_, LQ2[wave_], QT, wave_, mbox); }); \
+                       else WAVE_RUN(kb_quant<0, 0, 1>(T, ts.pb10, W, dSD, b, chain_, lane_, LQ, QT)); } while (0)
 #else
-#define QUANT_RUN(chain_) WAVE_RUN(kb_quant<0, 0>(T, ts.pb10, W, dSD, b, chain_, lane_, LQ, QT))
+#define QUANT_RUN(chain_) WAVE_RUN(kb_quant<0, 0, 1>(T, ts.pb10, W, dSD, b, chain_, lane_, LQ, QT))
 #endif
 static void gain_sim_run(const Tables& T, const Workspace& W, const StreamDesc* SD, const StreamIO* IO, const GainDesc* D, int S, int stage_blocks, int waves) {
     static thread_local float LG[LHIP_NL * 2 * GAIN_STRIDE];
@@ -125,9 +125,9 @@
                 if (lane_ == 0) f = ctr++;
                 f = wave_bcast(f, 0);
                 if (f >= nfs) break;
-                kb_quant_th(T, ts.pb10, W, dSD, f, lane_, LQ8[wave_], QT, hint, TS, wave_);
+                kb_quant_th<1>(T, ts.pb10, W, dSD, f, lane_, LQ8[wave_], QT, hint, TS, wave_);
             }
-            if (C == 2) tail_help(T, ts.pb10, W, dSD, lane_, LQ8, wave_, 8, QT, TS);
+            if (C == 2) tail_help<1>(T, ts.pb10, W, dSD, lane_, LQ8, wave_, 8, QT, TS);
         });
     } else
 #endif
@@ -138,18 +138,18 @@
             if (pair) { QUANT_RUN(0); continue; }
             int hl[64][3];
             for (int l = 0; l < 64; l++) for (int q = 0; q < 3; q++) hl[l][q] = hints[b % 3][q];
-            WAVE_RUN(kb_quant<0, 0>(T, ts.pb10, W, dSD, b, 0, lane_, LQ, QT, -1, nullptr, nullptr, hl[lane_]));
+            WAVE_RUN(kb_quant<0, 0, 1>(T, ts.pb10, W, dSD, b, 0, lane_, LQ, QT, -1, nullptr, nullptr, hl[lane_]));
             for (int l = 1; l < 64; l++) for (int q = 0; q < 3; q++) if (hl[l][q] != hl[0][q]) { set_err("wavesim: seed hint not wave-uniform"); return false; }
             for (int q = 0; q < 3; q++) hints[b % 3][q] = hl[0][q];
 #else
-            WAVE_RUN(kb_quant<0, 0>(T, ts.pb10, W, dSD, b, 0, lane_, LQ, QT, -1, nullptr, nullptr, hints[b % 3]));
+            WAVE_RUN(kb_quant<0, 0, 1>(T, ts.pb10, W, dSD, b, 0, lane_, LQ, QT, -1, nullptr, nullptr, hints[b % 3]));
 #endif
         }
     }
     for (;;) {
         W.nflagged[0] = 0; W.nflagged[1] = 0;
         for (int b = 0; b < nfs; b++) kb_validate_fast(T, W, dSD, b);
-        for (int i = 0; i < W.nflagged[1]; i++) WAVE_RUN(kb_validate(T, ts.pb10, W, dSD, W.slow_list[i], lane_, LQ, QT));
+        for (int i = 0; i < W.nflagged[1]; i++) WAVE_RUN(kb_validate<1>(T, ts.pb10, W, dSD, W.slow_list[i], lane_, LQ, QT));
         const int nf = W.nflagged[0];
         if (nf == 0) break;
         repaired += nf; iters++;
diff --git a/lamejs_amd/csrc/lhip_tables.h b/lamejs_amd/csrc/lhip_tables.h
--- a/lamejs_amd/csrc/lhip_tables.h
+++ b/lamejs_amd/csrc/lhip_tables.h
@@ -12,6 +12,7 @@
     int base_frame_bytes = 0;
     bool bad_option = false;
     InfoTagCfg tag;
+    bool skip_tail = false;
     int gain_on = 0;
     ~TableSet() { rt::dfree(d_blob); rt::dfree(d_extra); rt::dfree(d_qtabs); }
 };
@@ -217,6 +218,7 @@
     extra.resize(amp_at + 64);
     {
         const float* h_af = (const float*)host_arr("amp_filter");
+        ts.skip_tail = (double)h_af[28] < 1e-12 && (double)h_af[29] < 1e-12 && (double)h_af[30] < 1e-12 && (double)h_af[31] < 1e-12;
         const int32_t* h_order = (const int32_t*)host_arr("mdct_order");
         double amp[32];
         for (int i = 0; i < 32; i++) amp[i] = 1.0;
```

Result: faster. 2.349 million frames/s, median of 6 (+2.4%).
